# yilane/rag-project-icd10

Measured on AMD Instinct MI355X. Metric: queries_per_sec, higher is better.
Workload: dtype f16; 1 GPU; BASELINE configs[1]: 10000 random fp32 768-d queries x 37000x768 corpus, top_k=10, search only (pre-embedded, HBM-resident inputs), level reweight fused; nq_per_gpu=10000, corpus_rows=37000, dim=768, top_k=10, mode=auto, parallelism=single GPU, collective_ranks=1

## Files before the change

### include/icd_search.h

```cpp
#ifndef ICD_SEARCH_H
#define ICD_SEARCH_H

#include <stdint.h>

#ifdef __cplusplus
extern "C" {
#endif

#define ICD_ABI_VERSION 6
#define ICD_MAX_K 128

typedef struct icd_index icd_index;

typedef enum icd_status {
    ICD_OK = 0,
    ICD_ERR_INVALID = -1,
    ICD_ERR_HIP = -2,
    ICD_ERR_NOMEM = -3,
    ICD_ERR_UNSUPPORTED = -4,
    ICD_ERR_STATE = -5
} icd_status;

typedef enum icd_mode {
    ICD_MODE_AUTO = 0,
// ... 116 lines not shown
                          int32_t lmax, const int32_t *limits, int32_t ranker, double rrf_c, const double *weights, int32_t norm,
                          int32_t k, int32_t reweighted, double *out_adj, double *out_fused, int64_t *out_ids,
                          int32_t *out_levels, uint32_t *out_reqbits, int32_t out_on_device, void *stream);

int icd_index_search_hybrid_grouped(icd_index *idx, icd_fusion *fusion, icd_grouping *grouping, const float *queries, int64_t nq, int32_t R,
                                    int32_t queries_on_device, const int32_t *limits, icd_rowmask *const *masks, const float *radius,
                                    const float *range_filter, int32_t ranker, double rrf_c, const double *weights, int32_t norm, int32_t k,
                                    int32_t group_size, int32_t reweighted, double *out_adj, double *out_fused, int64_t *out_ids,
                                    int32_t *out_levels, uint32_t *out_reqbits, int32_t *out_groups, int32_t out_on_device, void *stream);
int icd_fusion_fuse_lists_grouped(icd_index *idx, icd_fusion *fusion, icd_grouping *grouping, const float *scores, const int64_t *ids,
                                  int64_t nq, int32_t R, int32_t lmax, const int32_t *limits, int32_t ranker, double rrf_c,
                                  const double *weights, int32_t norm, int32_t k, int32_t group_size, int32_t reweighted, double *out_adj,
                                  double *out_fused, int64_t *out_ids, int32_t *out_levels, uint32_t *out_reqbits, int32_t *out_groups,
                                  int32_t out_on_device, void *stream);

typedef struct icd_sparse icd_sparse;
#define ICD_SPARSE_MAX_QUERY_TERMS 64
int icd_sparse_tile_rows(void);
int icd_sparse_pack(const int64_t *row_off, const uint32_t *terms, const float *vals, int64_t n, int64_t vocab,
                    int64_t *post_off, uint32_t *post_row, float *post_val);
int icd_sparse_create(icd_index *idx, const int64_t *row_off, const uint32_t *terms, const float *vals, int64_t vocab,
                      int32_t max_nq, int32_t max_k, icd_sparse **out);
int icd_sparse_destroy(icd_sparse *sp);
int icd_sparse_stats(icd_sparse *sp, int64_t *out_vocab, int64_t *out_nnz, int64_t *out_bytes);
int icd_sparse_search(icd_index *idx, icd_sparse *sp, const int64_t *q_off, const uint32_t *q_terms, const float *q_vals,
                      int64_t nq, int32_t k, int32_t queries_on_device, icd_rowmask *const *masks, int32_t reweighted,
                      double *out_adj, float *out_raw, int64_t *out_ids, int32_t *out_levels, int32_t out_on_device, void *stream);
int icd_sparse_search_range(icd_index *idx, icd_sparse *sp, const int64_t *q_off, const uint32_t *q_terms, const float *q_vals,
                            int64_t nq, int32_t k, int32_t queries_on_device, icd_rowmask *const *masks,
                            const float *radius, const float *range_filter, const float *after_scores, const int64_t *after_ids,
                            int32_t bounds_on_device, int32_t reweighted,
                            double *out_adj, float *out_raw, int64_t *out_ids, int32_t *out_levels, int32_t out_on_device, void *stream);

int icd_grouping_pair_sparse(icd_index *idx, icd_grouping *grouping, icd_sparse *sp);
int icd_sparse_search_grouped(icd_index *idx, icd_sparse *sp, icd_grouping *grouping, const int64_t *q_off, const uint32_t *q_terms,
                              const float *q_vals, int64_t nq, int32_t k, int32_t group_size, int32_t queries_on_device,
                              icd_rowmask *const *masks, int32_t reweighted, double *out_adj, float *out_raw, int64_t *out_ids,
                              int32_t *out_levels, int32_t *out_groups, int32_t out_on_device, void *stream);

int icd_sparse_match_rowmasks(icd_index *idx, icd_sparse *sp, const int64_t *q_off, const uint32_t *q_terms, const int32_t *min_match,
                              int64_t nq, int32_t queries_on_device, icd_rowmask *const *base_masks, icd_rowmask **out_masks, void *stream);
int icd_rowmask_read(icd_rowmask *m, uint32_t *out_words, int64_t out_count);

typedef struct icd_columns icd_columns;
#define ICD_FILTER_MAX_COLUMNS 256
#define ICD_FILTER_RANGE 1
#define ICD_FILTER_SET 2
#define ICD_FILTER_TEXT 3
#define ICD_FILTER_AND 4
#define ICD_FILTER_OR 5
#define ICD_FILTER_NOT 6
int icd_columns_create(icd_index *idx, const int32_t *cols, int32_t ncols, icd_columns **out);
int icd_columns_destroy(icd_columns *columns);
int icd_columns_stats(icd_columns *columns, int32_t *out_ncols, int64_t *out_rows, int64_t *out_bytes);
int icd_filter_program_check(const int64_t *prog_off, const uint32_t *prog, int64_t nq, int32_t ncols, int64_t vocab, char *msg, int64_t msg_len);
int icd_filter_rowmasks(icd_index *idx, icd_columns *columns, icd_sparse *sparse, const int64_t *prog_off, const uint32_t *prog, int64_t nq,
                        icd_rowmask *const *base_masks, icd_rowmask **out_masks, void *stream);

#define ICD_SELECT_MAX_LIMIT 16384
int icd_rowmask_select(icd_index *idx, icd_rowmask *const *masks, int64_t nq, const int64_t *offsets, int32_t limit, int64_t *out_ids,
                       int64_t *out_total, int32_t *out_taken, int32_t out_on_device, void *stream);

int icd_rowmask_group_counts(icd_index *idx, icd_grouping *grouping, icd_rowmask *const *masks, int64_t nq,
                             int32_t *out_counts , int32_t out_on_device, void *stream);

typedef struct icd_mmr icd_mmr;
int icd_mmr_create(icd_index *idx, int64_t max_nq, icd_mmr **out);
int icd_mmr_destroy(icd_mmr *mmr);
int icd_mmr_stats(icd_mmr *mmr, int64_t *out_max_nq, int64_t *out_bytes);
int icd_index_search_mmr(icd_index *idx, icd_mmr *mmr, icd_rowmask *const *masks, const float *queries, int64_t nq, int32_t k,
                         int32_t fetch_k, double lambda, int32_t queries_on_device, const float *radius, const float *range_filter,
                         int32_t bounds_on_device, int32_t reweighted, double *out_adj, float *out_raw, int64_t *out_ids,
                         int32_t *out_levels, double *out_mmr, int32_t out_on_device, void *stream);

#define ICD_MAX_BOOSTS 4
typedef struct icd_boost icd_boost;
int icd_boost_create(icd_index *idx, int64_t max_nq, icd_boost **out);
int icd_boost_destroy(icd_boost *b);
int icd_boost_stats(icd_boost *b, int64_t *out_max_nq, int64_t *out_bytes);
int icd_index_search_boosted(icd_index *idx, icd_boost *ws, icd_rowmask *const *masks,
                             icd_rowmask *const *boost_masks ,
                             const float *boost_weights      ,
                             const float *queries, int64_t nq, int32_t k, int32_t queries_on_device,
                             const float *radius, const float *range_filter, const float *after_scores, const int64_t *after_ids,
                             int32_t bounds_on_device, int32_t reweighted, double *out_adj, float *out_raw, int64_t *out_ids,
                             int32_t *out_levels, int32_t out_on_device, void *stream);

typedef struct icd_byrows icd_byrows;
int icd_byrows_create(icd_index *idx, int64_t max_nq, icd_byrows **out);
int icd_byrows_destroy(icd_byrows *ws);
int icd_byrows_stats(icd_byrows *ws, int64_t *out_max_nq, int64_t *out_bytes);
int icd_index_search_by_rows(icd_index *idx, icd_byrows *ws, icd_rowmask *const *masks, const int64_t *ids, int64_t nq, int32_t k,
                             int32_t ids_on_device, int32_t include_self, const float *radius, const float *range_filter,
                             int32_t bounds_on_device, int32_t reweighted, double *out_adj, float *out_raw, int64_t *out_ids,
                             int32_t *out_levels, int32_t out_on_device, void *stream);

int icd_merge_topk(int32_t device, const float *scores, const int64_t *ids, const int32_t *levels,
                   int32_t G, int64_t nq, int32_t k,
                   double *out_adj, float *out_raw, int64_t *out_ids, int32_t *out_levels, void *stream);

#define ICD_GROUP_ID_BYTES 128
typedef struct icd_group icd_group;
typedef enum icd_group_mode { ICD_GROUP_ROW_SHARD = 0, ICD_GROUP_QUERY_SHARD = 1 } icd_group_mode;
int icd_group_unique_id(uint8_t *out_id );
int icd_group_create(icd_index *local, const uint8_t *id, int32_t rank, int32_t world, int32_t mode, int32_t max_nq,
                     int32_t max_k, icd_group **out);
int icd_group_prepare(icd_index *local, int32_t with_comm, int32_t rank, int32_t world, int32_t mode, int32_t max_nq,
                      int32_t max_k, icd_group **out);
int icd_group_connect(icd_group *group, const uint8_t *id);
int icd_group_search(icd_group *group, const float *queries, int64_t nq, int32_t k, int32_t gather, double *out_adj,
                     float *out_raw, int64_t *out_ids, int32_t *out_levels, void *stream);
int icd_group_destroy(icd_group *group);

int icd_index_lookup_levels(icd_index *idx, const int64_t *ids, int64_t count, int32_t *out_levels,
                            void *stream);

int icd_hier_rescore(int32_t device, const double *adj, const int64_t *ids, int64_t nq, int32_t k, int64_t id_base,
                     int64_t n_rows, const uint8_t *row_tags, const double *q_params, const double *weights,
                     int32_t *out_order, double *out_enhanced, double *out_score, double *out_vs, double *out_hb,
                     double *out_boost, void *stream);

int icd_hier_rescore_entities(int32_t device, const double *adj, const int64_t *ids, int64_t nq, int32_t k, int64_t id_base,
                              int64_t n_rows, const uint8_t *row_tags, const double *q_params, const double *weights,
                              int32_t *out_order, double *out_enhanced, double *out_score, double *out_vs, double *out_hb,
                              double *out_boost, void *stream);

int icd_score_stats(int32_t device, const double *scores, const int32_t *order, int64_t nq, int32_t k, int32_t use,
                    double *out, void *stream);

int icd_pack_winners(int32_t device, const int32_t *order, const int64_t *ids, const float *raw, const double *adj, const double *enhanced,
                     const double *vs, const double *hb, const double *boost, int64_t nq, int32_t k, int32_t kk, double *out, void *stream);

int icd_cosine_rows(int32_t device, const float *x, const float *y, int64_t y_stride, int64_t nq, int32_t dim,
                    double *out, void *stream);

#define ICD_TERM_MAX_LEN 32
int icd_term_first_match(int32_t device, const int32_t *key_cp, const int32_t *key_off, int32_t n_keys, const int32_t *term_cp,
                         const int32_t *term_off, int32_t n_terms, int32_t *out_first, void *stream);

int icd_packed_attention(int32_t device, const float *qkv, int64_t ld, const int32_t *starts, int32_t nseq, int32_t heads,
                         int32_t head_dim, int32_t max_len, float *out, int64_t out_ld, void *stream);

int icd_split_bf16x3(int32_t device, const float *x, int64_t rows, int32_t cols, int64_t ld, int32_t act, void *out, void *stream);

int icd_index_stats(icd_index *idx, icd_stats *out);

int icd_index_cert_terms(icd_index *idx, float *cmax, float *dcmax, int32_t *cexp, float *qnorm, float *qres, int64_t count);

int icd_index_set_chunks(icd_index *idx, int32_t chunks);

int icd_index_set_second_pass(icd_index *idx, int32_t enabled);

enum { ICD_OPT_FAMILY_ORDER = 1, ICD_OPT_STREAM_ONE = 2, ICD_OPT_HOST_ONE = 3, ICD_OPT_PACING_SHIFT = 4, ICD_OPT_PACING_LEAD = 5, ICD_OPT_EXACT_NARROW = 6,
       ICD_OPT_WIDE_FROM = 7 };
int icd_index_set_option(icd_index *idx, int32_t option, int32_t value);

int icd_unpack_query_slices(int32_t device, const void *gathered, int32_t world, int64_t nq, int32_t k, double *out_adj,
                                  float *out_raw, int64_t *out_ids, int32_t *out_levels, void *stream);

typedef struct icd_encoder icd_encoder;
typedef struct {
    int32_t layers, hidden, heads, inter;
    int32_t vocab, max_pos;
    int32_t pos_offset;
    float ln_eps;
    const float *word_emb, *pos_emb, *type_emb0, *emb_ln_g, *emb_ln_b;
    const float *const *w_qkv;  const float *const *b_qkv;
    const float *const *w_ao;   const float *const *b_ao;
    const float *const *ln1_g;  const float *const *ln1_b;
    const float *const *w_up;   const float *const *b_up;
    const float *const *w_down; const float *const *b_down;
    const float *const *ln2_g;  const float *const *ln2_b;
    int32_t arithmetic;
} icd_encoder_desc;
enum { ICD_ENCODER_ARITH_FP32 = 0, ICD_ENCODER_ARITH_BF16X3 = 1 };
#define ICD_ENCODER_MAX_TOKENS 512
#define ICD_ENCODER_MAX_SEQS 64
int icd_encoder_create(int32_t device, const icd_encoder_desc *desc, icd_encoder **out);
int icd_encoder_encode(icd_encoder *e, const int32_t *ids, const int32_t *lengths, int32_t nseq, int32_t pooling, int32_t normalize,
                       float *out, int32_t out_on_device, float *hidden_out, void *stream);
int icd_encoder_encode_many(icd_encoder *e, const int32_t *ids, const int32_t *lengths, int64_t nseq, int32_t pooling, int32_t normalize,
                            float *out, int32_t out_on_device, void *stream);
int icd_encoder_destroy(icd_encoder *e);

int icd_index_debug_counters(icd_index *idx, unsigned long long *out, int32_t count);

int icd_index_set_profiling(icd_index *idx, int32_t enabled);
int icd_index_last_profile(icd_index *idx, icd_profile *out);
int icd_index_profile_summary(icd_index *idx, icd_profile *out_mean, int32_t *out_count);

#ifdef __cplusplus
}
#endif
#endif
```

### rag_project_icd10_amd/_native.py

```python
from __future__ import annotations

import ctypes as C
import math
import os
import sys
from typing import Optional

import numpy as np

_HERE = os.path.dirname(os.path.abspath(__file__))
LIB_PATH = os.path.join(_HERE, "csrc", "libicdsearch.so")

MODE_AUTO = 0
MODE_EXACT = 1
MAX_K = 128
ABI_VERSION = 6

EXPORTED_SYMBOLS = (
    "icd_abi_version", "icd_last_error", "icd_device_count", "icd_index_create", "icd_index_create_view", "icd_index_destroy",
    "icd_index_search", "icd_index_search_reweighted", "icd_merge_topk", "icd_index_lookup_levels",
    "icd_index_stats", "icd_index_cert_terms", "icd_index_set_chunks", "icd_index_debug_counters", "icd_index_set_profiling",
    "icd_index_last_profile", "icd_index_profile_summary", "icd_index_set_option", "icd_packed_attention",
    "icd_hier_rescore", "icd_hier_rescore_entities",
    "icd_score_stats",
    "icd_cosine_rows",
    "icd_term_first_match",
    "icd_index_set_second_pass",
    "icd_group_unique_id", "icd_group_create", "icd_group_prepare", "icd_group_connect", "icd_group_search", "icd_group_destroy",
    "icd_unpack_query_slices", "icd_split_bf16x3", "icd_encoder_create", "icd_encoder_encode", "icd_encoder_encode_many", "icd_encoder_destroy", "icd_pack_winners",
    "icd_grouping_create", "icd_grouping_destroy", "icd_grouping_stats", "icd_index_search_grouped",
    "icd_index_search_range",
    "icd_rowmask_create", "icd_rowmask_destroy", "icd_rowmask_stats", "icd_rowmask_pack", "icd_index_search_masked",
    "icd_fusion_create", "icd_fusion_destroy", "icd_fusion_stats", "icd_index_search_hybrid", "icd_fusion_fuse_lists",
    "icd_sparse_tile_rows", "icd_sparse_pack", "icd_sparse_create", "icd_sparse_destroy", "icd_sparse_stats", "icd_sparse_search",
    "icd_grouping_pair_sparse", "icd_sparse_search_grouped", "icd_index_search_hybrid_grouped", "icd_fusion_fuse_lists_grouped",
    "icd_sparse_search_range",
    "icd_sparse_match_rowmasks", "icd_rowmask_read",
    "icd_columns_create", "icd_columns_destroy", "icd_columns_stats", "icd_filter_program_check", "icd_filter_rowmasks",
    "icd_rowmask_select", "icd_rowmask_group_counts",
    "icd_mmr_create", "icd_mmr_destroy", "icd_mmr_stats", "icd_index_search_mmr",
    "icd_boost_create", "icd_boost_destroy", "icd_boost_stats", "icd_index_search_boosted",
    "icd_byrows_create", "icd_byrows_destroy", "icd_byrows_stats", "icd_index_search_by_rows",
    "icd_grouping_prepare_scorers", "icd_index_search_grouped_scored",
    "icd_grouping_prepare_maxsim", "icd_index_search_maxsim",
)
MAXSIM_SCORERS = {"sum": 1, "mean": 2}
MAXSIM_MAX_T = 64
GROUP_SCORERS = {"max": 0, "sum": 1, "avg": 2}
MAX_BOOSTS = 4
SELECT_MAX_LIMIT = 16384
SELECT_SEGMENT_ROWS = 16384
FACET_LDS_GROUPS = 8192
SPARSE_MAX_QUERY_TERMS = 64
MAX_REQUESTS = 8
RANKER_RRF, RANKER_WEIGHTED = 0, 1
NORMS = {"none": 0, "cosine": 1, "atan": 2}
MAX_K = 128
CREATE_CORPUS_ON_DEVICE, CREATE_ROW_ORDER, CREATE_NO_PROBE, CREATE_NO_CENTER = 1, 2, 4, 8
OPTIONS = {"family_order": 1, "stream_one": 2, "host_one": 3, "pacing_shift": 4, "pacing_lead": 5, "exact_narrow": 6, "wide_from": 7}
GROUP_ROW_SHARD = 0
GROUP_QUERY_SHARD = 1
GROUP_ID_BYTES = 128
SPLIT_TAIL = 64


class IcdError(RuntimeError):

    def __init__(self, code: int, text: str):
        super().__init__(f"libicdsearch error {code}: {text}")
        self.code = code


class _Stats(C.Structure):
    _fields_ = [("n", C.c_int64), ("dim", C.c_int32), ("device", C.c_int32), ("id_base", C.c_int64),
                ("bytes_corpus_f32", C.c_int64), ("bytes_corpus_f16", C.c_int64), ("bytes_workspace", C.c_int64),
                ("max_nq", C.c_int32), ("max_k", C.c_int32), ("fast_path", C.c_int32), ("rmax", C.c_float),
                ("last_nq", C.c_int64), ("last_fallback", C.c_int64), ("last_chunks", C.c_int32),
                ("last_mode", C.c_int32), ("last_second_pass", C.c_int64), ("last_second_pass_lists", C.c_int32),
                ("second_pass_armed", C.c_int32), ("wide_mode", C.c_int32), ("sparse_fallback_armed", C.c_int32),
                ("centered", C.c_int32), ("mean_share", C.c_float)]


_ENC_LAYER_FIELDS = ("w_qkv", "b_qkv", "w_ao", "b_ao", "ln1_g", "ln1_b", "w_up", "b_up", "w_down", "b_down", "ln2_g", "ln2_b")


class _EncoderDesc(C.Structure):
    _fields_ = ([("layers", C.c_int32), ("hidden", C.c_int32), ("heads", C.c_int32), ("inter", C.c_int32), ("vocab", C.c_int32),
                 ("max_pos", C.c_int32), ("pos_offset", C.c_int32), ("ln_eps", C.c_float),
                 ("word_emb", C.c_void_p), ("pos_emb", C.c_void_p), ("type_emb0", C.c_void_p), ("emb_ln_g", C.c_void_p), ("emb_ln_b", C.c_void_p)]
                + [(name, C.POINTER(C.c_void_p)) for name in _ENC_LAYER_FIELDS] + [("arithmetic", C.c_int32)])


ENCODER_ARITH = {"fp32": 0, "bf16x3": 1}
ENCODER_MAX_TOKENS = 512
ENCODER_MAX_SEQS = 64


class _Profile(C.Structure):
    _fields_ = [("ms_prep", C.c_float), ("ms_coarse", C.c_float), ("ms_finalize", C.c_float),
                ("ms_exact", C.c_float), ("ms_exact_finalize", C.c_float), ("ms_total", C.c_float)]


_lib = None


def load_library(path: Optional[str] = None) -> C.CDLL:
    global _lib
    if _lib is not None and path is None:
        return _lib
    p = path or os.environ.get("ICD_SEARCH_LIB", LIB_PATH)
    if not os.path.exists(p):
        raise ImportError(
            f"{p} not found: the HIP extension is not built. Run `python -c 'import __graft_entry__ as g; g.build()'` "
            f"or `make -C rag_project_icd10_amd/csrc`. There is no CPU fallback for the search path.")
    lib = C.CDLL(p)
    vp, i32, i64 = C.c_void_p, C.c_int32, C.c_int64
    lib.icd_abi_version.restype = C.c_int
    lib.icd_last_error.restype = C.c_char_p
    lib.icd_device_count.restype = C.c_int
    lib.icd_index_create.argtypes = [vp, i64, i32, vp, i64, i32, i32, i32, i32, C.POINTER(vp)]
    lib.icd_index_create_view.argtypes = [vp, vp, i64, i32, i32, i32, i32, C.POINTER(vp)]
    lib.icd_index_destroy.argtypes = [vp]
    lib.icd_index_search.argtypes = [vp, vp, i64, i32, i32, i32, vp, vp, i32, vp]
    lib.icd_index_search_reweighted.argtypes = [vp, vp, i64, i32, i32, i32, vp, vp, vp, vp, i32, vp]
    lib.icd_grouping_create.argtypes = [vp, vp, i64, i32, i32, C.POINTER(vp)]
    lib.icd_grouping_destroy.argtypes = [vp]
    lib.icd_grouping_stats.argtypes = [vp, C.POINTER(i64), C.POINTER(i64), C.POINTER(i64)]
    lib.icd_index_search_grouped.argtypes = [vp, vp, vp, i64, i32, i32, i32, i32, vp, vp, vp, vp, vp, i32, vp]
    lib.icd_grouping_prepare_scorers.argtypes = [vp, vp]
    lib.icd_index_search_grouped_scored.argtypes = [vp, vp, vp, i64, i32, i32, i32, i32, i32, vp, vp, vp, vp, vp, vp, vp, i32, vp]
    lib.icd_grouping_prepare_maxsim.argtypes = [vp, vp, i64, i64]
    lib.icd_index_search_maxsim.argtypes = [vp, vp, vp, vp, i64, i32, i32, i32, vp, vp, vp, vp, vp, i32, vp]
    lib.icd_index_search_range.argtypes = [vp, vp, i64, i32, i32, vp, vp, vp, vp, i32, i32, vp, vp, vp, vp, i32, vp]
    lib.icd_rowmask_create.argtypes = [vp, vp, i64, i32, C.POINTER(vp)]
    lib.icd_rowmask_destroy.argtypes = [vp]
    lib.icd_rowmask_stats.argtypes = [vp, C.POINTER(i64), C.POINTER(i64)]
    lib.icd_rowmask_pack.argtypes = [vp, i64, i64, vp, i64]
    lib.icd_index_search_masked.argtypes = [vp, vp, vp, i64, i32, i32, vp, vp, vp, vp, i32, i32, vp, vp, vp, vp, i32, vp]
    lib.icd_fusion_create.argtypes = [vp, i64, C.POINTER(vp)]
    lib.icd_fusion_destroy.argtypes = [vp]
    lib.icd_fusion_stats.argtypes = [vp, C.POINTER(i64), C.POINTER(i64)]
    lib.icd_index_search_hybrid.argtypes = [vp, vp, vp, i64, i32, i32, vp, vp, vp, vp, i32, i32, i32, C.c_double, vp, i32, i32, i32,
                                            vp, vp, vp, vp, vp, i32, vp]
    lib.icd_fusion_fuse_lists.argtypes = [vp, vp, vp, vp, i64, i32, i32, vp, i32, C.c_double, vp, i32, i32, i32, vp, vp, vp, vp, vp, i32, vp]
    lib.icd_sparse_tile_rows.restype = C.c_int
    lib.icd_sparse_pack.argtypes = [vp, vp, vp, i64, i64, vp, vp, vp]
    lib.icd_sparse_create.argtypes = [vp, vp, vp, vp, i64, i32, i32, C.POINTER(vp)]
    lib.icd_sparse_destroy.argtypes = [vp]
    lib.icd_sparse_stats.argtypes = [vp, C.POINTER(i64), C.POINTER(i64), C.POINTER(i64)]
    lib.icd_sparse_search.argtypes = [vp, vp, vp, vp, vp, i64, i32, i32, vp, i32, vp, vp, vp, vp, i32, vp]
    lib.icd_sparse_search_range.argtypes = [vp, vp, vp, vp, vp, i64, i32, i32, vp, vp, vp, vp, vp, i32, i32, vp, vp, vp, vp, i32, vp]
    lib.icd_grouping_pair_sparse.argtypes = [vp, vp, vp]
    lib.icd_sparse_match_rowmasks.argtypes = [vp, vp, vp, vp, vp, i64, i32, vp, vp, vp]
    lib.icd_rowmask_read.argtypes = [vp, vp, i64]
    lib.icd_columns_create.argtypes = [vp, vp, i32, C.POINTER(vp)]
    lib.icd_columns_destroy.argtypes = [vp]
    lib.icd_columns_stats.argtypes = [vp, C.POINTER(i32), C.POINTER(i64), C.POINTER(i64)]
    lib.icd_filter_program_check.argtypes = [vp, vp, i64, i32, i64, vp, i64]
    lib.icd_filter_rowmasks.argtypes = [vp, vp, vp, vp, vp, i64, vp, vp, vp]
    lib.icd_rowmask_select.argtypes = [vp, vp, i64, vp, i32, vp, vp, vp, i32, vp]
    lib.icd_rowmask_group_counts.argtypes = [vp, vp, vp, i64, vp, i32, vp]
    lib.icd_mmr_create.argtypes = [vp, i64, C.POINTER(vp)]
    lib.icd_mmr_destroy.argtypes = [vp]
    lib.icd_mmr_stats.argtypes = [vp, C.POINTER(i64), C.POINTER(i64)]
    lib.icd_index_search_mmr.argtypes = [vp, vp, vp, vp, i64, i32, i32, C.c_double, i32, vp, vp, i32, i32, vp, vp, vp, vp, vp, i32, vp]
    lib.icd_byrows_create.argtypes = [vp, i64, C.POINTER(vp)]
    lib.icd_byrows_destroy.argtypes = [vp]
    lib.icd_byrows_stats.argtypes = [vp, C.POINTER(i64), C.POINTER(i64)]
    lib.icd_index_search_by_rows.argtypes = [vp, vp, vp, vp, i64, i32, i32, i32, vp, vp, i32, i32, vp, vp, vp, vp, i32, vp]
    lib.icd_boost_create.argtypes = [vp, i64, C.POINTER(vp)]
    lib.icd_boost_destroy.argtypes = [vp]
    lib.icd_boost_stats.argtypes = [vp, C.POINTER(i64), C.POINTER(i64)]
    lib.icd_index_search_boosted.argtypes = [vp, vp, vp, vp, vp, vp, i64, i32, i32, vp, vp, vp, vp, i32, i32, vp, vp, vp, vp, i32, vp]
    lib.icd_index_search_hybrid_grouped.argtypes = [vp, vp, vp, vp, i64, i32, i32, vp, vp, vp, vp, i32, C.c_double, vp, i32, i32, i32, i32,
                                                    vp, vp, vp, vp, vp, vp, i32, vp]
    lib.icd_fusion_fuse_lists_grouped.argtypes = [vp, vp, vp, vp, vp, i64, i32, i32, vp, i32, C.c_double, vp, i32, i32, i32, i32,
                                                  vp, vp, vp, vp, vp, vp, i32, vp]
    lib.icd_sparse_search_grouped.argtypes = [vp, vp, vp, vp, vp, vp, i64, i32, i32, i32, vp, i32, vp, vp, vp, vp, vp, i32, vp]
    lib.icd_merge_topk.argtypes = [i32, vp, vp, vp, i32, i64, i32, vp, vp, vp, vp, vp]
    lib.icd_index_lookup_levels.argtypes = [vp, vp, i64, vp, vp]
    lib.icd_index_stats.argtypes = [vp, C.POINTER(_Stats)]
    lib.icd_index_cert_terms.argtypes = [vp, vp, vp, vp, vp, vp, i64]
    lib.icd_index_set_chunks.argtypes = [vp, i32]
    lib.icd_index_set_second_pass.argtypes = [vp, i32]
    lib.icd_index_set_option.argtypes = [vp, i32, i32]
    lib.icd_group_unique_id.argtypes = [vp]
    lib.icd_group_create.argtypes = [vp, vp, i32, i32, i32, i32, i32, C.POINTER(vp)]
    lib.icd_group_prepare.argtypes = [vp, i32, i32, i32, i32, i32, i32, C.POINTER(vp)]
    lib.icd_group_connect.argtypes = [vp, vp]
    lib.icd_group_search.argtypes = [vp, vp, i64, i32, i32, vp, vp, vp, vp, vp]
    lib.icd_group_destroy.argtypes = [vp]
    lib.icd_split_bf16x3.argtypes = [i32, vp, i64, i32, i64, i32, vp, vp]
    lib.icd_unpack_query_slices.argtypes = [i32, vp, i32, i64, i32, vp, vp, vp, vp, vp]
    lib.icd_packed_attention.argtypes = [i32, vp, i64, vp, i32, i32, i32, i32, vp, i64, vp]
    lib.icd_encoder_create.argtypes = [i32, C.POINTER(_EncoderDesc), C.POINTER(vp)]
    lib.icd_encoder_encode.argtypes = [vp, vp, vp, i32, i32, i32, vp, i32, vp, vp]
    lib.icd_encoder_encode_many.argtypes = [vp, vp, vp, i64, i32, i32, vp, i32, vp]
    lib.icd_encoder_destroy.argtypes = [vp]
    lib.icd_hier_rescore.argtypes = [i32, vp, vp, i64, i32, i64, i64, vp, vp, vp, vp, vp, vp, vp, vp, vp, vp]
    lib.icd_hier_rescore_entities.argtypes = lib.icd_hier_rescore.argtypes
    lib.icd_score_stats.argtypes = [i32, vp, vp, i64, i32, i32, vp, vp]
    lib.icd_pack_winners.argtypes = [i32, vp, vp, vp, vp, vp, vp, vp, vp, i64, i32, i32, vp, vp]
    lib.icd_cosine_rows.argtypes = [i32, vp, vp, i64, i64, i32, vp, vp]
    lib.icd_term_first_match.argtypes = [i32, vp, vp, i32, vp, vp, i32, vp, vp]
    lib.icd_index_debug_counters.argtypes = [vp, vp, i32]
    lib.icd_index_set_profiling.argtypes = [vp, i32]
    lib.icd_index_last_profile.argtypes = [vp, C.POINTER(_Profile)]
    lib.icd_index_profile_summary.argtypes = [vp, C.POINTER(_Profile), C.POINTER(C.c_int32)]
    have = lib.icd_abi_version()
    if have != ABI_VERSION:
        raise ImportError(f"{p} has ABI version {have}, this package needs {ABI_VERSION}: rebuild it (make -C rag_project_icd10_amd/csrc)")
    for name in EXPORTED_SYMBOLS:
# ... 1476 lines not shown
```

### rag_project_icd10_amd/csrc/coarse_flat_kernel.hpp

```cpp
#pragma once
#include "coarse_common.hpp"
#include "flat_partition.hpp"

namespace icd {

struct CoarseFlatArgs {
    const _Float16 *q16;
    const _Float16 *c16;
    int nq;
    int n;
    int n_pad;
    int ctiles;
    int total_units;
    int units_per_wg;
    int pos_period;
    int list_tiles;
    int boot_tiles;
    int sparse_from;
    int P;
    float *part_scores;
    int *part_rows;
    float *bounds;
    unsigned int *shared_thr;
    const int *nq_ptr;
    const int *qlist;
    int nwg_virtual;
    int skip_below;
    unsigned long long *dbg;
    unsigned int *pace;
    int pace_period;
    int pace_epochs;
    int pace_shift;
    int pace_lead;
};

constexpr int CO_BOOT_MIN_TILES = 6;
constexpr int CO_KP_WIDE = 24;
constexpr int CO_BOOT_TILES = 8;
constexpr int PACE_SPIN_LIMIT = 20000;
constexpr int CO_SPARSE_FROM = 40;

template <int KP>
__device__ __forceinline__ float flush_emit_parallel(const char *smem, uint32_t qb, int h, int rot, int nlo, int nhi, float thr,
                                                      bool store, float *out_scores, int *out_rows) {
    constexpr int CAP = 64, HALF = 32;
    float v[HALF];
    uint32_t rw[HALF];
    const int lo_end = nlo, hi_begin = CAP - nhi;
#pragma unroll
    for (int j = 0; j < HALF; ++j) {
        const int slot = HALF * h + ((j + rot) & (HALF - 1));
        const bool valid = slot < lo_end || slot >= hi_begin;
        const float sv = *reinterpret_cast<const float *>(smem + qb + slot * 4);
        rw[j] = *reinterpret_cast<const uint32_t *>(smem + qb + CAP * 4 + slot * 4);
        v[j] = valid ? sv : -INFINITY;
    }
    auto pair_sum = [&](int x) {
        const auto sw = __builtin_amdgcn_permlane32_swap((unsigned)x, (unsigned)x, false, false);
        return x + (int)(h ? sw[0] : sw[1]);
    };
    const int total = nlo + nhi;
    float mx = -INFINITY;
#pragma unroll
    for (int j = 0; j < HALF; ++j) mx = fmaxf(mx, v[j]);
    {
        const auto sw = __builtin_amdgcn_permlane32_swap(__float_as_uint(mx), __float_as_uint(mx), false, false);
        mx = fmaxf(mx, __uint_as_float(h ? sw[0] : sw[1]));
    }
    uint32_t lo = order_f32(thr), hi = order_f32(mx);
    int cnt_lo = 0;
#pragma unroll
    for (int j = 0; j < HALF; ++j) cnt_lo += (v[j] > thr) ? 1 : 0;
    cnt_lo = pair_sum(cnt_lo);
    bool active = total > KP && cnt_lo > KP && hi > lo + 1u;
    while (__builtin_amdgcn_ballot_w64(active) != 0ull) {
        const uint32_t mid = lo + ((hi - lo) >> 1);
        const float midf = unorder_f32(mid);
        int c = 0;
#pragma unroll
        for (int j = 0; j < HALF; ++j) c += (v[j] > midf) ? 1 : 0;
        c = pair_sum(c);
        if (active) {
            if (c >= KP) { lo = mid; cnt_lo = c; } else hi = mid;
            active = cnt_lo > KP && hi > lo + 1u;
        }
    }
    float cut = total > KP ? unorder_f32(lo) : -INFINITY;
    float bound = total > KP ? cut : thr;
    int quota_ties = 0;
    float tie = 0.0f;
    if (cnt_lo > KP) {
        tie = unorder_f32(hi);
        int above = 0, tied = 0;
#pragma unroll
        for (int j = 0; j < HALF; ++j) { above += (v[j] > tie) ? 1 : 0; tied += (v[j] == tie) ? 1 : 0; }
        const int above_all = pair_sum(above);
        const auto sw = __builtin_amdgcn_permlane32_swap((unsigned)tied, (unsigned)tied, false, false);
        const int tied_low_lane = h ? (int)sw[0] : tied;
        const int room = KP - above_all;
        quota_ties = h ? max(0, min(tied, room - min(tied_low_lane, room))) : min(tied, room);
        cut = tie;
        bound = tie;
    }
    int mine_n = 0;
#pragma unroll
    for (int j = 0; j < HALF; ++j) mine_n += (v[j] > cut) ? 1 : 0;
    mine_n += quota_ties;
    const auto swn = __builtin_amdgcn_permlane32_swap((unsigned)mine_n, (unsigned)mine_n, false, false);
    const int other_n = (int)(h ? swn[0] : swn[1]);
    int dest = h ? other_n : 0;
    const int kept = mine_n + other_n;
    if (store) {
        int ties_left = quota_ties;
#pragma unroll
        for (int j = 0; j < HALF; ++j) {
            bool take = v[j] > cut;
            if (!take && ties_left > 0 && v[j] == tie && cnt_lo > KP) { take = true; --ties_left; }
            if (take) {
                out_scores[dest] = v[j];
                out_rows[dest] = (int)rw[j];
                ++dest;
            }
        }
        if (h == 0) {
            for (int d = kept; d < KP; ++d) { out_scores[d] = -INFINITY; out_rows[d] = -1; }
        }
    }
    return bound;
}

template <int KP, typename Ops>
__device__ __forceinline__ void compact_all_parallel(char *smem, Sel2 &st, uint32_t qb, int h, int rot) {
    constexpr int CAP = 64, HALF = 32;
    const int mine = Ops::used(st, h);
    const auto swm = __builtin_amdgcn_permlane32_swap((unsigned)mine, (unsigned)mine, false, false);
    const int other = (int)(h ? swm[0] : swm[1]);
    const int nlo = st.kept + (h ? other : mine), nhi = h ? mine : other;
    const int total = nlo + nhi;
    float v[HALF];
    uint32_t rw[HALF];
    const int lo_end = nlo, hi_begin = CAP - nhi;
#pragma unroll
    for (int j = 0; j < HALF; ++j) {
        const int slot = HALF * h + ((j + rot) & (HALF - 1));
        const bool valid = slot < lo_end || slot >= hi_begin;
        const float sv = *reinterpret_cast<const float *>(smem + qb + slot * 4);
        rw[j] = *reinterpret_cast<const uint32_t *>(smem + qb + CAP * 4 + slot * 4);
        v[j] = valid ? sv : -INFINITY;
    }
    auto pair_sum = [&](int x) {
        const auto sw = __builtin_amdgcn_permlane32_swap((unsigned)x, (unsigned)x, false, false);
        return x + (int)(h ? sw[0] : sw[1]);
    };
    float mx = -INFINITY;
#pragma unroll
    for (int j = 0; j < HALF; ++j) mx = fmaxf(mx, v[j]);
    {
        const auto sw = __builtin_amdgcn_permlane32_swap(__float_as_uint(mx), __float_as_uint(mx), false, false);
        mx = fmaxf(mx, __uint_as_float(h ? sw[0] : sw[1]));
    }
    uint32_t lo = order_f32(st.thr), hi = order_f32(mx);
    int cnt_lo = 0;
#pragma unroll
    for (int j = 0; j < HALF; ++j) cnt_lo += (v[j] > st.thr) ? 1 : 0;
    cnt_lo = pair_sum(cnt_lo);
    bool active = total > KP && cnt_lo > KP && hi > lo + 1u;
    while (__builtin_amdgcn_ballot_w64(active) != 0ull) {
        const uint32_t mid = lo + ((hi - lo) >> 1);
        const float midf = unorder_f32(mid);
        int c = 0;
#pragma unroll
        for (int j = 0; j < HALF; ++j) c += (v[j] > midf) ? 1 : 0;
        c = pair_sum(c);
        if (active) {
            if (c >= KP) { lo = mid; cnt_lo = c; } else hi = mid;
            active = cnt_lo > KP && hi > lo + 1u;
        }
    }
    float cut = unorder_f32(lo);
    int quota_ties = 0;
    float tie = 0.0f;
    if (cnt_lo > KP) {
        tie = unorder_f32(hi);
        int above = 0, tied = 0;
#pragma unroll
        for (int j = 0; j < HALF; ++j) { above += (v[j] > tie) ? 1 : 0; tied += (v[j] == tie) ? 1 : 0; }
        const int above_all = pair_sum(above);
        const auto sw = __builtin_amdgcn_permlane32_swap((unsigned)tied, (unsigned)tied, false, false);
        const int tied_low_lane = h ? (int)sw[0] : tied;
        const int room = KP - above_all;
        quota_ties = h ? max(0, min(tied, room - min(tied_low_lane, room))) : min(tied, room);
        cut = tie;
    }
    int mine_n = 0;
#pragma unroll
    for (int j = 0; j < HALF; ++j) mine_n += (v[j] > cut) ? 1 : 0;
    mine_n += quota_ties;
    const auto swn = __builtin_amdgcn_permlane32_swap((unsigned)mine_n, (unsigned)mine_n, false, false);
    const int other_n = (int)(h ? swn[0] : swn[1]);
    if (total > KP) {
        int dest = h ? other_n : 0;
        int ties_left = quota_ties;
#pragma unroll
        for (int j = 0; j < HALF; ++j) {
            bool take = v[j] > cut;
            if (!take && ties_left > 0 && v[j] == tie && cnt_lo > KP) { take = true; --ties_left; }
            if (take) {
                *reinterpret_cast<float *>(smem + qb + dest * 4) = v[j];
                *reinterpret_cast<uint32_t *>(smem + qb + CAP * 4 + dest * 4) = rw[j];
                ++dest;
            }
        }
        const int kept = mine_n + other_n;
        st.thr = cut;
        st.kept = kept;
        st.aw0 = h ? qb + (CAP - 1) * 4 : qb + (uint32_t)kept * 4;
        st.aw = st.aw0;
    }
}

constexpr int CF_PRODUCT_VAR = 1 + 2 + 8 + 128 + 16 + 2048 + 32768;
constexpr int CF_CACHED_VAR = CF_PRODUCT_VAR + 2097152 + 4194304 + 134217728 + 268435456 + 1073741824;
constexpr int CF_PACED_VAR = CF_PRODUCT_VAR + 67108864;
__host__ __device__ constexpr int cf_ring_stages(int var) { return (var & 1048576) ? 6 : CO_S; }
__host__ __device__ constexpr int cf_lds_bytes(int var) { return cf_ring_stages(var) * CO_STAGE_BYTES + CO_BM * CO_CAP * 8 + ((var & 1048576) ? 0 : 4 * 256); }
#define ICD_CF_STAMP(t) do { __builtin_amdgcn_sched_barrier(0); \
    asm volatile("s_memtime %0\n\ts_waitcnt lgkmcnt(0)" : "=s"(t) :: "memory"); \
    __builtin_amdgcn_sched_barrier(0); } while (0)

template <int D, int VAR = CF_PRODUCT_VAR, int KP = CO_KP, bool PERSIST = false>
__global__ __launch_bounds__(256, 1) void coarse_flat_kernel(CoarseFlatArgs a) {
    constexpr int CO_QUOTA = (CO_CAP - KP) / 2 - CO_CHECK_EVERY;
    static_assert(CO_QUOTA >= 8 && KP + 2 * (CO_QUOTA + CO_CHECK_EVERY) <= CO_CAP, "candidate buffer layout");
    constexpr bool EARLY_THR = (VAR & 1) != 0;
    constexpr bool DMA_SPREAD = (VAR & 2) != 0;
    constexpr bool Q_AGPR = (VAR & 8) != 0;
    constexpr bool PF2 = (VAR & 128) != 0;
    constexpr bool REV_WAIT = (VAR & 4) != 0;
    constexpr bool QUAD = (VAR & 16) != 0;
    constexpr bool SETPRIO = (VAR & 131072) != 0;
    constexpr int EXCH = (VAR & 524288) ? 4 : ((VAR & 262144) ? 2 : 1);
    constexpr bool X16 = (VAR & 32768) != 0;
    static_assert(!X16 || (QUAD && (VAR & 8) != 0 && D % 32 == 0), "the 16x16x32 form is built on the quad select and pinned queries");
    constexpr int EPOCH = ((VAR & 32) && (VAR & 2048)) ? 32 : ((VAR & 32) ? 16 : ((VAR & 2048) ? 24 : 0));
    constexpr bool NOBAR = (VAR & 256) != 0, NOVM = (VAR & 512) != 0, STAMPS = (VAR & 1024) != 0;
    constexpr bool NOPASS = (VAR & 4096) != 0, NOSEL = (VAR & 8192) != 0, NODMA = (VAR & 16384) != 0;
    constexpr bool PAIRBAR = (VAR & 1048576) != 0;
    constexpr bool DMA_WIDE = (VAR & 2097152) != 0;
    constexpr bool BOOT_MED3 = (VAR & 4194304) != 0;
    constexpr bool DIRTY_GUARD = (VAR & 8388608) != 0;
    constexpr bool SPARSE_PRE = (VAR & 16777216) != 0;
    static_assert(!SPARSE_PRE || (QUAD && X16), "the group pre-filter is built on the quad select of the 16x16x32 form");
    static_assert(!DMA_WIDE || (X16 && DMA_SPREAD && PF2 && !NODMA), "the wide spread is built on the product's 16x16x32 stage");
    constexpr bool CLOCKS = (VAR & 33554432) != 0;
    constexpr bool PACE = (VAR & 67108864) != 0;
    static_assert(!PACE || (EARLY_THR && EXCH == 1 && !PERSIST), "the pace poll rides on the early threshold load of every tile");
    static_assert(!(CLOCKS && STAMPS), "one use of the debug buffer at a time");
    constexpr bool LOOKAHEAD = (VAR & 134217728) != 0;
    constexpr int LA_B = (VAR & 268435456) ? 8 : 4;
    constexpr bool LA_MAX = (VAR & 536870912) != 0;
    static_assert(!LOOKAHEAD || (QUAD && X16 && !SPARSE_PRE), "the look-ahead tests are built on the quad select of the 16x16x32 form");
    constexpr bool LA_GUARDX = (VAR & 1073741824) != 0;
    static_assert(LOOKAHEAD || (VAR & (268435456 | 536870912 | 1073741824)) == 0, "sub-flags of the look-ahead bit");
    static_assert(!LA_GUARDX || !DIRTY_GUARD, "one form of the overflow guard");
    constexpr int S = cf_ring_stages(VAR);
    constexpr int VM_MID = NOVM ? 63 : (PAIRBAR ? 4 : 4 * (S - 3));
    constexpr int PRO = PAIRBAR ? 4 : S - 1;
    constexpr int VM_TILE_END = NOVM ? 0 : (PAIRBAR ? (DMA_WIDE ? 6 : 8) : (DMA_WIDE ? 4 * (S - 2) - 2 : 4 * (S - 2)));
    constexpr int KS = D / CO_BK;
    constexpr int NF = D / 16;
    static_assert(KS % S == 0, "ring slot must be a compile-time function of the stage");
    using Ops = Sel2Ops<KP>;
    extern __shared__ __attribute__((aligned(16))) char smem[];

    const int tid = threadIdx.x, lane = tid & 63;
    const int wave = __builtin_amdgcn_readfirstlane(tid >> 6);
    const int c = lane & 31, h = lane >> 5;
    const int q16 = lane & 15, g16 = lane >> 4;
    const int nq_act = PERSIST && a.nq_ptr ? min(__builtin_amdgcn_readfirstlane(*a.nq_ptr), a.nq) : a.nq;
    const int total_units = PERSIST ? ((nq_act + CO_BM - 1) / CO_BM) * a.ctiles : a.total_units;
    const int nwg_logical = PERSIST ? (total_units + a.units_per_wg - 1) / a.units_per_wg : (int)gridDim.x;
    if (PERSIST && nq_act <= a.skip_below) return;
    unsigned long long clk_c0 = 0, clk_r0 = 0;
    if constexpr (CLOCKS) {
        clk_c0 = __builtin_amdgcn_s_memtime();
        clk_r0 = __builtin_amdgcn_s_memrealtime();
        __builtin_amdgcn_s_waitcnt(0xC07F);
    }

    uint32_t src_off[4];
#pragma unroll
    for (int i = 0; i < 4; ++i) {
        const int row_local = (wave * 4 + i) * 8 + (lane >> 3);
        const int piece = (lane & 7) ^ ((row_local >> 1) & 7);
        src_off[i] = (uint32_t)row_local * (uint32_t)(D * 2) + (uint32_t)piece * 16u - (uint32_t)(i * 1024);
    }
    uint32_t rd_off[4];
    if constexpr (X16) {
#pragma unroll
        for (int k2 = 0; k2 < 2; ++k2) rd_off[k2] = (uint32_t)q16 * 128u + (uint32_t)(((4 * k2 + g16) ^ ((q16 >> 1) & 7)) * 16);
        rd_off[2] = rd_off[3] = 0u;
    } else {
        const int sw = (c >> 1) & 7;
#pragma unroll
        for (int s = 0; s < 4; ++s) rd_off[s] = (uint32_t)c * 128u + (uint32_t)(((2 * s + h) ^ sw) * 16);
    }
    auto read_frags = [&](half8 (&f)[4], int ring_slot, int s) {
        if constexpr (X16) {
            const char *sb = smem + ring_slot * CO_STAGE_BYTES + (s & 1) * 8192 + rd_off[s >> 1];
#pragma unroll
            for (int t = 0; t < 4; ++t) f[t] = *reinterpret_cast<const half8 *>(sb + t * 2048);
        } else {
            const char *sb = smem + ring_slot * CO_STAGE_BYTES + rd_off[s];
#pragma unroll
            for (int t = 0; t < 4; ++t) f[t] = *reinterpret_cast<const half8 *>(sb + t * 4096);
        }
    };
    constexpr uint32_t RING_BYTES = (uint32_t)S * CO_STAGE_BYTES;
    const uint32_t wave_qbase = RING_BYTES + (uint32_t)(wave * 32) * Ops::QBYTES;
    const uint32_t wave_scratch = RING_BYTES + (uint32_t)CO_BM * Ops::QBYTES + (uint32_t)wave * 256u;
    unsigned long long st_vm = 0, st_bar = 0, st_body = 0, st_sel = 0, st_tiles = 0, st_prev = 0;
    unsigned long long st_comp[2] = {0, 0}, st_thr = 0, st_boot = 0;
    [[maybe_unused]] unsigned long long st_app = 0;
    const int last_tile = a.ctiles - 1;

    half8 qf[NF];
    int cur_mtile = -1;
    for (int vblock = (int)blockIdx.x; vblock < (PERSIST ? nwg_logical : (int)blockIdx.x + 1); vblock += PERSIST ? (int)gridDim.x : 1) {
    const int wg = flat_workgroup_of_block(vblock, nwg_logical, a.pos_period);
    const int u_begin = wg * a.units_per_wg;
    const int u_end = min(total_units, u_begin + a.units_per_wg);
    if (u_begin >= u_end) continue;
    int u = u_begin;
    [[maybe_unused]] bool pacing = false;
    [[maybe_unused]] int pace_cls = 0, pace_members = 0, pace_last_epochs = 0;
    [[maybe_unused]] bool pace_last_mine = false;
    if constexpr (PACE) {
        if (a.pace && a.pace_period > 0) {
            pacing = true;
            pace_cls = wg % a.pace_period;
            pace_members = (nwg_logical - pace_cls + a.pace_period - 1) / a.pace_period;
            const int last_units = total_units - (nwg_logical - 1) * a.units_per_wg;
            pace_last_mine = ((nwg_logical - 1) % a.pace_period) == pace_cls;
            pace_last_epochs = last_units >> a.pace_shift;
        }
    }
    while (u < u_end) {
        const int mtile = u / a.ctiles;
        const int t0 = u - mtile * a.ctiles;
        const int run0 = max(u_begin - mtile * a.ctiles, 0);
        const int run1 = min(u_end - mtile * a.ctiles, a.ctiles);
        const int j = (t0 - run0) / a.list_tiles;
        const int t1 = min(run1, run0 + (j + 1) * a.list_tiles);
        const int ntiles = t1 - t0;
        const int ord = flat_first_ordinal(mtile, wg, a.ctiles, a.units_per_wg, a.list_tiles) + j;
        const int slot0 = mtile * CO_BM;

        if (mtile != cur_mtile) {
            if constexpr (X16) {
#pragma unroll
                for (int gr = 0; gr < 2; ++gr) {
                    int qr = slot0 + wave * 32 + 16 * gr + q16;
                    if (PERSIST && a.qlist) qr = a.qlist[min(qr, nq_act - 1)];
                    const _Float16 *qrow = a.q16 + (size_t)qr * D + 8 * g16;
#pragma unroll
                    for (int s = 0; s < NF / 2; ++s) qf[gr * (NF / 2) + s] = *reinterpret_cast<const half8 *>(qrow + 32 * s);
                }
            } else {
                int qr = slot0 + wave * 32 + c;
                if (PERSIST && a.qlist) qr = a.qlist[min(qr, nq_act - 1)];
                const _Float16 *qrow = a.q16 + (size_t)qr * D + 8 * h;
#pragma unroll
                for (int s = 0; s < NF; ++s) qf[s] = *reinterpret_cast<const half8 *>(qrow + 16 * s);
            }
            if constexpr (Q_AGPR) {
#pragma unroll
                for (int s = 0; s < NF; ++s) asm volatile("" : "+a"(qf[s]));
            }
            cur_mtile = mtile;
        }
        const __amdgpu_buffer_rsrc_t crsrc = __builtin_amdgcn_make_buffer_rsrc(
            const_cast<_Float16 *>(a.c16) + (size_t)t0 * CO_BN * D, 0,
            (int)min((size_t)(a.ctiles - t0) * CO_BN * (size_t)(D * 2), (size_t)0x7FFFFFFF), 0x00020000);
        auto issue_pieces = [&](int g_tile, int g_ks, int ring_slot, auto LO, auto HI) {
            const int trow = min(g_tile, last_tile - t0);
            char *dst = smem + ring_slot * CO_STAGE_BYTES + wave * 4096;
            const uint32_t soff = (uint32_t)trow * (uint32_t)(CO_BN * D * 2) + (uint32_t)g_ks * (CO_BK * 2);
            __attribute__((address_space(3))) void *ldst = (__attribute__((address_space(3))) void *)dst;
            constexpr int lo = decltype(LO)::value, hi = decltype(HI)::value;
            if constexpr (lo <= 0 && 0 < hi) __builtin_amdgcn_raw_ptr_buffer_load_lds(crsrc, ldst, 16, src_off[0], soff, 0, 0);
            if constexpr (lo <= 1 && 1 < hi) __builtin_amdgcn_raw_ptr_buffer_load_lds(crsrc, ldst, 16, src_off[1], soff, 1024, 0);
            if constexpr (lo <= 2 && 2 < hi) __builtin_amdgcn_raw_ptr_buffer_load_lds(crsrc, ldst, 16, src_off[2], soff, 2048, 0);
            if constexpr (lo <= 3 && 3 < hi) __builtin_amdgcn_raw_ptr_buffer_load_lds(crsrc, ldst, 16, src_off[3], soff, 3072, 0);
        };
        auto issue_stage = [&](int g_tile, int g_ks, int ring_slot) {
            issue_pieces(g_tile, g_ks, ring_slot, std::integral_constant<int, 0>{}, std::integral_constant<int, 4>{});
        };

        Sel2 st;
        Ops::init(st, wave_qbase + (uint32_t)c * Ops::QBYTES, h, (slot0 + wave * 32 + c) < nq_act && !NOPASS);
        float boot1 = -INFINITY, boot2 = -INFINITY, boot3 = -INFINITY;
        const int boot_tiles = ntiles >= CO_BOOT_MIN_TILES ? min(a.boot_tiles, ntiles / 3) : 0;
        unsigned int *my_shared = a.shared_thr + (slot0 + wave * 32 + c);
        const bool publish = (slot0 + wave * 32 + c) < nq_act;
        uint32_t published = 0u;
        int dirty = 0;
        auto filter_reg = [&](const f32x16 (&pa)[4], auto F, uint32_t rowbase, auto GUARD) {
            constexpr int f = decltype(F)::value;
            constexpr int t = f >> 4, r = f & 15;
            constexpr uint32_t roff = (uint32_t)(t * 32 + (r & 3) + 8 * (r >> 2));
            float v = pa[t][r];
            if constexpr (decltype(GUARD)::value) {
                if ((int)(rowbase + roff) >= a.n) v = -INFINITY;
            }
            const bool pass = v > st.thr;
            if (__builtin_expect(__builtin_amdgcn_ballot_w64(pass) != 0ull, 0)) {
                asm volatile("" ::: "memory");
                if (pass) {
                    *reinterpret_cast<float *>(smem + st.aw) = v;
                    *reinterpret_cast<uint32_t *>(smem + st.aw + Ops::ROW_OFF) = rowbase + roff;
                    st.aw += st.inc;
                }
            }
            if constexpr (r % CO_CHECK_EVERY == CO_CHECK_EVERY - 1) {
                if (__builtin_amdgcn_ballot_w64(Ops::used(st, h) > CO_QUOTA) != 0ull)
                    Ops::template check<PAIRBAR>(st, lane, smem, wave_qbase, wave_scratch, false, CO_LIMIT, STAMPS ? st_comp : nullptr, CO_QUOTA);
            }
        };

        [[maybe_unused]] auto append_quad = [&](unsigned long long m0, unsigned long long m1, unsigned long long m2, unsigned long long m3,
                               float v0, float v1, float v2, float v3, uint32_t rowq) {
            uint32_t r1, r2, r3, aw = st.aw;
            const uint32_t inc = st.inc;
            asm volatile("v_or_b32_e32 %1, 1, %12\n\t"
                         "v_or_b32_e32 %2, 2, %12\n\t"
                         "v_or_b32_e32 %3, 3, %12\n\t"
                         "s_mov_b64 exec, %4\n\t"
                         "ds_write2st64_b32 %0, %8, %12 offset1:1\n\t"
                         "v_add_u32_e32 %0, %0, %13\n\t"
                         "s_mov_b64 exec, %5\n\t"
                         "ds_write2st64_b32 %0, %9, %1 offset1:1\n\t"
                         "v_add_u32_e32 %0, %0, %13\n\t"
                         "s_mov_b64 exec, %6\n\t"
                         "ds_write2st64_b32 %0, %10, %2 offset1:1\n\t"
                         "v_add_u32_e32 %0, %0, %13\n\t"
                         "s_mov_b64 exec, %7\n\t"
                         "ds_write2st64_b32 %0, %11, %3 offset1:1\n\t"
                         "v_add_u32_e32 %0, %0, %13\n\t"
                         "s_mov_b64 exec, -1"
                         : "+v"(aw), "=&v"(r1), "=&v"(r2), "=&v"(r3)
                         : "s"(m0), "s"(m1), "s"(m2), "s"(m3), "v"(v0), "v"(v1), "v"(v2), "v"(v3), "v"(rowq), "v"(inc)
                         : "memory");
            st.aw = aw;
            if constexpr (DIRTY_GUARD) dirty = 1;
            if constexpr (STAMPS) st_app += (unsigned long long)(__builtin_popcountll(m0) + __builtin_popcountll(m1) + __builtin_popcountll(m2) + __builtin_popcountll(m3));
        };
        [[maybe_unused]] auto quad_guard = [&]() {
            if constexpr (LA_GUARDX) {
                const uint32_t aw = st.aw, aw0 = st.aw0;
                uint32_t dist;
                asm("v_sad_u32 %0, %1, %2, 0" : "=v"(dist) : "v"(aw), "v"(aw0));
                if (__builtin_amdgcn_ballot_w64(dist > 4u * (uint32_t)CO_QUOTA) != 0ull)
                    Ops::template check<PAIRBAR>(st, lane, smem, wave_qbase, wave_scratch, false, CO_LIMIT, STAMPS ? st_comp : nullptr, CO_QUOTA);
            } else
            if constexpr (DIRTY_GUARD) {
                if (dirty) {
                    dirty = 0;
                    if (__builtin_amdgcn_ballot_w64(Ops::used(st, h) > CO_QUOTA) != 0ull)
                        Ops::template check<PAIRBAR>(st, lane, smem, wave_qbase, wave_scratch, false, CO_LIMIT, STAMPS ? st_comp : nullptr, CO_QUOTA);
                }
            } else if (__builtin_amdgcn_ballot_w64(Ops::used(st, h) > CO_QUOTA) != 0ull)
                Ops::template check<PAIRBAR>(st, lane, smem, wave_qbase, wave_scratch, false, CO_LIMIT, STAMPS ? st_comp : nullptr, CO_QUOTA);
        };
        auto filter_quad = [&](const f32x16 (&pa)[X16 ? 1 : 4], const f32x4 (&px)[X16 ? 16 : 1], auto Q, uint32_t rowbase, auto GUARD) {
            constexpr int q = decltype(Q)::value;
            constexpr int t = q >> 2, g = q & 3;
            constexpr uint32_t qoff = X16 ? (uint32_t)(16 * (q >> 1) + 4 * (q & 1)) : (uint32_t)(t * 32 + 8 * g);
            float v0 = X16 ? px[X16 ? q : 0][0] : pa[X16 ? 0 : t][4 * g + 0], v1 = X16 ? px[X16 ? q : 0][1] : pa[X16 ? 0 : t][4 * g + 1];
            float v2 = X16 ? px[X16 ? q : 0][2] : pa[X16 ? 0 : t][4 * g + 2], v3 = X16 ? px[X16 ? q : 0][3] : pa[X16 ? 0 : t][4 * g + 3];
            const uint32_t rowq = rowbase + qoff;
            if constexpr (decltype(GUARD)::value) {
                if ((int)(rowq + 0u) >= a.n) v0 = -INFINITY;
                if ((int)(rowq + 1u) >= a.n) v1 = -INFINITY;
                if ((int)(rowq + 2u) >= a.n) v2 = -INFINITY;
                if ((int)(rowq + 3u) >= a.n) v3 = -INFINITY;
            }
            const unsigned long long m0 = __builtin_amdgcn_ballot_w64(v0 > st.thr), m1 = __builtin_amdgcn_ballot_w64(v1 > st.thr);
            const unsigned long long m2 = __builtin_amdgcn_ballot_w64(v2 > st.thr), m3 = __builtin_amdgcn_ballot_w64(v3 > st.thr);
            if (__builtin_expect(((m0 | m1) | (m2 | m3)) != 0ull, 0)) {
                uint32_t r1, r2, r3;
                asm volatile("v_or_b32_e32 %1, 1, %12\n\t"
                             "v_or_b32_e32 %2, 2, %12\n\t"
                             "v_or_b32_e32 %3, 3, %12\n\t"
                             "s_mov_b64 exec, %4\n\t"
                             "ds_write2st64_b32 %0, %8, %12 offset1:1\n\t"
                             "v_add_u32_e32 %0, %0, %13\n\t"
                             "s_mov_b64 exec, %5\n\t"
                             "ds_write2st64_b32 %0, %9, %1 offset1:1\n\t"
                             "v_add_u32_e32 %0, %0, %13\n\t"
                             "s_mov_b64 exec, %6\n\t"
                             "ds_write2st64_b32 %0, %10, %2 offset1:1\n\t"
                             "v_add_u32_e32 %0, %0, %13\n\t"
                             "s_mov_b64 exec, %7\n\t"
                             "ds_write2st64_b32 %0, %11, %3 offset1:1\n\t"
                             "v_add_u32_e32 %0, %0, %13\n\t"
                             "s_mov_b64 exec, -1"
                             : "+v"(st.aw), "=&v"(r1), "=&v"(r2), "=&v"(r3)
                             : "s"(m0), "s"(m1), "s"(m2), "s"(m3), "v"(v0), "v"(v1), "v"(v2), "v"(v3), "v"(rowq), "v"(st.inc)
                             : "memory");
                if constexpr (DIRTY_GUARD) dirty = 1;
                if constexpr (STAMPS) st_app += (unsigned long long)(__builtin_popcountll(m0) + __builtin_popcountll(m1) + __builtin_popcountll(m2) + __builtin_popcountll(m3));
            }
            if constexpr (q % 2 == 1) {
                if constexpr (DIRTY_GUARD) {
                    if (dirty) {
                        dirty = 0;
                        if (__builtin_amdgcn_ballot_w64(Ops::used(st, h) > CO_QUOTA) != 0ull)
                            Ops::template check<PAIRBAR>(st, lane, smem, wave_qbase, wave_scratch, false, CO_LIMIT, STAMPS ? st_comp : nullptr, CO_QUOTA);
                    }
                } else
                if (__builtin_amdgcn_ballot_w64(Ops::used(st, h) > CO_QUOTA) != 0ull)
                    Ops::template check<PAIRBAR>(st, lane, smem, wave_qbase, wave_scratch, false, CO_LIMIT, STAMPS ? st_comp : nullptr, CO_QUOTA);
            }
        };
        static_assert(!QUAD || Ops::ROW_OFF == 256, "ds_write2st64_b32 offset1:1 = the row array of the query's buffer");
        auto filter_group = [&](const f32x16 (&pa)[X16 ? 1 : 4], const f32x4 (&px)[X16 ? 16 : 1], auto G, uint32_t rowbase, auto GUARD) {
            constexpr int g = decltype(G)::value;
            const f32x4 &x0 = px[X16 ? 2 * g : 0], &x1 = px[X16 ? 2 * g + 1 : 0];
            float m = raw_max3_f32(x0[0], x0[1], x0[2]);
            m = raw_max3_f32(m, x0[3], x1[0]);
            m = raw_max3_f32(m, x1[1], x1[2]);
            m = raw_max_f32(m, x1[3]);
            if (__builtin_expect(__builtin_amdgcn_ballot_w64(m > st.thr) != 0ull, 0)) {
                filter_quad(pa, px, std::integral_constant<int, 2 * g>{}, rowbase, GUARD);
                filter_quad(pa, px, std::integral_constant<int, 2 * g + 1>{}, rowbase, GUARD);
            }
        };
        auto filter_block = [&](const f32x4 (&px)[X16 ? 16 : 1], auto Q0, uint32_t rowbase, auto GUARD) {
            constexpr int q0 = decltype(Q0)::value;
            unsigned long long m[LA_B][LA_MAX ? 1 : 4];
            auto masked = [&](auto Q, auto I) {
                constexpr int q = decltype(Q)::value, i = decltype(I)::value;
                float v = px[X16 ? q : 0][i];
                if constexpr (decltype(GUARD)::value) {
                    if ((int)(rowbase + (uint32_t)(16 * (q >> 1) + 4 * (q & 1) + i)) >= a.n) v = -INFINITY;
                }
                return v;
            };
            using I0 = std::integral_constant<int, 0>; using I1 = std::integral_constant<int, 1>;
            using I2 = std::integral_constant<int, 2>; using I3 = std::integral_constant<int, 3>;
            auto cmp4 = [&](auto Q, unsigned long long &m0, unsigned long long &m1, unsigned long long &m2, unsigned long long &m3) {
                const float t0 = masked(Q, I0{}), t1 = masked(Q, I1{}), t2 = masked(Q, I2{}), t3 = masked(Q, I3{}), thr = st.thr;
                asm volatile("v_cmp_gt_f32_e64 %0, %4, %8\n\t"
                             "v_cmp_gt_f32_e64 %1, %5, %8\n\t"
                             "v_cmp_gt_f32_e64 %2, %6, %8\n\t"
                             "v_cmp_gt_f32_e64 %3, %7, %8"
                             : "=&s"(m0), "=&s"(m1), "=&s"(m2), "=&s"(m3)
                             : "v"(t0), "v"(t1), "v"(t2), "v"(t3), "v"(thr));
            };
            static_for<0, LA_B>([&](auto J) {
                using Q = std::integral_constant<int, q0 + decltype(J)::value>;
                constexpr int j = decltype(J)::value;
                if constexpr (LA_MAX) {
                    const float mx = raw_max_f32(raw_max3_f32(masked(Q{}, I0{}), masked(Q{}, I1{}), masked(Q{}, I2{})), masked(Q{}, I3{}));
                    const float thr = st.thr;
                    unsigned long long mq;
                    asm volatile("v_cmp_gt_f32_e64 %0, %1, %2" : "=s"(mq) : "v"(mx), "v"(thr));
                    m[j][0] = mq;
                } else cmp4(Q{}, m[j][0], m[j][LA_MAX ? 0 : 1], m[j][LA_MAX ? 0 : 2], m[j][LA_MAX ? 0 : 3]);
            });
            __builtin_amdgcn_sched_barrier(0);
            static_for<0, LA_B>([&](auto J) {
                constexpr int j = decltype(J)::value, q = q0 + j;
                using Q = std::integral_constant<int, q>;
                const uint32_t rowq = rowbase + (uint32_t)(16 * (q >> 1) + 4 * (q & 1));
                const f32x4 &x = px[X16 ? q : 0];
                if constexpr (LA_MAX) {
                    if (__builtin_expect(m[j][0] != 0ull, 0)) {
                        unsigned long long m0, m1, m2, m3;
                        cmp4(Q{}, m0, m1, m2, m3);
                        append_quad(m0, m1, m2, m3, x[0], x[1], x[2], x[3], rowq);
                    }
                } else {
                    const unsigned long long m0 = m[j][0], m1 = m[j][LA_MAX ? 0 : 1], m2 = m[j][LA_MAX ? 0 : 2], m3 = m[j][LA_MAX ? 0 : 3];
                    if (__builtin_expect(((m0 | m1) | (m2 | m3)) != 0ull, 0)) append_quad(m0, m1, m2, m3, x[0], x[1], x[2], x[3], rowq);
                }
                if constexpr (q % 2 == 1) quad_guard();
            });
        };

        asm volatile("s_waitcnt vmcnt(0)" ::: "memory");
#pragma unroll
        for (int p = 0; p < PRO - (DMA_WIDE ? 1 : 0); ++p) issue_stage(p / KS, p % KS, p % S);
        if constexpr (DMA_WIDE) issue_pieces((PRO - 1) / KS, (PRO - 1) % KS, (PRO - 1) % S, std::integral_constant<int, 0>{}, std::integral_constant<int, 2>{});
        half8 afn[4], bfn[4];
        asm volatile("s_waitcnt vmcnt(%0) lgkmcnt(0)\n\ts_barrier" ::"i"(4 * (PRO - 1) - (DMA_WIDE ? 2 : 0)) : "memory");
        read_frags(afn, 0, 0);
        if constexpr (PF2) read_frags(bfn, 0, 1);
        if constexpr (STAMPS) ICD_CF_STAMP(st_prev);

        for (int tile = 0; tile < ntiles; ++tile) {
            uint32_t seen_early = 0u;
            [[maybe_unused]] uint32_t pace_seen = 0u;
            [[maybe_unused]] bool pace_due = false;
            [[maybe_unused]] int pace_need = -1, pace_done_epoch = 0;
            if constexpr (PACE) {
                if (pacing) {
                    const int done_after = (u - u_begin) + tile + 1;
                    pace_due = (done_after & ((1 << a.pace_shift) - 1)) == 0;
                    pace_done_epoch = (done_after >> a.pace_shift) - 1;
                    pace_need = pace_done_epoch + 1 - a.pace_lead;
                }
            }
            f32x16 acc[X16 ? 1 : 4];
            f32x4 xs[X16 ? 16 : 1];
            if constexpr (!X16) {
#pragma unroll
                for (int t = 0; t < 4; ++t)
#pragma unroll
                    for (int r = 0; r < 16; ++r) acc[X16 ? 0 : t][r] = 0.0f;
            }
#pragma unroll
            for (int t = 0; t < (X16 ? 16 : 1); ++t)
#pragma unroll
                for (int r = 0; r < 4; ++r) xs[t][r] = 0.0f;
            static_for<0, KS>([&](auto KSI) {
                constexpr int ks = decltype(KSI)::value;
                constexpr int slot = ks % S, nslot = (ks + 1) % S;
                auto mfma4 = [&](const half8 (&f)[4], int qi, int t_lo = 0, int t_hi = 4) {
                    if constexpr (X16) {
                        const int quad = qi & 3, kq = (qi >> 2) * 2 + (quad >> 1);
#pragma unroll
                        for (int t = 0; t < 4; ++t) {
                            if (t < t_lo || t >= t_hi) continue;
                            const int rg = 4 * (quad & 1) + t;
#pragma unroll
                            for (int gr = 0; gr < 2; ++gr)
                                xs[2 * rg + gr] = __builtin_amdgcn_mfma_f32_16x16x32_f16(f[t], qf[gr * (NF / 2) + kq], xs[2 * rg + gr], 0, 0, 0);
                        }
                    } else {
#pragma unroll
                        for (int tt = 0; tt < 4; ++tt) {
                            const int t = REV_WAIT ? 3 - tt : tt;
                            acc[t] = __builtin_amdgcn_mfma_f32_32x32x16_f16(f[t], qf[qi], acc[t], 0, 0, 0);
                        }
                    }
                };
                constexpr int M4 = X16 ? 8 : 4;
                half8 f1[4], f2[4], f3[4];
                if constexpr (DMA_WIDE) {
                    constexpr int pks = PAIRBAR ? ks + 3 : ks + S - 2;
                    read_frags(f2, slot, 2);
                    mfma4(afn, ks * 4 + 0, 0, 2);
                    __builtin_amdgcn_sched_barrier(0);
                    issue_pieces(tile + pks / KS, pks % KS, pks % S, std::integral_constant<int, 2>{}, std::integral_constant<int, 3>{});
                    __builtin_amdgcn_sched_barrier(0);
                    mfma4(afn, ks * 4 + 0, 2, 4);
                    read_frags(f3, slot, 3);
                    mfma4(bfn, ks * 4 + 1, 0, 2);
                    __builtin_amdgcn_sched_barrier(0);
                    issue_pieces(tile + pks / KS, pks % KS, pks % S, std::integral_constant<int, 3>{}, std::integral_constant<int, 4>{});
                    __builtin_amdgcn_sched_barrier(0);
                    mfma4(bfn, ks * 4 + 1, 2, 4);
                } else if constexpr (PF2) {
                    read_frags(f2, slot, 2);
                    mfma4(afn, ks * 4 + 0);
                    read_frags(f3, slot, 3);
                    mfma4(bfn, ks * 4 + 1);
                } else {
                    read_frags(f1, slot, 1);
                    mfma4(afn, ks * 4 + 0);
                    read_frags(f2, slot, 2);
                    mfma4(f1, ks * 4 + 1);
                }
                if constexpr (DMA_WIDE) {
                } else {
                __builtin_amdgcn_sched_group_barrier(0x100, 4, 0);
                __builtin_amdgcn_sched_group_barrier(0x008, M4, 0);
                __builtin_amdgcn_sched_group_barrier(0x100, 4, 0);
                __builtin_amdgcn_sched_group_barrier(0x008, M4, 0);
                }
                __builtin_amdgcn_sched_barrier(0);
                if constexpr (STAMPS) {
                    unsigned long long ta, tb, tc;
                    ICD_CF_STAMP(ta);
                    asm volatile("s_waitcnt vmcnt(%0)" ::"i"(VM_MID) : "memory");
                    ICD_CF_STAMP(tb);
                    if constexpr (!NOBAR) asm volatile("s_barrier" ::: "memory");
                    ICD_CF_STAMP(tc);
                    st_body += ta - st_prev; st_vm += tb - ta; st_bar += tc - tb; st_prev = tc;
                } else if constexpr (NOBAR) {
                    asm volatile("s_waitcnt vmcnt(%0) lgkmcnt(0)" ::"i"(VM_MID) : "memory");
                } else if constexpr (PAIRBAR && (ks & 1) == 1) {
                } else {
                    if constexpr (SETPRIO) __builtin_amdgcn_s_setprio(0);
                    asm volatile("s_waitcnt vmcnt(%0) lgkmcnt(0)\n\ts_barrier" ::"i"(VM_MID) : "memory");
                    if constexpr (SETPRIO) __builtin_amdgcn_s_setprio(1);
                }
                __builtin_amdgcn_sched_barrier(0);
                if constexpr (EARLY_THR && ks == KS - 2) {
                    if (EXCH == 1 || (tile & (EXCH - 1)) == EXCH - 1) {
                        asm volatile("global_load_dword %0, %1, off sc1" : "=v"(seen_early) : "v"(my_shared) : "memory");
                    }
                    if constexpr (PACE) {
                        if (pacing && pace_due && pace_need >= 0 && wave == 0) {
                            const unsigned int *pp = a.pace + (size_t)pace_cls * a.pace_epochs + pace_need;
                            asm volatile("global_load_dword %0, %1, off sc1" : "=v"(pace_seen) : "v"(pp) : "memory");
                        }
                    }
                    __builtin_amdgcn_sched_barrier(0);
                }
                if constexpr (!NODMA && !PAIRBAR) {
                    constexpr int nks = ks + S - 1;
                    if constexpr (!DMA_WIDE) issue_stage(tile + nks / KS, nks % KS, nks % S);
                }
                if constexpr (!NODMA && PAIRBAR && !DMA_WIDE && (ks & 1) == 0) {
                    constexpr int n4 = ks + 4, n5 = ks + 5;
                    issue_stage(tile + n4 / KS, n4 % KS, n4 % S);
                    issue_stage(tile + n5 / KS, n5 % KS, n5 % S);
                }
                if constexpr (DMA_WIDE) {
                    constexpr int nks = PAIRBAR ? ks + 4 : ks + S - 1;
                    read_frags(afn, nslot, 0);
                    mfma4(f2, ks * 4 + 2, 0, 2);
                    __builtin_amdgcn_sched_barrier(0);
                    issue_pieces(tile + nks / KS, nks % KS, nks % S, std::integral_constant<int, 0>{}, std::integral_constant<int, 1>{});
                    __builtin_amdgcn_sched_barrier(0);
                    mfma4(f2, ks * 4 + 2, 2, 4);
                    read_frags(bfn, nslot, 1);
                    mfma4(f3, ks * 4 + 3, 0, 2);
                    __builtin_amdgcn_sched_barrier(0);
                    issue_pieces(tile + nks / KS, nks % KS, nks % S, std::integral_constant<int, 1>{}, std::integral_constant<int, 2>{});
                    __builtin_amdgcn_sched_barrier(0);
                    mfma4(f3, ks * 4 + 3, 2, 4);
                } else if constexpr (PF2) {
                    read_frags(afn, nslot, 0);
                    mfma4(f2, ks * 4 + 2);
                    read_frags(bfn, nslot, 1);
                    mfma4(f3, ks * 4 + 3);
                } else {
                    read_frags(f3, slot, 3);
                    mfma4(f2, ks * 4 + 2);
                    read_frags(afn, nslot, 0);
                    mfma4(f3, ks * 4 + 3);
                }
                if constexpr (!DMA_SPREAD) {
                    __builtin_amdgcn_sched_group_barrier(0x020, 4, 1);
                    __builtin_amdgcn_sched_group_barrier(0x100, 4, 1);
                    __builtin_amdgcn_sched_group_barrier(0x008, M4, 1);
                    __builtin_amdgcn_sched_group_barrier(0x100, 4, 1);
                    __builtin_amdgcn_sched_group_barrier(0x008, M4, 1);
                } else if constexpr (DMA_WIDE) {
                } else {
                    __builtin_amdgcn_sched_group_barrier(0x100, 4, 1);
#pragma unroll
                    for (int i = 0; i < 4; ++i) {
                        __builtin_amdgcn_sched_group_barrier(0x008, M4 / 4, 1);
                        if constexpr (!PAIRBAR) __builtin_amdgcn_sched_group_barrier(0x020, 1, 1);
                        else if constexpr ((ks & 1) == 0) __builtin_amdgcn_sched_group_barrier(0x020, 2, 1);
                    }
                    __builtin_amdgcn_sched_group_barrier(0x100, 4, 1);
                    __builtin_amdgcn_sched_group_barrier(0x008, M4, 1);
                }
                __builtin_amdgcn_sched_barrier(0);
            });
            if constexpr (X16 && (VAR & 65536) == 0) {
#pragma unroll
                for (int rg = 0; rg < 8; ++rg)
#pragma unroll
                    for (int i = 0; i < 4; ++i) {
                        const auto sw = __builtin_amdgcn_permlane16_swap(__float_as_uint(xs[2 * rg][i]), __float_as_uint(xs[2 * rg + 1][i]), false, false);
                        xs[2 * rg][i] = __uint_as_float(sw[0]);
                        xs[2 * rg + 1][i] = __uint_as_float(sw[1]);
                    }
            }
            unsigned long long ts0 = 0;
            if constexpr (STAMPS) ICD_CF_STAMP(ts0);
            if (EXCH == 1 || (tile & (EXCH - 1)) == EXCH - 1) {
                uint32_t seen;
                if constexpr (EARLY_THR) {
                    if constexpr (PACE) asm volatile("s_waitcnt vmcnt(%2)" : "+v"(seen_early), "+v"(pace_seen) : "i"(VM_TILE_END) : "memory");
                    else asm volatile("s_waitcnt vmcnt(%1)" : "+v"(seen_early) : "i"(VM_TILE_END) : "memory");
                    seen = seen_early;
                } else {
                    seen = __hip_atomic_load(my_shared, __ATOMIC_RELAXED, __HIP_MEMORY_SCOPE_AGENT);
                }
                if constexpr (PACE) {
                    if (pacing && pace_due && wave == 0) {
                        if (pace_done_epoch < a.pace_epochs && lane == 0)
                            __hip_atomic_fetch_add(a.pace + (size_t)pace_cls * a.pace_epochs + pace_done_epoch, 1u, __ATOMIC_RELAXED, __HIP_MEMORY_SCOPE_AGENT);
                        if (pace_need >= 0 && pace_need < a.pace_epochs) {
                            const uint32_t want = (uint32_t)(pace_members - ((pace_last_mine && pace_need >= pace_last_epochs) ? 1 : 0));
                            uint32_t got = (uint32_t)__builtin_amdgcn_readfirstlane((int)pace_seen);
                            int spins = 0;
                            while (got < want) {
                                if (++spins > PACE_SPIN_LIMIT) { pacing = false; break; }
                                __builtin_amdgcn_s_sleep(16);
                                got = __hip_atomic_load(a.pace + (size_t)pace_cls * a.pace_epochs + pace_need, __ATOMIC_RELAXED, __HIP_MEMORY_SCOPE_AGENT);
                            }
                        }
                    }
                }
                const uint32_t mine_key = order_f32(st.thr);
                if (seen > mine_key) st.thr = unorder_f32(seen);
                else if (h == 0 && publish && mine_key > seen && mine_key > published) {
                    __hip_atomic_fetch_max(my_shared, mine_key, __ATOMIC_RELAXED, __HIP_MEMORY_SCOPE_AGENT);
                    published = mine_key;
                }
            }
            unsigned long long ts_a = 0;
            if constexpr (STAMPS) { ICD_CF_STAMP(ts_a); st_thr += ts_a - ts0; }
            const int tile_row0 = (t0 + tile) * CO_BN;
            const uint32_t rowbase = (uint32_t)(tile_row0 + (X16 ? 8 : 4) * h);
            if (tile < boot_tiles && tile_row0 + CO_BN <= a.n) {
                if constexpr (BOOT_MED3) {
                    float c1 = -INFINITY, c2 = -INFINITY, c3 = -INFINITY;
#pragma unroll
                    for (int t = 0; t < 4; ++t)
#pragma unroll
                        for (int r = 0; r < 16; r += 2) {
                            const float va = X16 ? xs[X16 ? 4 * t + (r >> 2) : 0][r & 3] : acc[X16 ? 0 : t][r];
                            const float vb = X16 ? xs[X16 ? 4 * t + ((r + 1) >> 2) : 0][(r + 1) & 3] : acc[X16 ? 0 : t][r + 1];
                            const float a3 = __builtin_amdgcn_fmed3f(boot2, boot3, va), a2 = __builtin_amdgcn_fmed3f(boot1, boot2, va);
                            boot1 = raw_max_f32(boot1, va); boot2 = a2; boot3 = a3;
                            const float b3 = __builtin_amdgcn_fmed3f(c2, c3, vb), b2 = __builtin_amdgcn_fmed3f(c1, c2, vb);
                            c1 = raw_max_f32(c1, vb); c2 = b2; c3 = b3;
                        }
#pragma unroll
                    for (int i = 0; i < 3; ++i) {
                        const float v = i == 0 ? c1 : (i == 1 ? c2 : c3);
                        const float a3 = __builtin_amdgcn_fmed3f(boot2, boot3, v), a2 = __builtin_amdgcn_fmed3f(boot1, boot2, v);
                        boot1 = raw_max_f32(boot1, v); boot2 = a2; boot3 = a3;
                    }
                } else {
#pragma unroll
                for (int t = 0; t < 4; ++t)
#pragma unroll
                    for (int r = 0; r < 16; ++r) {
                        const float v = X16 ? xs[X16 ? 4 * t + (r >> 2) : 0][r & 3] : acc[X16 ? 0 : t][r];
                        const float lo1 = raw_min_f32(boot1, v);
                        boot1 = raw_max_f32(boot1, v);
                        const float lo2 = raw_min_f32(boot2, lo1);
                        boot2 = raw_max_f32(boot2, lo1);
                        boot3 = raw_max_f32(boot3, lo2);
                    }
                }
                const auto sw = __builtin_amdgcn_permlane32_swap(__float_as_uint(boot3), __float_as_uint(boot3), false, false);
                const float thr0 = fminf(boot3, __uint_as_float(h ? sw[0] : sw[1]));
                if (thr0 > st.thr) st.thr = thr0;
            }
            if constexpr (STAMPS) { unsigned long long ts_b; ICD_CF_STAMP(ts_b); st_boot += ts_b - ts_a; }
            if constexpr (NOSEL) {
                if constexpr (X16) {
#pragma unroll
                    for (int t = 0; t < 16; ++t) asm volatile("" ::"v"(xs[X16 ? t : 0]));
                } else {
#pragma unroll
                    for (int t = 0; t < 4; ++t) asm volatile("" ::"v"(acc[X16 ? 0 : t]));
                }
            } else if constexpr (LOOKAHEAD) {
                if (tile_row0 + CO_BN > a.n) static_for<0, 16 / LA_B>([&](auto Bk) { filter_block(xs, std::integral_constant<int, LA_B * decltype(Bk)::value>{}, rowbase, std::true_type{}); });
                else static_for<0, 16 / LA_B>([&](auto Bk) { filter_block(xs, std::integral_constant<int, LA_B * decltype(Bk)::value>{}, rowbase, std::false_type{}); });
            } else if constexpr (QUAD) {
                if (tile_row0 + CO_BN > a.n) static_for<0, 16>([&](auto Q) { filter_quad(acc, xs, Q, rowbase, std::true_type{}); });
                else if (SPARSE_PRE && tile >= a.sparse_from) static_for<0, 8>([&](auto G) { filter_group(acc, xs, G, rowbase, std::false_type{}); });
                else static_for<0, 16>([&](auto Q) { filter_quad(acc, xs, Q, rowbase, std::false_type{}); });
            } else if (tile_row0 + CO_BN > a.n) static_for<0, 64>([&](auto F) { filter_reg(acc, F, rowbase, std::true_type{}); });
            else static_for<0, 64>([&](auto F) { filter_reg(acc, F, rowbase, std::false_type{}); });
            if constexpr (EPOCH > 0) {
                if ((tile + 1) % EPOCH == 0 && tile + 1 < ntiles && __builtin_amdgcn_ballot_w64(Ops::used(st, h) > 3) != 0ull)
                    compact_all_parallel<KP, Ops>(smem, st, wave_qbase + (uint32_t)c * Ops::QBYTES, h, c);
            }
            if constexpr (STAMPS) {
                unsigned long long ts1;
                ICD_CF_STAMP(ts1);
                st_sel += ts1 - ts0; st_prev += ts1 - ts0; st_tiles += 1;
            }
        }
        asm volatile("s_waitcnt vmcnt(0)" ::: "memory");
        asm volatile("" ::"v"(afn[0]), "v"(afn[1]), "v"(afn[2]), "v"(afn[3]));
        if constexpr (PF2) asm volatile("" ::"v"(bfn[0]), "v"(bfn[1]), "v"(bfn[2]), "v"(bfn[3]));

        {
            const int mine = Ops::used(st, h);
            const auto swm = __builtin_amdgcn_permlane32_swap((unsigned)mine, (unsigned)mine, false, false);
            const int other = (int)(h ? swm[0] : swm[1]);
            const int nlo = st.kept + (h ? other : mine), nhi = h ? mine : other;
            const int slot = slot0 + wave * 32 + c;
            const bool store = slot < nq_act;
            const size_t o = ((size_t)min(slot, nq_act - 1) * a.P + ord) * KP;
            const float bound = flush_emit_parallel<KP>(smem, wave_qbase + (uint32_t)c * Ops::QBYTES, h, c, nlo, nhi, st.thr,
                                                           store, a.part_scores + o, a.part_rows + o);
            if (store && h == 0) {
                a.bounds[(size_t)slot * a.P + ord] = bound;
                if (t1 == a.ctiles) {
                    for (int e = ord + 1; e < a.P; ++e) {
                        const size_t oe = ((size_t)slot * a.P + e) * KP;
                        for (int d = 0; d < KP; ++d) { a.part_scores[oe + d] = -INFINITY; a.part_rows[oe + d] = -1; }
                        a.bounds[(size_t)slot * a.P + e] = -INFINITY;
                    }
                }
            }
        }
        __syncthreads();
        u += ntiles;
    }
    }
    if constexpr (CLOCKS) {
        const unsigned long long c1 = __builtin_amdgcn_s_memtime(), r1 = __builtin_amdgcn_s_memrealtime();
        if (lane == 0 && a.dbg && blockIdx.x < 2048) {
            unsigned long long *d = a.dbg + ((size_t)blockIdx.x * 4 + wave) * 8;
            d[0] = c1 - clk_c0; d[1] = r1 - clk_r0; d[4] = 1;
        }
    }
    if constexpr (STAMPS) {
        if (lane == 0 && a.dbg) {
            unsigned long long *d = a.dbg + ((size_t)blockIdx.x * 4 + wave) * 8;
            d[0] = st_vm; d[1] = st_bar; d[2] = st_body; d[3] = st_sel; d[4] = (st_app << 32) | (st_tiles & 0xffffffffull); d[5] = st_comp[0]; d[6] = st_comp[1];
            d[7] = (st_thr << 32) | (st_boot & 0xffffffffull);
        }
    }
}

}
```

### rag_project_icd10_amd/csrc/flat_partition.hpp

```cpp
#pragma once
#include <algorithm>
#if defined(__HIPCC__)
#define ICD_HD __host__ __device__
#else
#define ICD_HD
#endif

namespace icd {

constexpr int FLAT_SPARE_TILES = 7;

ICD_HD inline int flat_lists_of_run(int len, int list_tiles) { return (len + list_tiles - 1) / list_tiles; }

ICD_HD inline int flat_first_ordinal(int m, int w, int ctiles, int U, int list_tiles) {
    const long long m0 = (long long)m * ctiles, m1 = m0 + ctiles;
    int ord = 0;
    for (long long wp = m0 / U; wp < w; ++wp) {
        const long long r0 = wp * U > m0 ? wp * U : m0;
        const long long r1 = (wp + 1) * U < m1 ? (wp + 1) * U : m1;
        if (r1 > r0) ord += flat_lists_of_run((int)(r1 - r0), list_tiles);
    }
    return ord;
}


ICD_HD inline int flat_class_period(int U, int ctiles) {
    int g = U % ctiles, h = ctiles;
    while (g) { const int t = h % g; h = g; g = t; }
    return ctiles / h;
}

struct FlatPlan { int ctiles, U; };
ICD_HD inline FlatPlan plan_flat_tiles(int mtc, int ctiles_min, int spare, int num_cu) {
    FlatPlan best{ctiles_min, 1};
    double best_cost = 1e300;
    for (int ce = ctiles_min; ce <= ctiles_min + spare; ++ce) {
        const long long units = (long long)mtc * ce;
        const int umin = (int)((units + num_cu - 1) / num_cu) > 1 ? (int)((units + num_cu - 1) / num_cu) : 1;
        const int umax = umin + (umin / 16 > 1 ? umin / 16 : 1);
        for (int U = umin; U <= umax; ++U) {
            const int nwg = (int)((units + U - 1) / U);
            const int members = nwg / flat_class_period(U, ce);
            const double cost = (double)U * (members >= 4 ? 1.0 : (members >= 2 ? 1.03 : 1.07));
            if (cost < best_cost - 1e-9) { best_cost = cost; best.ctiles = ce; best.U = U; }
        }
    }
    return best;
}

ICD_HD inline int flat_workgroup_of_block(int w, int G, int T) {
    if (T <= 0) return w;
    const int xcd = w & 7, q8 = G >> 3, r8 = G & 7;
    const int jx = (xcd < r8 ? xcd * (q8 + 1) : r8 * (q8 + 1) + (xcd - r8) * q8) + (w >> 3);
    const int qT = G / T, rT = G - qT * T;
    if (qT == 0) return jx;
    if (jx < rT * (qT + 1)) return jx / (qT + 1) + (jx % (qT + 1)) * T;
    const int jj = jx - rT * (qT + 1);
    return rT + jj / qT + (jj % qT) * T;
}


constexpr int FLAT_TILE_ROWS = 128;
constexpr int COARSE_MAX_P = 32;
constexpr int PASS2_CHUNKS = 20;
constexpr int PASS2_MAX_P = 24;
constexpr int PASS2_BELOW = 320;
constexpr long long FLAT_DESC_MAX_BYTES = 0x7FFFFFFFLL;

ICD_HD inline int flat_max_list_tiles(int dim) { return (int)(FLAT_DESC_MAX_BYTES / ((long long)FLAT_TILE_ROWS * dim * 2)); }

inline int flat_lists_needed(int mtc, int ctiles, int U, int list_tiles) {
    int worst = 0;
    for (int m = 0; m < mtc; ++m) {
        const long long m1 = (long long)(m + 1) * ctiles;
        const int wl = (int)((m1 - 1) / U);
        const int p = flat_first_ordinal(m, wl + 1, ctiles, U, list_tiles);
        if (p > worst) worst = p;
    }
    return worst;
}

struct CoarsePlanIn {
    int mtc, ctiles, U;
    int nq, k;
    int kp;
    int kp2;
    int max_cand;
    int wide_lists;
    int wide_now;
    int chunks_override;
    int list_override;
    int pass2;
    long long partc_cap, part2_cap;
    int max_list_tiles;
};
struct CoarsePlan {
    int ok;
    int U, list_tiles, P;
    int U2, list_tiles2, P2;
};

inline CoarsePlan plan_coarse_lists(const CoarsePlanIn &in) {
    const int ctiles = in.ctiles, lcap = std::min(in.max_list_tiles, ctiles);
    CoarsePlan r{};
    int U = in.U;
    int L = std::max(1, (ctiles + 1) / 2);
    if (in.wide_lists) L = std::max(1, std::min(L, ctiles / ((in.k + 5) / 6)));
    else if (in.k > 8) L = std::max(1, std::min(L, ctiles / ((in.k + 3) / 4)));
    if (in.list_override > 0) L = in.list_override;
    if (in.chunks_override > 0) {
        U = std::max(1, (ctiles + in.chunks_override - 1) / in.chunks_override);
        L = ctiles;
    } else if (in.wide_now) {
        L = std::max(1, (ctiles + PASS2_CHUNKS - 1) / PASS2_CHUNKS);
    }
    L = std::min(L, lcap);
    auto fits = [&](int p) { return p <= COARSE_MAX_P && p * in.kp <= in.max_cand && (long long)in.nq * p * in.kp <= in.partc_cap; };
    int P = flat_lists_needed(in.mtc, ctiles, U, L);
    while (!fits(P)) {
        if (L < lcap) L = std::min(lcap, L + std::max(1, L / 8));
        else if (U < ctiles) U = std::min(ctiles, U + std::max(1, U / 4));
        else break;
        P = flat_lists_needed(in.mtc, ctiles, U, L);
    }
    r.ok = fits(P) ? 1 : 0;
    r.U = U; r.list_tiles = L; r.P = P;
    if (!r.ok) return r;
    if (in.pass2 && P * in.kp < PASS2_BELOW) {
        int U2 = std::max(1, (ctiles + PASS2_CHUNKS - 1) / PASS2_CHUNKS);
        const int L2 = lcap;
        int p2 = flat_lists_needed(in.mtc, ctiles, U2, L2);
        while ((p2 > PASS2_MAX_P || (long long)in.nq * p2 * in.kp2 > in.part2_cap) && U2 < ctiles) {
            U2 = std::min(ctiles, U2 + std::max(1, U2 / 8));
            p2 = flat_lists_needed(in.mtc, ctiles, U2, L2);
        }
        if (p2 <= PASS2_MAX_P && (long long)in.nq * p2 * in.kp2 <= in.part2_cap && p2 * in.kp2 > P * in.kp) {
            r.U2 = U2; r.list_tiles2 = L2; r.P2 = p2;
        }
    }
    return r;
}

inline long long coarse_partc_entries(int max_nq_pad, int kcap, int kp, int kp_wide, int max_cand) {
    const int lists = std::min(COARSE_MAX_P, std::max(6, (std::min(kcap, 64) + 3) / 4 + 4));
    const int wide = kcap > 64 ? std::min(max_cand / kp_wide, (kcap + 5) / 6 + 4) : 0;
    return std::max((long long)max_nq_pad * std::max(std::max(lists, PASS2_MAX_P) * kp, wide * kp_wide), 1LL << 20);
}
inline long long coarse_part2_entries(int max_nq_pad, int kp) { return (long long)max_nq_pad * PASS2_MAX_P * kp; }

inline int stream_rows_per_wg(int n, int num_cu) {
    const int nwg_max = std::max(1, std::min(num_cu, 256));
    return ((n + nwg_max - 1) / nwg_max + 255) / 256 * 256;
}
struct StreamOneRows { int rps, rows_per_wg, nwg; };
inline StreamOneRows plan_stream_one_rows(int n, int num_cu) {
    const int ncu = std::max(1, std::min(num_cu, 256));
    const int per_cu = (n + ncu - 1) / ncu;
    const int rps = std::min(64, ((per_cu + 3) / 4 + 7) / 8 * 8);
    const int steps = (per_cu + 4 * rps - 1) / (4 * rps);
    StreamOneRows p;
    p.rps = rps; p.rows_per_wg = 4 * rps * steps; p.nwg = (n + p.rows_per_wg - 1) / p.rows_per_wg;
    return p;
}

ICD_HD inline int plan_reduce_levels(int nlists, int per_max, int p_final, int p_cap, int *plan ) {
    const int target = p_final > 0 ? p_final : p_cap;
    int levels = 1;
    long long reach = (long long)per_max * target;
    while (reach < nlists) { reach *= per_max; ++levels; }
    const bool extra = levels % 2 == 0;
    if (levels + (extra ? 1 : 0) > 8) return 0;
    int cnt = 0, cur = nlists;
    if (extra) { cur = (cur + 1) / 2; plan[cnt++] = cur; }
    for (int l = 1; l < levels; ++l) { cur = (cur + per_max - 1) / per_max; plan[cnt++] = cur; }
    plan[cnt++] = p_final > 0 ? p_final : ((cur + per_max - 1) / per_max > 1 ? (cur + per_max - 1) / per_max : 1);
    return cnt;
}

}
```

### rag_project_icd10_amd/csrc/icd_search.hip

```cpp
#include <hip/hip_runtime.h>

#include <algorithm>
#include <atomic>
#include <chrono>
#include <cmath>
#include <cstdarg>
#include <cstdio>
#include <cstring>
#include <mutex>
#include <new>
#include <string>
#include <vector>

#include "../../include/icd_search.h"
#include "coarse_flat_kernel.hpp"
#include "attention_kernel.hpp"
#include "exact_kernel.hpp"
#include "finalize.hpp"
#include "group_topk.hpp"
#include "group_aggregate_kernel.hpp"
#include "maxsim_kernel.hpp"
#include "hybrid_fuse.hpp"
#include "sparse_kernel.hpp"
#include "text_match_kernel.hpp"
#include "filter_mask_kernel.hpp"
#include "mask_select_kernel.hpp"
#include "facet_count_kernel.hpp"
#include "mmr_select_kernel.hpp"
#include "byrows_kernel.hpp"
#include "hier_kernel.hpp"
#include "stats_kernel.hpp"
#include "stream_kernel.hpp"
#include "term_lookup.hpp"
#include "search_policy.hpp"

using namespace icd;

namespace {
thread_local std::string g_err = "";
}

extern "C" __attribute__((visibility("hidden"))) int icd_internal_fail(int code, const char *fmt, ...) {
    char buf[512];
    va_list ap;
    va_start(ap, fmt);
    vsnprintf(buf, sizeof buf, fmt, ap);
    va_end(ap);
    g_err = buf;
    return code;
}

namespace {
constexpr auto &fail = icd_internal_fail;
}

__global__ void unpack_query_slices_kernel(const double *r_adj, const long long *r_ids, const float *r_raw, const int *r_lv,
                                           int world, long long nq, int k, long long width, double *out_adj, float *out_raw,
                                           long long *out_ids, int *out_lv) {
    const long long total = nq * (long long)k;
    const long long base = nq / world, rem = nq % world;
    for (long long e = (long long)blockIdx.x * blockDim.x + threadIdx.x; e < total; e += (long long)gridDim.x * blockDim.x) {
        const long long q = e / k;
        const int j = (int)(e - q * k);
        const long long split = rem * (base + 1);
        const int r = q < split ? (int)(q / (base + 1)) : (int)(rem + (q - split) / (base > 0 ? base : 1));
        const long long lo = (long long)r * base + (r < rem ? r : rem);
        const long long src = (long long)r * width * k + (q - lo) * k + j;
        out_adj[e] = r_adj[src]; out_ids[e] = r_ids[src]; out_raw[e] = r_raw[src]; out_lv[e] = r_lv[src];
    }
}
extern "C" __attribute__((visibility("hidden"))) int icd_internal_unpack_query_slices(const void *r_adj, const void *r_ids, const void *r_raw,
        const void *r_lv, int world, long long nq, int k, long long width, void *out_adj, void *out_raw, void *out_ids, void *out_lv, void *stream) {
    const long long total = nq * (long long)k;
    if (total <= 0) return 0;
    const int blocks = (int)std::min<long long>((total + 255) / 256, 2048);
    hipLaunchKernelGGL(unpack_query_slices_kernel, dim3(blocks), dim3(256), 0, reinterpret_cast<hipStream_t>(stream),
                       static_cast<const double *>(r_adj), static_cast<const long long *>(r_ids), static_cast<const float *>(r_raw),
                       static_cast<const int *>(r_lv), world, nq, k, width, static_cast<double *>(out_adj), static_cast<float *>(out_raw),
                       static_cast<long long *>(out_ids), static_cast<int *>(out_lv));
    return hipGetLastError() == hipSuccess ? 0 : 1;
}

namespace {

#define HIP_TRY(expr)                                                                              \
    do {                                                                                           \
        hipError_t e_ = (expr);                                                                    \
        if (e_ != hipSuccess)                                                                      \
            return fail(e_ == hipErrorOutOfMemory ? ICD_ERR_NOMEM : ICD_ERR_HIP, "%s: %s (%s:%d)", \
                        #expr, hipGetErrorString(e_), __FILE__, __LINE__);                         \
    } while (0)

#define HIP_TRY_OR(undo, expr)                                                                                             \
    do {                                                                                                                   \
        hipError_t e_ = (expr);                                                                                            \
        if (e_ != hipSuccess) {                                                                                            \
            undo;                                                                                                          \
            return fail(e_ == hipErrorOutOfMemory ? ICD_ERR_NOMEM : ICD_ERR_HIP, "%s: %s", #expr, hipGetErrorString(e_)); \
        }                                                                                                                  \
    } while (0)

constexpr size_t PACE_WORDS = (size_t)1 << 18;
constexpr size_t COARSE_CACHED_IMAGE_BYTES = (size_t)96 << 20;
constexpr int FAST_MAX_K = 100;
static_assert(FLAT_TILE_ROWS == CO_BN, "flat_partition.hpp plans tiles of CO_BN rows");
constexpr int NUM_EV = 6;
constexpr int EV_RING = 128;

constexpr int MAX_DEVICES = 64;
template <auto KERN>
hipError_t ensure_dynamic_lds(int device, size_t bytes) {
    static int configured[MAX_DEVICES] = {};
    if (device < 0 || device >= MAX_DEVICES) return hipErrorInvalidDevice;
    if ((size_t)configured[device] >= bytes) return hipSuccess;
    hipError_t e = hipFuncSetAttribute(reinterpret_cast<const void *>(KERN), hipFuncAttributeMaxDynamicSharedMemorySize, (int)bytes);
    if (e == hipSuccess) configured[device] = (int)bytes;
    return e;
}
template <auto KERN, typename... Args>
hipError_t launch_lds(int device, size_t lds_limit, dim3 grid, dim3 block, size_t lds, hipStream_t s, const Args &...args) {
    const hipError_t e = ensure_dynamic_lds<KERN>(device, lds_limit);
    if (e != hipSuccess) return e;
    hipLaunchKernelGGL(KERN, grid, block, lds, s, args...);
    return hipGetLastError();
}

template <typename T>
hipError_t dmalloc(T **p, size_t count) {
    return hipMalloc(reinterpret_cast<void **>(p), std::max<size_t>(count, 1) * sizeof(T));
}

}

struct icd_index {
    uint32_t magic = 0x1CD10A3Du;
    int device = 0;
    bool opt_permute = true;
    bool opt_probe = true;
    bool opt_center = true;
    int opt_pace_shift = 3, opt_pace_lead = 2;
    bool opt_exact_narrow = true;
    int opt_host_one = 3;
    bool opt_stream_one = true;
    bool opt_family_order = true;
    int opt_wide_from = 48;
    int64_t n = 0, id_base = 0;
    long long *row_map = nullptr;
    int n_pad = 0;
    int dim = 0;
    int max_nq = 0, max_nq_pad = 0, max_k = 0;
    bool fast = false;
    float rmax = 0.f;
    float rmax_scaled = 0.f;
    float dcmax_scaled = 0.f;
    int cexp = 0;
    float *cmean = nullptr;
    float rmax_unc_scaled = 0.f;
    float mean_share = 0.f;
    int num_cu = 256;
    float *corpus = nullptr;
    _Float16 *c16 = nullptr;
    int *levels = nullptr;
    float *qdev = nullptr;
    _Float16 *q16 = nullptr;
    float *qnorm = nullptr;
    float *qres = nullptr;
    int *qexp = nullptr;
    unsigned char *qbad = nullptr;
    float *thr0 = nullptr;
    unsigned int *shared_thr = nullptr;
    long long perm_mul = 0; int perm_mod = 0;
    float *partc_s = nullptr; int *partc_r = nullptr; float *partc_b = nullptr; size_t partc_cap = 0;
    float *part2_s = nullptr; int *part2_r = nullptr; float *part2_b = nullptr; size_t part2_cap = 0;
    float *partx_s = nullptr; int *partx_r = nullptr; size_t partx_cap = 0;
    float *lists_s = nullptr; int *lists_r = nullptr; size_t lists_cap = 0;
    int *nflag = nullptr; int *flagged = nullptr;
    int fallback_word = 0;
    int *h_nflag = nullptr;
    int *h_nflag_dev = nullptr;
    hipEvent_t ev_nflag = nullptr;
    unsigned int *scratch_u32 = nullptr;
    int *order = nullptr, *order_key = nullptr; unsigned int *order_hist = nullptr;
    float *o_scores = nullptr; long long *o_ids = nullptr;
    double *o_adj = nullptr; float *o_adj_raw = nullptr; long long *o_adj_ids = nullptr; int *o_adj_lv = nullptr;
    char *h_pin = nullptr, *h_pin_dev = nullptr;
    const float *host_q = nullptr;
    bool host_one_call = false;
    unsigned long long done_seq = 0;
    bool done_armed = false;
    size_t bytes_ws = 0;
    int chunks_override = 0;
    SearchPolicy pol;
    std::mutex mu;
    int probe_flagged = -1, probe_left = -1;
    bool pass2_enabled = true;
    bool adapt_enabled = true;
    bool profiling = false;
    int prof_every = 1;
    long prof_tick = 0;
    bool prof_now = false;
    bool capturing = false;
    hipEvent_t evring[EV_RING][NUM_EV + 1] = {};
    bool evring_valid[EV_RING][NUM_EV + 1] = {};
    long prof_count = 0;
    hipEvent_t *ev = evring[0];
    bool *ev_valid = evring_valid[0];
    int64_t last_nq = 0;
    int last_chunks = 0, last_mode = 0;
    int last_p2 = 0, last_p2_word = 0;
    BandQ *band_dev = nullptr, *h_band = nullptr;
    std::vector<long long> h_row_map;
    int band_pending = 0;
    const uint32_t **mask_dev = nullptr, **h_mask = nullptr;
    uint32_t *mask_ones = nullptr;
    hipEvent_t ev_mask = nullptr;
    bool mask_copy_pending = false;
    int *sel_counts = nullptr;
    long long *sel_off = nullptr, *h_sel_off = nullptr;
    long long *sel_ids = nullptr, *sel_total = nullptr;
    int *sel_taken = nullptr;
    size_t sel_out_cap = 0;
    unsigned long long uid = 0;
    unsigned long long *dbg = nullptr;
    unsigned int *pace = nullptr;
};

namespace {

bool valid(icd_index *idx) { return idx && idx->magic == 0x1CD10A3Du; }

}

extern "C" __attribute__((visibility("hidden"))) int icd_internal_is_view(const icd_index *idx) {
    return idx && idx->row_map ? 1 : 0;
}

namespace {

void free_all(icd_index *x) {
    if (!x) return;
    hipFree(x->corpus); hipFree(x->c16); hipFree(x->levels); hipFree(x->qdev); hipFree(x->q16);
    hipFree(x->qnorm); hipFree(x->qres); hipFree(x->qexp); hipFree(x->qbad); hipFree(x->thr0); hipFree(x->shared_thr); hipFree(x->partc_s); hipFree(x->partc_r); hipFree(x->partc_b); hipFree(x->partx_s);
    hipFree(x->part2_s); hipFree(x->part2_r); hipFree(x->part2_b);
    hipFree(x->partx_r); hipFree(x->lists_s); hipFree(x->lists_r); hipFree(x->nflag); hipFree(x->flagged); hipFree(x->scratch_u32);
    hipFree(x->order); hipFree(x->order_key); hipFree(x->order_hist); hipFree(x->cmean);
    hipFree(x->o_scores); hipFree(x->o_ids); hipFree(x->o_adj); hipFree(x->o_adj_raw);
    hipFree(x->o_adj_ids); hipFree(x->o_adj_lv);
    hipFree(x->dbg);
    hipFree(x->pace);
    hipFree(x->row_map);
    hipFree(x->band_dev);
    if (x->h_band) hipHostFree(x->h_band);
    hipFree(x->mask_dev); hipFree(x->mask_ones);
    if (x->h_mask) hipHostFree(x->h_mask);
    hipFree(x->sel_counts); hipFree(x->sel_off); hipFree(x->sel_ids); hipFree(x->sel_total); hipFree(x->sel_taken);
    if (x->h_sel_off) hipHostFree(x->h_sel_off);
    if (x->ev_mask) hipEventDestroy(x->ev_mask);
    if (x->h_nflag) hipHostFree(x->h_nflag);
    if (x->h_pin) hipHostFree(x->h_pin);
    if (x->ev_nflag) hipEventDestroy(x->ev_nflag);
    for (int r = 0; r < EV_RING; ++r)
        for (int i = 0; i <= NUM_EV; ++i)
            if (x->evring[r][i]) hipEventDestroy(x->evring[r][i]);
    x->magic = 0;
    delete x;
}


int exact_kp_for(int k) { return k <= 16 ? 16 : (k <= 32 ? 32 : (k <= 64 ? 64 : 128)); }

int fullest_round(int mtiles, int slots, int c_lo, int c_hi, double enough) {
    double best = 0;
    int bestc = c_lo;
    for (int c = c_lo; c <= c_hi; ++c) {
        const long items = (long)mtiles * c;
        const double util = (double)items / (double)(((items + slots - 1) / slots) * slots);
        if (util > best + 1e-9) { best = util; bestc = c; }
        if (util >= enough) { bestc = c; break; }
    }
    return bestc;
}

int pick_chunks(int mtiles, int row_tiles, int pmax, int slots) {
    int p = 1;
    if (mtiles * 2 <= slots) p = std::max(1, slots / mtiles);
    else p = fullest_round(mtiles, slots, 1, std::min(pmax, 8), 0.9);
    p = std::min(p, pmax);
    p = std::min(p, std::max(1, row_tiles));
    return std::max(1, p);
}

template <int KP, int E, int NW, int CAPV = 64 * E, int BK = 32, int OCC = 1, int GROUP = 32, bool BAND = false, bool MASK = false, bool BOOST = false>
int launch_exact(icd_index *x, const ExactArgs &a, int mtiles, hipStream_t s) {
    constexpr auto kern = exact_topk_kernel<KP, E, NW, CAPV, BK, OCC, GROUP, BAND, MASK, BOOST>;
    const size_t lds = exact_lds_bytes<KP, E, NW, CAPV, BK>();
    HIP_TRY(launch_lds<kern>(x->device, (size_t)((int)lds), dim3(mtiles * a.P), dim3(NW * 64), lds, s, a));
    return ICD_OK;
}

template <int D, int VAR = CF_PRODUCT_VAR, int KP = CO_KP, bool PERSIST = false>
int launch_coarse_flat(icd_index *x, const CoarseFlatArgs &a, int nwg, hipStream_t s) {
    constexpr auto kern = coarse_flat_kernel<D, VAR, KP, PERSIST>;
    constexpr int lds = cf_lds_bytes(VAR);
    HIP_TRY(launch_lds<kern>(x->device, (size_t)(lds), dim3(nwg), dim3(256), lds, s, a));
    return ICD_OK;
}

constexpr int LDS_LIMIT = 160 * 1024;
constexpr size_t PIN_Q_BYTES = 64 * 1024;
constexpr size_t PIN_DONE_BYTES = 64;
constexpr size_t PIN_OUT_BYTES = 96 * 1024;

inline bool stream_fits(int kp, int qb, int dim) {
    const int e = kp <= 32 ? 2 : (kp == 64 ? 3 : 4);
    return (size_t)qb * dim * 4 + (size_t)4 * 2 * ST_STAGE_BYTES + (size_t)4 * qb * 64 * e * 8 <= (size_t)LDS_LIMIT;
}

template <int KP, int E, int QB, bool BAND = false, bool MASK = false, bool BOOST = false>
int launch_stream(icd_index *x, const float *dq, const int *qlist, const int *nq_ptr, int nq, int max_active,
                  int p_out, int *p_used, hipStream_t s, const float *thr0 = nullptr, const BandQ *band = nullptr, RowMasks mask = nullptr,
                  const BoostQ *boost = nullptr) {
    const int n = (int)x->n;
    const int per_max = FIN_MAX_CAND / KP;
    const int p_cap = FIN_MAX_CAND / KP;
    const int rows_per_wg = stream_rows_per_wg(n, x->num_cu);
    if ((long long)rows_per_wg * x->dim * 4 > FLAT_DESC_MAX_BYTES) return fail(ICD_ERR_UNSUPPORTED, "stream kernel: %d rows x dim %d per work-group exceed its buffer descriptor", rows_per_wg, x->dim);
    const int nwg = (n + rows_per_wg - 1) / rows_per_wg;
    int plan[8];
    const int levels = plan_reduce_levels(4 * nwg, per_max, p_out, p_cap, plan);
    if (levels <= 0) return fail(ICD_ERR_INVALID, "stream kernel: no reduction plan for %d lists (KP=%d, P=%d)", 4 * nwg, KP, p_out);
    p_out = plan[levels - 1];
    if (p_used) *p_used = p_out;
    StreamArgs a{};
    a.corpus = x->corpus; a.queries = dq; a.qlist = qlist; a.nq_ptr = nq_ptr; a.nq = std::min(nq, max_active);
    a.max_active = max_active; a.n = n; a.dim = x->dim; a.rows_per_wg = rows_per_wg; a.nwg = nwg;
    a.list_scores = x->lists_s; a.list_rows = x->lists_r; a.thr0 = thr0; a.band.q = band; a.mask = mask; a.boost = boost;
    int stages = 4;
    while (stages > 2 && stream_lds_bytes<KP, E, QB>(x->dim, stages) > (size_t)LDS_LIMIT) --stages;
    a.ring_stages = stages;
    if ((size_t)a.nq * 4 * nwg * KP > x->lists_cap) return fail(ICD_ERR_INVALID, "stream workspace too small");
    for (int l = 0; l < levels; ++l) {
        const size_t cap = (l % 2 == 0) ? x->partx_cap + (size_t)128 * FIN_MAX_CAND_X : x->lists_cap;
        if ((size_t)a.nq * plan[l] * KP > cap) return fail(ICD_ERR_INVALID, "stream workspace too small for reduction level %d", l);
    }
    constexpr auto kern = stream_topk_kernel<KP, E, QB, false, BAND, MASK, BOOST>;
    const size_t lds = stream_lds_bytes<KP, E, QB>(x->dim, stages);
    if (lds > (size_t)LDS_LIMIT) return fail(ICD_ERR_INVALID, "stream kernel: dim=%d does not fit LDS with %d queries per pass", x->dim, QB);
    HIP_TRY(launch_lds<kern>(x->device, (size_t)((int)lds), dim3(nwg), dim3(256), lds, s, a));
    int nlists = 4 * nwg;
    for (int l = 0; l < levels; ++l) {
        ReduceArgs r{};
        r.list_scores = (l % 2 == 0) ? x->lists_s : x->partx_s; r.list_rows = (l % 2 == 0) ? x->lists_r : x->partx_r;
        r.part_scores = (l % 2 == 0) ? x->partx_s : x->lists_s; r.part_rows = (l % 2 == 0) ? x->partx_r : x->lists_r;
        r.nlists = nlists; r.KP = KP; r.P_out = plan[l];
        r.nq_ptr = nq_ptr; r.nq = a.nq; r.max_active = max_active;
        hipLaunchKernelGGL(reduce_lists_kernel, dim3((a.nq * plan[l] + 3) / 4), dim3(256), 4 * 512 * 8, s, r);
        HIP_TRY(hipGetLastError());
        nlists = plan[l];
    }
    return ICD_OK;
}

struct StreamOnePlan { int rps, rows_per_wg, nwg, stages; };
inline bool plan_stream_one(int n, int dim, int num_cu, int qb, int cap_entries, StreamOnePlan *p) {
    const StreamOneRows g = plan_stream_one_rows(n, num_cu);
    const int rps = g.rps;
    p->rps = g.rps; p->rows_per_wg = g.rows_per_wg; p->nwg = g.nwg;
    if ((long long)g.rows_per_wg * dim * 4 > FLAT_DESC_MAX_BYTES) return false;
    const size_t fixed = (size_t)qb * dim * 4 + (size_t)4 * qb * cap_entries * 8;
    if (fixed + (size_t)4 * 2 * rps * 128 > (size_t)LDS_LIMIT) return false;
    p->stages = (int)std::min<size_t>(8, ((size_t)LDS_LIMIT - fixed) / ((size_t)4 * rps * 128));
    return p->nwg >= 1 && p->nwg <= 256 && p->stages >= 2;
}

template <int KP, int E, int QB, bool BAND = false, bool MASK = false, bool BOOST = false>
int launch_stream_one(icd_index *x, const float *dq, int nq, const FinArgs &f, hipStream_t s, const float *host_q = nullptr, bool poll_done = false,
                      const BandArgs *band = nullptr, RowMasks mask = nullptr, const BoostQ *boost = nullptr) {
    StreamOnePlan pl;
    if (!plan_stream_one((int)x->n, x->dim, x->num_cu, QB, 64 * E, &pl)) return fail(ICD_ERR_INVALID, "single-launch stream kernel: no plan for n=%lld dim=%d", (long long)x->n, x->dim);
    if ((size_t)nq * pl.nwg * KP * 2 > x->lists_cap) return fail(ICD_ERR_INVALID, "stream workspace too small");
    StreamArgs a{};
    a.corpus = x->corpus; a.queries = dq; a.qlist = nullptr; a.nq_ptr = nullptr; a.nq = nq; a.max_active = nq;
    a.n = (int)x->n; a.dim = x->dim; a.rows_per_wg = pl.rows_per_wg; a.nwg = pl.nwg; a.ring_stages = pl.stages;
    a.rows_per_step = pl.rps;
    a.wg_keys = reinterpret_cast<u64 *>(x->lists_s);
    a.ticket = reinterpret_cast<u64 *>(x->nflag + 6);
    a.fin = f;
    a.fin.counters = x->nflag; a.fin.host_counters = x->h_nflag_dev;
    if (band) a.band = *band;
    a.mask = mask; a.boost = boost;
    if (poll_done) {
        a.done = reinterpret_cast<u64 *>(x->h_pin_dev + PIN_Q_BYTES + PIN_OUT_BYTES);
        a.done_value = ++x->done_seq;
        x->done_armed = true;
    }
    const size_t lds = std::max<size_t>(stream_one_lds_bytes<KP, E, QB>(x->dim, pl.stages, pl.rps), (size_t)84 * 1024);
    constexpr auto kern = stream_topk_kernel<KP, E, QB, true, BAND, MASK, BOOST>;
    if constexpr (QB == 1) {
        if (host_q) {
            constexpr auto kern_in = stream_one_inline_kernel<KP, E, BAND, MASK, BOOST>;
            StreamInlineQuery iq;
            memcpy(iq.v, host_q, (size_t)x->dim * sizeof(float));
            a.queries = nullptr;
            HIP_TRY(launch_lds<kern_in>(x->device, (size_t)LDS_LIMIT, dim3(pl.nwg), dim3(256), lds, s, a, iq));
            return ICD_OK;
        }
    }
    HIP_TRY(launch_lds<kern>(x->device, (size_t)LDS_LIMIT, dim3(pl.nwg), dim3(256), lds, s, a));
    return ICD_OK;
}

template <bool RESCORE, bool DEEP, int EWM>
int launch_finalize_t(icd_index *x, const FinArgs &a, hipStream_t s) {
    constexpr auto kern = finalize_kernel<RESCORE, DEEP, EWM>;
    const size_t lds = 4 * fin_wave_lds_bytes(RESCORE, x->dim, a.lds_cand > 0 ? a.lds_cand : a.P * a.KP, EWM);
    const size_t lds_limit = (size_t)((int)(4 * fin_wave_lds_bytes(RESCORE, x->dim, (!RESCORE && EWM >= 4) ? FIN_MAX_CAND_X : FIN_MAX_CAND, EWM)));
    HIP_TRY(launch_lds<kern>(x->device, lds_limit, dim3((a.nq + 3) / 4), dim3(256), lds, s, a));
    return ICD_OK;
}

template <bool RESCORE>
int launch_finalize(icd_index *x, const FinArgs &a, hipStream_t s) {
    const bool deep = RESCORE && a.nq <= 8 * x->num_cu;
    if (!RESCORE && std::max(a.lds_cand, a.P * a.KP) > FIN_MAX_CAND) return launch_finalize_t<false, false, 4>(x, a, s);
    if (a.k <= 32) return deep ? launch_finalize_t<RESCORE, true, 1>(x, a, s) : launch_finalize_t<RESCORE, false, 1>(x, a, s);
    return deep ? launch_finalize_t<RESCORE, true, 4>(x, a, s) : launch_finalize_t<RESCORE, false, 4>(x, a, s);
}

void rec(icd_index *x, int i, hipStream_t s) {
    if (x->prof_now) {
        hipEventRecord(x->ev[i], s);
        x->ev_valid[i] = true;
    }
}

struct Outs {
    float *scores; long long *ids;
    double *adj; float *adj_raw; long long *adj_ids; int *adj_lv;
    int *lv;
};

__global__ void gather_rows_kernel(const float *src, float *dst, long long stride, int dim, int rows) {
    const int r = blockIdx.x;
    if (r >= rows) return;
    const float4 *s4 = reinterpret_cast<const float4 *>(src + (size_t)r * stride * dim);
    float4 *d4 = reinterpret_cast<float4 *>(dst + (size_t)r * dim);
    for (int i = threadIdx.x; i < dim / 4; i += blockDim.x) d4[i] = s4[i];
}

__global__ __launch_bounds__(256) void gather_view_rows_kernel(const float *src, const int *src_levels, const long long *map,
                                                               long long id_base, long long rows, int dim, float *dst, int *dst_levels) {
    const long long i = (long long)blockIdx.x * 4 + (threadIdx.x >> 6);
    const int lane = threadIdx.x & 63;
    if (i >= rows) return;
    const long long r = map[i] - id_base;
// ... 214 lines not shown
            a.band = c.band->q; a.mask = c.mask;
            if (kpx == 16) rc = launch_exact<16, 1, 4, 60, 16, 2, 32, true, true>(x, a, c.mtx, s);
            else if (kpx == 32) rc = launch_exact<32, 1, 4, 62, 16, 2, 16, true, true>(x, a, c.mtx, s);
            else if (kpx == 64) rc = launch_exact<64, 2, 4, 112, 32, 1, 32, true, true>(x, a, c.mtx, s);
            else rc = launch_exact<128, 3, 2, 192, 32, 1, 32, true, true>(x, a, c.mtx, s);
        }
        else if (c.band) {
            a.band = c.band->q;
            if (kpx == 16) rc = launch_exact<16, 1, 4, 60, 16, 2, 32, true>(x, a, c.mtx, s);
            else if (kpx == 32) rc = launch_exact<32, 1, 4, 62, 16, 2, 16, true>(x, a, c.mtx, s);
            else if (kpx == 64) rc = launch_exact<64, 2, 4, 112, 32, 1, 32, true>(x, a, c.mtx, s);
            else rc = launch_exact<128, 3, 2, 192, 32, 1, 32, true>(x, a, c.mtx, s);
        }
        else if (launch_exact_variant(x, c.ov, kpx, a, c.mtx, s, &rc)) {}
        else if (kpx == 16) rc = launch_exact<16, 1, 4, 60, 16, 2>(x, a, c.mtx, s);
        else if (kpx == 32) rc = launch_exact<32, 1, 4, 62, 16, 2, 16>(x, a, c.mtx, s);
        else if (kpx == 64) rc = launch_exact<64, 2, 4, 112>(x, a, c.mtx, s);
        else rc = launch_exact<128, 3, 2>(x, a, c.mtx, s);
        if (rc) return rc;
    }
    rec(x, 4, s);
    FinArgs g = c.f;
    g.part_scores = x->partx_s; g.part_rows = x->partx_r; g.P = px; g.KP = kpx;
    g.P_dense = px_dense; g.sparse_max = sparse_here; g.track_run = track_run ? 1 : 0; g.lds_cand = std::max(px, (stream && mfma) ? c.p_dense_max : px_dense) * kpx;
    g.dense_grid = c.mtx * std::max(1, px_dense); g.dense_bmq = c.bmq; g.dense_max_p = (stream && mfma) ? c.p_dense_max : 0; g.dense_one_per_cu = c.wg_per_cu_x > 1 ? x->num_cu : 0; g.n_rows = (int)x->n;
    g.nq = nq; g.nq_ptr = nq_ptr; g.qlist = qlist;
    g.counters = x->nflag; g.host_counters = x->h_nflag_dev;
    rc = launch_finalize<false>(x, g, s);
    rec(x, 5, s);
    return rc;
}

int stage_host_query(const SearchCtx &c) {
    icd_index *x = c.x;
    if (!x->host_q) return ICD_OK;
    const size_t qbytes = (size_t)x->dim * sizeof(float);
    memcpy(x->h_pin, x->host_q, qbytes);
    HIP_TRY(hipMemcpyAsync(x->qdev, x->h_pin, qbytes, hipMemcpyHostToDevice, c.s));
    x->host_q = nullptr;
    return ICD_OK;
}

int stage_host_bands(const SearchCtx &c) {
    icd_index *x = c.x;
    if (!c.band || x->band_pending <= 0) return ICD_OK;
    HIP_TRY(hipMemcpyAsync(x->band_dev, x->h_band, (size_t)x->band_pending * sizeof(BandQ), hipMemcpyHostToDevice, c.s));
    x->band_pending = 0;
    return ICD_OK;
}


int search_tiny(const SearchCtx &c) {
    icd_index *x = c.x;
    const int nq = c.nq;
    hipStream_t s = c.s;
    x->last_mode = ICD_MODE_EXACT;
    x->last_chunks = c.p_sparse;
    StreamOnePlan pl;
    const int qb1 = nq <= 1 ? 1 : (nq <= 2 ? 2 : 4);
    const bool one = nq <= 4 && c.kpx == 16 && x->opt_stream_one && plan_stream_one((int)x->n, x->dim, x->num_cu, qb1, 64 * 2, &pl) &&
                     (size_t)nq * pl.nwg * c.kpx * 2 <= x->lists_cap;
    if (one) {
        rec(x, 3, s);
        const float *hq = qb1 == 1 ? x->host_q : nullptr;
        if (!hq) { const int rcq = stage_host_query(c); if (rcq) return rcq; }
        const bool poll = x->host_one_call && (x->opt_host_one & 2) != 0;
        if (c.band) {
            BandArgs b = *c.band;
            if (x->band_pending > 0) { b.q = nullptr; x->band_pending = 0; }
            if (c.mask && c.boost) {
                const int rco = qb1 == 1 ? launch_stream_one<16, 2, 1, true, true, true>(x, c.dq, 1, c.f, s, hq, poll, &b, c.mask, c.boost->q)
                              : qb1 == 2 ? launch_stream_one<16, 2, 2, true, true, true>(x, c.dq, 2, c.f, s, nullptr, false, &b, c.mask, c.boost->q)
                                         : launch_stream_one<16, 2, 4, true, true, true>(x, c.dq, (int)nq, c.f, s, nullptr, false, &b, c.mask, c.boost->q);
                rec(x, 4, s);
                rec(x, 5, s);
                return rco;
            }
            if (c.mask) {
                const int rcm = qb1 == 1 ? launch_stream_one<16, 2, 1, true, true>(x, c.dq, 1, c.f, s, hq, poll, &b, c.mask)
                              : qb1 == 2 ? launch_stream_one<16, 2, 2, true, true>(x, c.dq, 2, c.f, s, nullptr, false, &b, c.mask)
                                         : launch_stream_one<16, 2, 4, true, true>(x, c.dq, (int)nq, c.f, s, nullptr, false, &b, c.mask);
                rec(x, 4, s);
                rec(x, 5, s);
                return rcm;
            }
            const int rcb = qb1 == 1 ? launch_stream_one<16, 2, 1, true>(x, c.dq, 1, c.f, s, hq, poll, &b)
                          : qb1 == 2 ? launch_stream_one<16, 2, 2, true>(x, c.dq, 2, c.f, s, nullptr, false, &b)
                                     : launch_stream_one<16, 2, 4, true>(x, c.dq, (int)nq, c.f, s, nullptr, false, &b);
            rec(x, 4, s);
            rec(x, 5, s);
            return rcb;
        }
        const int rc1 = qb1 == 1 ? launch_stream_one<16, 2, 1>(x, c.dq, 1, c.f, s, hq, poll) : qb1 == 2 ? launch_stream_one<16, 2, 2>(x, c.dq, 2, c.f, s)
                      : launch_stream_one<16, 2, 4>(x, c.dq, (int)nq, c.f, s);
        rec(x, 4, s);
        rec(x, 5, s);
        return rc1;
    }
    { const int rcq = stage_host_query(c); if (rcq) return rcq; }
    { const int rcb = stage_host_bands(c); if (rcb) return rcb; }
    HIP_TRY(hipMemsetAsync(x->nflag, 0, sizeof(int), s));
    rec(x, 3, s);
    return run_exact(c, nullptr, nullptr, c.p_sparse, false, true);
}

int search_exact_narrow(const SearchCtx &c, bool *taken) {
    icd_index *x = c.x;
    const int nq = c.nq, k = c.k;
    hipStream_t s = c.s;
    *taken = false;
    HIP_TRY(hipMemsetAsync(x->nflag, 0, sizeof(int), s));
    const int slots = x->num_cu * 2;
    const int mtx_n = (nq + 127) / 128;
    const int p_need = std::max(2, (k + 7) / 8);
    const int pn = fullest_round(mtx_n, slots, p_need, std::min(FIN_MAX_CAND_X / 32, std::max(p_need + 8, slots / std::max(1, mtx_n))), 2.0);
    if (!((size_t)nq * pn * 32 <= x->partx_cap && pn * 32 <= FIN_MAX_CAND_X)) return ICD_OK;
    *taken = true;
    x->last_chunks = pn;
    x->fallback_word = 0;
    rec(x, 3, s);
    ExactArgs a{};
    a.corpus = x->corpus; a.queries = c.dq; a.nq = nq; a.n = (int)x->n; a.dim = x->dim; a.P = pn; a.strided = 1;
    a.rows_per_chunk = 128;
    a.part_scores = x->partx_s; a.part_rows = x->partx_r;
    int rc = launch_exact<32, 1, 4, 62, 16, 2, 16>(x, a, mtx_n, s);
    if (rc) return rc;
    rec(x, 4, s);
    FinArgs g = c.f;
    g.part_scores = x->partx_s; g.part_rows = x->partx_r; g.P = pn; g.KP = 32; g.nq = nq; g.lds_cand = pn * 32;
    g.narrow_check = 1; g.nflag = x->nflag; g.flagged = x->flagged;
    rc = launch_finalize<false>(x, g, s);
    if (rc) return rc;
    rec(x, 5, s);
    return run_exact(c, x->flagged, x->nflag, std::min(c.p_sparse, c.row_tiles), true, c.stream_ok, true, false, nullptr);
}

int search_exact(const SearchCtx &c) {
    icd_index *x = c.x;
    HIP_TRY(hipMemsetAsync(x->nflag, 0, sizeof(int), c.s));
    int px = pick_chunks(c.mtx, c.row_tiles, c.pmax_x, x->num_cu * c.wg_per_cu_x);
    const int rc = fit_chunks(c, &px);
    if (rc) return rc;
    x->last_chunks = px;
    rec(x, 3, c.s);
    return run_exact(c, nullptr, nullptr, px, true, false);
}

struct AutoPlan {
    bool wide_lists;
    bool wide_now;
    bool sparse_off;
    int kp_c;
    int ctiles, U, nwg;
    int pc;
    CoarseFlatArgs a;
    int p2, nwg2;
    CoarseFlatArgs a2;
};

int auto_prep(const SearchCtx &c, int nq_pad) {
    icd_index *x = c.x;
    ConvertArgs cv{};
    cv.src = c.dq; cv.dst = x->q16; cv.rows = c.nq; cv.rows_pad = nq_pad; cv.dim = x->dim; cv.mode = 0;
    cv.norm = x->qnorm; cv.res = x->qres; cv.scale_exp = x->qexp; cv.bad = x->qbad; cv.zero_u32 = x->shared_thr; cv.zero_i32 = x->nflag;
    cv.zero_u32b = x->shared_thr + x->max_nq_pad;
    hipLaunchKernelGGL(convert_rows_kernel, dim3((nq_pad + 3) / 4), dim3(256), 0, c.s, cv);
    HIP_TRY(hipGetLastError());
    rec(x, 1, c.s);
    return ICD_OK;
}

int split_class_period(int U, int ctiles, int nwg, int xcd_mode = -1) {
    int period = flat_class_period(U, ctiles);
    const int members = nwg / std::max(1, period);
    int split = (members + 11) / 12;
    if (xcd_mode == 0) period = 0;
    else if (xcd_mode == 1) period = 1 << 30;
    else if (xcd_mode == 2) split = 1;
    if (period > 0 && period < (1 << 20)) period *= std::max(1, split);
    return period;
}

int auto_plan(const SearchCtx &c, int nq_pad, AutoPlan &pl) {
    icd_index *x = c.x;
    const int nq = c.nq, k = c.k;
    const int mtc = nq_pad / 128;
    const int ctiles_min = (int)((x->n + 127) / 128);
    const FlatPlan plan = plan_flat_tiles(mtc, ctiles_min, x->n_pad / 128 - ctiles_min, x->num_cu);
    const int ctiles = plan.ctiles;
    pl.ctiles = ctiles;
    pl.wide_lists = k > x->opt_wide_from && x->dim == 768;
    const bool counters_in = !x->capturing && hipEventQuery(x->ev_nflag) == hipSuccess;
    if (counters_in) policy_take_counters(x->pol, search_counters(x->h_nflag));
    const SearchDecision dec = policy_decide(x->pol, x->adapt_enabled, nq, k, x->chunks_override);
    pl.sparse_off = dec.sparse_off;
    pl.wide_now = dec.wide_now;
    pl.kp_c = pl.wide_lists ? CO_KP_WIDE : CO_KP;

    CoarseFlatArgs &a = pl.a;
    a = CoarseFlatArgs{};
    a.q16 = x->q16; a.c16 = x->c16; a.nq = nq; a.n = (int)x->n; a.n_pad = ctiles * 128; a.ctiles = ctiles;
    a.total_units = mtc * ctiles;
    a.boot_tiles = c.ov.flat_boot >= 0 ? c.ov.flat_boot : std::max(1, std::min(CO_BOOT_TILES, 96 / std::max(1, k)));
    a.sparse_from = c.ov.flat_sparse >= 0 ? c.ov.flat_sparse : CO_SPARSE_FROM;
    CoarsePlanIn pin{};
    pin.mtc = mtc; pin.ctiles = ctiles; pin.U = std::max(plan.U, c.ov.flat_u); pin.nq = nq; pin.k = k;
    pin.kp = pl.kp_c; pin.kp2 = CO_KP; pin.max_cand = FIN_MAX_CAND;
    pin.wide_lists = pl.wide_lists; pin.wide_now = pl.wide_now; pin.chunks_override = x->chunks_override;
    pin.pass2 = x->pass2_enabled && x->pol.pass2_armed() && x->part2_s;
    pin.partc_cap = (long long)x->partc_cap; pin.part2_cap = (long long)x->part2_cap;
    pin.max_list_tiles = flat_max_list_tiles(x->dim);
    if (c.ov.flat_list > 0) pin.list_override = c.ov.flat_list;
    const CoarsePlan cp = plan_coarse_lists(pin);
    if (!cp.ok)
        return fail(ICD_ERR_UNSUPPORTED, "coarse pass: no list plan for n=%lld dim=%d nq=%d k=%d (lists per query %d, at most %d tiles per list)",
                    (long long)x->n, x->dim, nq, k, cp.P, pin.max_list_tiles);
    const int U = cp.U;
    pl.U = U; pl.pc = cp.P;
    x->last_chunks = cp.P;
    pl.nwg = (a.total_units + U - 1) / U;
    a.list_tiles = cp.list_tiles;
    a.units_per_wg = U; a.P = cp.P;
    a.pos_period = split_class_period(U, ctiles, pl.nwg, c.ov.xcd_mode);
    a.part_scores = x->partc_s; a.part_rows = x->partc_r; a.bounds = x->partc_b; a.shared_thr = x->shared_thr;
    a.dbg = x->dbg;
    a.nwg_virtual = pl.nwg;
    pl.p2 = 0; pl.nwg2 = 0;
    pl.a2 = CoarseFlatArgs{};
    if (cp.P2 > 0) {
        const int U2 = cp.U2;
        CoarseFlatArgs &a2 = pl.a2;
        pl.p2 = cp.P2;
        a2 = a;
        a2.nq_ptr = nullptr; a2.qlist = nullptr;
        a2.units_per_wg = U2; a2.list_tiles = cp.list_tiles2; a2.P = pl.p2;
        a2.boot_tiles = a.boot_tiles;
        pl.nwg2 = (int)(((long long)mtc * ctiles + U2 - 1) / U2);
        a2.pos_period = split_class_period(U2, ctiles, pl.nwg2);
        a2.nwg_virtual = pl.nwg2;
        a2.part_scores = x->part2_s; a2.part_rows = x->part2_r; a2.bounds = x->part2_b;
        a2.shared_thr = x->shared_thr + x->max_nq_pad;
    }
    return ICD_OK;
}

int auto_coarse(const SearchCtx &c, AutoPlan &pl) {
    icd_index *x = c.x;
    hipStream_t s = c.s;
    CoarseFlatArgs &a = pl.a;
    const int nwg = pl.nwg;
    int rc;
    if (launch_coarse_variant(x, c.ov, a, nwg, s, &rc)) return rc;
    if (x->dim == 1024) return launch_coarse_flat<1024, (CF_PRODUCT_VAR & (3 | 16 | 2048))>(x, a, nwg, s);
    if (pl.wide_lists) return launch_coarse_flat<768, CF_PRODUCT_VAR, CO_KP_WIDE>(x, a, nwg, s);
    if ((size_t)x->n_pad * x->dim * 2 <= COARSE_CACHED_IMAGE_BYTES) return launch_coarse_flat<768, CF_CACHED_VAR>(x, a, nwg, s);
    const int t0 = flat_class_period(pl.U, pl.ctiles);
    const int members0 = t0 > 0 ? nwg / t0 : 0;
    const int epochs = x->opt_pace_shift >= 0 ? (pl.U >> x->opt_pace_shift) + 1 : 0;
    if (x->opt_pace_shift >= 0 && members0 >= 4 && (size_t)t0 * epochs <= PACE_WORDS) {
        a.pace = x->pace; a.pace_period = t0; a.pace_epochs = epochs; a.pace_shift = x->opt_pace_shift; a.pace_lead = std::max(1, x->opt_pace_lead);
        HIP_TRY(hipMemsetAsync(x->pace, 0, (size_t)t0 * epochs * sizeof(unsigned int), s));
    }
    return launch_coarse_flat<768, CF_PACED_VAR>(x, a, nwg, s);
}

int auto_first_finalize(const SearchCtx &c, const AutoPlan &pl, FinArgs &g, bool *wide_fin) {
    icd_index *x = c.x;
    const int nq = c.nq, k = c.k;
    hipStream_t s = c.s;
    g = c.f;
    g.part_scores = x->partc_s; g.part_rows = x->partc_r; g.bounds = x->partc_b; g.P = pl.pc; g.KP = pl.kp_c; g.nq = nq;
    g.perm_mul = x->perm_mul; g.perm_mod = x->perm_mod;
    g.perm_inv = (x->perm_mod > 0 && (double)x->perm_mod * (double)x->perm_mod < 9007199254740992.0) ? 1.0 / (double)x->perm_mod : 0.0;
    *wide_fin = pl.wide_now && k <= 32 && pl.pc * g.KP >= 128;
    if (*wide_fin) g.wide_window = 1;
    if (c.ov.fin_skip_walk) g.skip_walk = 1;
    if (*wide_fin && x->opt_family_order && nq >= 1024) {
        OrderArgs o{};
        o.part_scores = g.part_scores; o.part_rows = g.part_rows; o.P = g.P; o.KP = g.KP; o.nq = nq;
        o.perm_mul = g.perm_mul; o.perm_mod = g.perm_mod; o.perm_inv = g.perm_inv;
        o.shift = 6;
        while (((long long)x->n >> o.shift) >= ORDER_BUCKETS) ++o.shift;
        o.key = x->order_key; o.hist = x->order_hist; o.order = x->order;
        HIP_TRY(hipMemsetAsync(x->order_hist, 0, 2 * ORDER_BUCKETS * sizeof(unsigned int), s));
        hipLaunchKernelGGL(order_keys_kernel, dim3((nq + 3) / 4), dim3(256), 0, s, o);
        hipLaunchKernelGGL(order_scatter_kernel, dim3((nq + 1023) / 1024), dim3(1024), 0, s, o);
        HIP_TRY(hipGetLastError());
        g.qlist = x->order; g.lists_by_query = 1; g.nq = 4 * ((nq + 3) / 4);
    }
    const int rc = *wide_fin ? launch_finalize_t<true, false, 4>(x, g, s) : launch_finalize<true>(x, g, s);
    g.qlist = nullptr; g.lists_by_query = 0; g.nq = nq;
    return rc;
}

int auto_wide_retry(const SearchCtx &c, const FinArgs &g) {
    icd_index *x = c.x;
    FinArgs g2 = g;
    g2.qlist = x->flagged; g2.nq_ptr = x->nflag; g2.lists_by_query = 1; g2.wide_window = 1;
    g2.nflag = x->nflag + 1; g2.flagged = x->flagged + x->max_nq_pad;
    const int rc = launch_finalize_t<true, false, 4>(x, g2, c.s);
    if (rc) return rc;
    x->fallback_word = 1;
    return ICD_OK;
}

int auto_second_pass(const SearchCtx &c, AutoPlan &pl, const FinArgs &g) {
    icd_index *x = c.x;
    hipStream_t s = c.s;
    CoarseFlatArgs &a2 = pl.a2;
    const int w_in = x->fallback_word;
    a2.nq_ptr = x->nflag + w_in;
    a2.qlist = x->flagged + (size_t)w_in * x->max_nq_pad;
    a2.skip_below = PASS2_SKIP;
    const int grid2 = std::max(8, std::min(pl.nwg2, x->num_cu) & ~7);
    int rc;
    if (x->dim == 1024) rc = launch_coarse_flat<1024, (CF_PRODUCT_VAR & (3 | 16 | 2048)), CO_KP, true>(x, a2, grid2, s);
    else rc = launch_coarse_flat<768, CF_PRODUCT_VAR, CO_KP, true>(x, a2, grid2, s);
    if (rc) return rc;
    FinArgs g3 = g;
    g3.part_scores = x->part2_s; g3.part_rows = x->part2_r; g3.bounds = x->part2_b; g3.P = pl.p2; g3.KP = CO_KP;
    g3.qlist = a2.qlist; g3.nq_ptr = a2.nq_ptr; g3.lists_by_query = 0; g3.wide_window = 1; g3.skip_below = PASS2_SKIP;
    g3.nflag = x->nflag + 2; g3.flagged = x->flagged + (size_t)2 * x->max_nq_pad;
    rc = launch_finalize_t<true, false, 4>(x, g3, s);
    if (rc) return rc;
    x->fallback_word = 2;
    x->last_p2 = pl.p2; x->last_p2_word = w_in;
    return ICD_OK;
}

int auto_fallback(const SearchCtx &c, bool sparse_off) {
    icd_index *x = c.x;
    const int *fl_list = x->flagged + (size_t)x->fallback_word * x->max_nq_pad;
    const int *fl_count = x->nflag + x->fallback_word;
    int px = std::min(c.p_sparse, c.row_tiles);
    if (px < c.p_sparse) {
        const int rc = fit_chunks(c, &px);
        if (rc) return rc;
        return run_exact(c, fl_list, fl_count, px, true, false, true, true, c.f.thr0);
    }
    return run_exact(c, fl_list, fl_count, c.p_sparse, true, c.stream_ok, !sparse_off, true, c.f.thr0);
}

int search_auto(const SearchCtx &c) {
    icd_index *x = c.x;
    const int nq_pad = ((c.nq + 127) / 128) * 128;
    int rc = auto_prep(c, nq_pad);
    if (rc) return rc;
    AutoPlan pl;
    rc = auto_plan(c, nq_pad, pl);
    if (rc) return rc;
    rc = auto_coarse(c, pl);
    if (rc) return rc;
    rec(x, 2, c.s);
    FinArgs g;
    bool wide_fin = false;
    rc = auto_first_finalize(c, pl, g, &wide_fin);
    if (rc) return rc;
    x->fallback_word = 0;
    if (!wide_fin && c.k <= 32 && pl.pc * g.KP >= 128) {
        rc = auto_wide_retry(c, g);
        if (rc) return rc;
    }
    if (pl.p2 > 0) {
        rc = auto_second_pass(c, pl, g);
        if (rc) return rc;
    }
    policy_note_search(x->pol, x->adapt_enabled, x->pass2_enabled, c.nq, pl.p2, pl.wide_now, x->chunks_override, pl.pc * pl.kp_c);
    rec(x, 3, c.s);
    return auto_fallback(c, pl.sparse_off);
}

int search_device(icd_index *x, const float *dq, int nq, int k, int mode, const Outs &o, hipStream_t s, const BandArgs *band = nullptr, RowMasks mask = nullptr,
                  const BoostDev *boost = nullptr) {
    const bool use_fast = !band && (mode == ICD_MODE_AUTO) && x->fast && k <= FAST_MAX_K && (x->dim == 768 || x->dim == 1024);
    x->prof_now = !x->capturing && x->profiling && (x->prof_tick++ % x->prof_every == 0);
    if (x->prof_now) {
        const int slot = (int)(x->prof_count % EV_RING);
        x->ev = x->evring[slot];
        x->ev_valid = x->evring_valid[slot];
        ++x->prof_count;
        for (int i = 0; i <= NUM_EV; ++i) x->ev_valid[i] = false;
    }
    x->last_nq = nq;
    x->fallback_word = 0;
    x->last_p2 = 0;
    x->last_mode = use_fast ? ICD_MODE_AUTO : ICD_MODE_EXACT;
    rec(x, 0, s);
    const SearchCtx c = make_search_ctx(x, dq, nq, k, use_fast, o, s, band, mask, boost);
    if (c.stream_ok && nq <= (use_fast ? (k <= 16 ? 16 : 0) : ST_MAX_ACTIVE)) return search_tiny(c);
    { const int rcq = stage_host_query(c); if (rcq) return rcq; }
    { const int rcb = stage_host_bands(c); if (rcb) return rcb; }
    if (!band && !use_fast && c.kpx > 32 && x->opt_exact_narrow && nq > ST_MAX_ACTIVE && c.row_tiles >= 64) {
        bool taken = false;
        const int rc = search_exact_narrow(c, &taken);
        if (rc || taken) return rc;
    }
    return use_fast ? search_auto(c) : search_exact(c);
}

}

extern "C" {

int icd_abi_version(void) { return ICD_ABI_VERSION; }

const char *icd_last_error(void) { return g_err.c_str(); }

int icd_device_count(void) {
// ... 405 lines not shown
    BandArgs band{};
    x->band_pending = 0;
    if (r.range && (rc = pack_bands(x, *r.range, (int)nq, s, &band))) return rc;
    const float *dq = x->qdev;
    const size_t qbytes = (size_t)nq * x->dim * sizeof(float);
    if (!r.q_on_device && nq == 1 && (x->opt_host_one & 1) && qbytes <= sizeof(StreamInlineQuery) && !x->capturing) {
        x->host_q = r.queries;
    } else {
        const float *src = r.queries;
        if (!r.q_on_device && qbytes <= PIN_Q_BYTES) { memcpy(x->h_pin, src, qbytes); src = reinterpret_cast<const float *>(x->h_pin); }
        if ((rc = hc.upload(src, x->qdev, (size_t)nq * x->dim, &dq))) return rc;
    }
    const Outs &user = r.outs;
    Outs dev = user;
    const size_t no = (size_t)nq * k;
    const bool pinned_out = !r.out_on_device && no * 36 <= PIN_OUT_BYTES;
    if (pinned_out) {
        char *d = x->h_pin_dev + PIN_Q_BYTES;
        dev.adj = user.adj ? reinterpret_cast<double *>(d) : nullptr;                          d += no * 8;
        dev.ids = user.ids ? reinterpret_cast<long long *>(d) : nullptr;                       d += no * 8;
        dev.adj_ids = user.adj_ids ? reinterpret_cast<long long *>(d) : nullptr;               d += no * 8;
        dev.scores = user.scores ? reinterpret_cast<float *>(d) : nullptr;                     d += no * 4;
        dev.adj_raw = user.adj_raw ? reinterpret_cast<float *>(d) : nullptr;                   d += no * 4;
        dev.adj_lv = user.adj_lv ? reinterpret_cast<int *>(d) : nullptr;
        dev.lv = (user.lv && !user.adj_lv) ? reinterpret_cast<int *>(d) : nullptr;
    } else {
        dev.scores = hc.target(user.scores, x->o_scores); dev.ids = hc.target(user.ids, x->o_ids);
        dev.adj = hc.target(user.adj, x->o_adj); dev.adj_raw = hc.target(user.adj_raw, x->o_adj_raw);
        dev.adj_ids = hc.target(user.adj_ids, x->o_adj_ids);
        dev.adj_lv = hc.target(user.adj_lv, x->o_adj_lv); dev.lv = hc.target(user.lv, x->o_adj_lv);
    }
    x->done_armed = false;
    x->host_one_call = !r.q_on_device && nq == 1 && pinned_out && !x->capturing;
    rc = search_device(x, dq, (int)nq, k, r.mode, dev, s, r.range ? &band : nullptr, (r.masks || r.boost) ? x->mask_dev : nullptr, r.boost ? &boost : nullptr);
    x->band_pending = 0;
    x->host_q = nullptr;
    x->host_one_call = false;
    if (rc) return rc;
    rec(x, NUM_EV, s);
    if (x->done_armed && pinned_out) {
        const volatile unsigned long long *done = reinterpret_cast<const volatile unsigned long long *>(x->h_pin + PIN_Q_BYTES + PIN_OUT_BYTES);
        const auto t0 = std::chrono::steady_clock::now();
        bool seen = false;
        for (unsigned spin = 0;; ++spin) {
            if (__atomic_load_n(done, __ATOMIC_ACQUIRE) == x->done_seq) { seen = true; break; }
            if ((spin & 255u) == 255u && std::chrono::steady_clock::now() - t0 > std::chrono::microseconds(DONE_POLL_US)) break;
        }
        if (!seen) HIP_TRY(hipStreamSynchronize(s));
        copy_pinned_out(x, user, no);
        return ICD_OK;
    }
    if (!x->capturing) HIP_TRY(hipEventRecord(x->ev_nflag, s));
    if (pinned_out) {
        HIP_TRY(hipStreamSynchronize(s));
        copy_pinned_out(x, user, no);
        return ICD_OK;
    }
    if ((rc = hc.copy_back({{user.scores, dev.scores, 4}, {user.ids, dev.ids, 8}, {user.adj, dev.adj, 8}, {user.adj_raw, dev.adj_raw, 4},
                            {user.adj_ids, dev.adj_ids, 8}, {user.adj_lv, dev.adj_lv, 4}, {user.lv, dev.lv, 4}}, no)))
        return rc;
    return hc.finish(host_bands);
}

extern "C" {

int icd_index_search(icd_index *idx, const float *queries, int64_t nq, int32_t k, int32_t queries_on_device,
                     int32_t mode, float *out_scores, int64_t *out_ids, int32_t out_on_device, void *stream) {
    if (!out_scores || !out_ids) return fail(ICD_ERR_INVALID, "output pointer is NULL");
    return run_search(idx, SearchRequest{queries, nq, k, queries_on_device != 0, out_on_device != 0, mode,
                                         outs_for(false, nullptr, out_scores, out_ids, nullptr), nullptr, nullptr, reinterpret_cast<hipStream_t>(stream)});
}

int icd_index_search_reweighted(icd_index *idx, const float *queries, int64_t nq, int32_t k,
                                int32_t queries_on_device, int32_t mode, double *out_adj, float *out_raw,
                                int64_t *out_ids, int32_t *out_levels, int32_t out_on_device, void *stream) {
    if (!out_adj || !out_ids) return fail(ICD_ERR_INVALID, "output pointer is NULL");
    return run_search(idx, SearchRequest{queries, nq, k, queries_on_device != 0, out_on_device != 0, mode,
                                         outs_for(true, out_adj, out_raw, out_ids, out_levels), nullptr, nullptr, reinterpret_cast<hipStream_t>(stream)});
}

int icd_index_lookup_levels(icd_index *idx, const int64_t *ids, int64_t count, int32_t *out_levels, void *stream) {
    if (!valid(idx)) return fail(ICD_ERR_STATE, "invalid handle");
    if (idx->row_map) return fail(ICD_ERR_UNSUPPORTED, "icd_index_lookup_levels: not supported on a view (its hits carry their levels)");
    std::lock_guard<std::mutex> guard(idx->mu);
    if (!ids || !out_levels || count < 0) return fail(ICD_ERR_INVALID, "bad arguments");
    if (count == 0) return ICD_OK;
    HIP_TRY(hipSetDevice(idx->device));
    hipLaunchKernelGGL(lookup_levels_kernel, dim3((unsigned)((count + 255) / 256)), dim3(256), 0,
                       reinterpret_cast<hipStream_t>(stream), reinterpret_cast<const long long *>(ids),
                       (long long)count, idx->levels, (long long)idx->id_base, (long long)idx->n, out_levels);
    HIP_TRY(hipGetLastError());
    return ICD_OK;
}

int icd_index_stats(icd_index *idx, icd_stats *out) {
    if (!valid(idx)) return fail(ICD_ERR_STATE, "invalid handle");
    std::lock_guard<std::mutex> guard(idx->mu);
    if (!out) return fail(ICD_ERR_INVALID, "out is NULL");
    memset(out, 0, sizeof *out);
    out->n = idx->n; out->dim = idx->dim; out->device = idx->device; out->id_base = idx->id_base;
    out->bytes_corpus_f32 = (int64_t)idx->n * idx->dim * 4;
    out->bytes_corpus_f16 = idx->c16 ? (int64_t)idx->n_pad * idx->dim * 2 : 0;
    out->bytes_workspace = (int64_t)idx->bytes_ws;
    out->max_nq = idx->max_nq; out->max_k = idx->max_k; out->fast_path = idx->fast ? 1 : 0;
    out->rmax = idx->rmax;
    out->last_nq = idx->last_nq;
    int nf = 0;
    if (idx->h_nflag && idx->last_nq > 0) {
        HIP_TRY(hipSetDevice(idx->device));
        HIP_TRY(hipEventSynchronize(idx->ev_nflag));
        nf = idx->h_nflag[idx->fallback_word];
    }
    out->last_fallback = nf;
    out->last_second_pass = (idx->last_p2 > 0 && idx->h_nflag && idx->last_nq > 0) ? idx->h_nflag[idx->last_p2_word] : 0;
    out->last_second_pass_lists = idx->last_p2;
    out->wide_mode = idx->pol.wide_mode ? 1 : 0;
    out->second_pass_armed = (idx->pass2_enabled && idx->pol.pass2_armed()) ? 1 : 0;
    out->sparse_fallback_armed = idx->pol.sparse_disarmed ? 0 : 1;
    out->centered = idx->cmean ? 1 : 0; out->mean_share = idx->mean_share;
    out->last_chunks = idx->last_chunks; out->last_mode = idx->last_mode;
    return ICD_OK;
}

int icd_index_cert_terms(icd_index *idx, float *cmax, float *dcmax, int32_t *cexp, float *qnorm, float *qres, int64_t count) {
    if (!valid(idx)) return fail(ICD_ERR_STATE, "invalid handle");
    std::lock_guard<std::mutex> guard(idx->mu);
    if (!idx->fast) return fail(ICD_ERR_INVALID, "the index has no fp16 image");
    if (count < 0 || count > idx->max_nq_pad || ((qnorm || qres) && count > idx->last_nq))
        return fail(ICD_ERR_INVALID, "count=%lld exceeds the last search's batch", (long long)count);
    if (cmax) *cmax = idx->rmax_scaled;
    if (dcmax) *dcmax = idx->dcmax_scaled;
    if (cexp) *cexp = idx->cexp;
    if (count > 0 && (qnorm || qres)) {
        HIP_TRY(hipSetDevice(idx->device));
        HIP_TRY(hipDeviceSynchronize());
        if (qnorm) HIP_TRY(hipMemcpy(qnorm, idx->qnorm, (size_t)count * sizeof(float), hipMemcpyDeviceToHost));
        if (qres) HIP_TRY(hipMemcpy(qres, idx->qres, (size_t)count * sizeof(float), hipMemcpyDeviceToHost));
    }
    return ICD_OK;
}

int icd_index_set_option(icd_index *idx, int32_t option, int32_t value) {
    if (!valid(idx)) return fail(ICD_ERR_STATE, "invalid handle");
    std::lock_guard<std::mutex> guard(idx->mu);
    icd_index *x = idx;
    switch (option) {
    case ICD_OPT_FAMILY_ORDER: x->opt_family_order = (value & 1) != 0; break;
    case ICD_OPT_STREAM_ONE:   x->opt_stream_one = value != 0; break;
    case ICD_OPT_HOST_ONE:     x->opt_host_one = value & 3; break;
    case ICD_OPT_PACING_SHIFT: x->opt_pace_shift = value > 12 ? 12 : value; break;
    case ICD_OPT_PACING_LEAD:  x->opt_pace_lead = value < 1 ? 1 : value; break;
    case ICD_OPT_EXACT_NARROW: x->opt_exact_narrow = value != 0; break;
    case ICD_OPT_WIDE_FROM:    x->opt_wide_from = value < 0 ? 0 : value; break;
    default: return fail(ICD_ERR_INVALID, "option %d: not one of ICD_OPT_*", option);
    }
    return ICD_OK;
}

int icd_index_set_second_pass(icd_index *idx, int32_t enabled) {
    if (!valid(idx)) return fail(ICD_ERR_STATE, "invalid handle");
    std::lock_guard<std::mutex> guard(idx->mu);
    idx->pass2_enabled = enabled != 0;
    idx->adapt_enabled = enabled == 1;
    idx->pol.rearm(idx->pass2_enabled && idx->adapt_enabled);
    if (idx->nflag) { HIP_TRY(hipSetDevice(idx->device)); HIP_TRY(hipDeviceSynchronize()); HIP_TRY(hipMemset(idx->nflag + 4, 0, sizeof(int))); idx->h_nflag[4] = 0; }
    return ICD_OK;
}

int icd_index_set_chunks(icd_index *idx, int32_t chunks) {
    if (!valid(idx)) return fail(ICD_ERR_STATE, "invalid handle");
    std::lock_guard<std::mutex> guard(idx->mu);
    if (chunks < 0 || chunks > COARSE_MAX_P) return fail(ICD_ERR_INVALID, "chunks=%d (0..%d)", chunks, COARSE_MAX_P);
    idx->chunks_override = chunks;
    return ICD_OK;
}

int icd_index_debug_counters(icd_index *idx, unsigned long long *out, int32_t count) {
    if (!valid(idx)) return fail(ICD_ERR_STATE, "invalid handle");
    std::lock_guard<std::mutex> guard(idx->mu);
    if (!out || count <= 0 || count > 8192 * 16) return fail(ICD_ERR_INVALID, "bad arguments");
    HIP_TRY(hipSetDevice(idx->device));
    HIP_TRY(hipMemcpy(out, idx->dbg, (size_t)count * 8, hipMemcpyDeviceToHost));
    return ICD_OK;
}

int icd_index_set_profiling(icd_index *idx, int32_t enabled) {
    if (!valid(idx)) return fail(ICD_ERR_STATE, "invalid handle");
    std::lock_guard<std::mutex> guard(idx->mu);
    if (enabled < 0) return fail(ICD_ERR_INVALID, "enabled=%d", enabled);
    idx->profiling = enabled != 0;
    idx->prof_every = enabled > 1 ? enabled : 1;
    idx->prof_tick = 0;
    return ICD_OK;
}

int icd_index_profile_summary(icd_index *idx, icd_profile *out_mean, int32_t *out_count) {
    if (!valid(idx)) return fail(ICD_ERR_STATE, "invalid handle");
    std::lock_guard<std::mutex> guard(idx->mu);
    if (!out_mean || !out_count) return fail(ICD_ERR_INVALID, "out is NULL");
    memset(out_mean, 0, sizeof *out_mean);
    HIP_TRY(hipSetDevice(idx->device));
    const long total = idx->prof_count;
    const int n = (int)std::min<long>(total, EV_RING);
    int used = 0;
    double acc[6] = {0, 0, 0, 0, 0, 0};
    for (int j = 0; j < n; ++j) {
        const int slot = (int)((total - 1 - j) % EV_RING);
        hipEvent_t *ev = idx->evring[slot];
        const bool *ok = idx->evring_valid[slot];
        if (!ok[0] || !ok[NUM_EV]) continue;
        HIP_TRY(hipEventSynchronize(ev[NUM_EV]));
        auto span = [&](int a, int b) -> double {
            float ms = 0.f;
            if (ok[a] && ok[b]) hipEventElapsedTime(&ms, ev[a], ev[b]);
            return ms;
        };
        acc[0] += span(0, 1); acc[1] += span(1, 2); acc[2] += span(2, 3); acc[3] += span(3, 4);
        acc[4] += span(4, 5); acc[5] += span(0, NUM_EV);
        ++used;
    }
    if (used) {
        out_mean->ms_prep = (float)(acc[0] / used); out_mean->ms_coarse = (float)(acc[1] / used);
        out_mean->ms_finalize = (float)(acc[2] / used); out_mean->ms_exact = (float)(acc[3] / used);
        out_mean->ms_exact_finalize = (float)(acc[4] / used); out_mean->ms_total = (float)(acc[5] / used);
    }
    *out_count = used;
    idx->prof_count = 0;
    for (int r = 0; r < EV_RING; ++r)
        for (int i = 0; i <= NUM_EV; ++i) idx->evring_valid[r][i] = false;
    return ICD_OK;
}

int icd_index_last_profile(icd_index *idx, icd_profile *out) {
    if (!valid(idx)) return fail(ICD_ERR_STATE, "invalid handle");
    std::lock_guard<std::mutex> guard(idx->mu);
    if (!out) return fail(ICD_ERR_INVALID, "out is NULL");
    memset(out, 0, sizeof *out);
    if (!idx->ev_valid[0] || !idx->ev_valid[NUM_EV]) return fail(ICD_ERR_STATE, "no profiled search recorded");
    HIP_TRY(hipSetDevice(idx->device));
    HIP_TRY(hipEventSynchronize(idx->ev[NUM_EV]));
    auto span = [&](int a, int b) -> float {
        float ms = 0.f;
        if (idx->ev_valid[a] && idx->ev_valid[b]) hipEventElapsedTime(&ms, idx->ev[a], idx->ev[b]);
        return ms;
    };
    out->ms_prep = span(0, 1);
    out->ms_coarse = span(1, 2);
    out->ms_finalize = span(2, 3);
    out->ms_exact = span(3, 4);
    out->ms_exact_finalize = span(4, 5);
    out->ms_total = span(0, NUM_EV);
    return ICD_OK;
}

}

#include "icd_utility.hpp"
#include "icd_grouped.hpp"
#include "icd_maxsim.hpp"
#include "icd_hybrid.hpp"
#include "icd_sparse.hpp"
#include "icd_text_match.hpp"
#include "icd_filter.hpp"
#include "icd_facet.hpp"
#include "icd_mmr.hpp"
#include "icd_byrows.hpp"
#include "icd_encoder.hpp"
```

Measured before the change: 15.96 million queries/s.

## Split the ragged last query tile across waves by corpus rows in coarse pass

The final partial query tile, with nq not a multiple of 128, is processed in a row-split form. Each wave handles its own corpus rows for the few real queries, so wasted query slots no longer drive the tile schedule. A new planner weighs split and unsplit work-unit layouts and picks the split one when it lowers per-workgroup units. This adds a new kernel template path and more planning complexity, and carries a risk of correctness or register pressure issues in the specialized loop.

Measured after the change: 15.98 million queries/s, median of 4. About the same (+0.1%).

```diff
diff --git a/include/icd_search.h b/include/icd_search.h
--- a/include/icd_search.h
+++ b/include/icd_search.h
@@ -292,7 +292,7 @@
 int icd_index_set_second_pass(icd_index *idx, int32_t enabled);
 
 enum { ICD_OPT_FAMILY_ORDER = 1, ICD_OPT_STREAM_ONE = 2, ICD_OPT_HOST_ONE = 3, ICD_OPT_PACING_SHIFT = 4, ICD_OPT_PACING_LEAD = 5, ICD_OPT_EXACT_NARROW = 6,
-       ICD_OPT_WIDE_FROM = 7 };
+       ICD_OPT_WIDE_FROM = 7, ICD_OPT_RAGGED_SPLIT = 8 };
 int icd_index_set_option(icd_index *idx, int32_t option, int32_t value);
 
 int icd_unpack_query_slices(int32_t device, const void *gathered, int32_t world, int64_t nq, int32_t k, double *out_adj,
diff --git a/rag_project_icd10_amd/_native.py b/rag_project_icd10_amd/_native.py
--- a/rag_project_icd10_amd/_native.py
+++ b/rag_project_icd10_amd/_native.py
@@ -57,7 +57,7 @@
 NORMS = {"none": 0, "cosine": 1, "atan": 2}
 MAX_K = 128
 CREATE_CORPUS_ON_DEVICE, CREATE_ROW_ORDER, CREATE_NO_PROBE, CREATE_NO_CENTER = 1, 2, 4, 8
-OPTIONS = {"family_order": 1, "stream_one": 2, "host_one": 3, "pacing_shift": 4, "pacing_lead": 5, "exact_narrow": 6, "wide_from": 7}
+OPTIONS = {"family_order": 1, "stream_one": 2, "host_one": 3, "pacing_shift": 4, "pacing_lead": 5, "exact_narrow": 6, "wide_from": 7, "ragged_split": 8}
 GROUP_ROW_SHARD = 0
 GROUP_QUERY_SHARD = 1
 GROUP_ID_BYTES = 128
diff --git a/rag_project_icd10_amd/csrc/coarse_flat_kernel.hpp b/rag_project_icd10_amd/csrc/coarse_flat_kernel.hpp
--- a/rag_project_icd10_amd/csrc/coarse_flat_kernel.hpp
+++ b/rag_project_icd10_amd/csrc/coarse_flat_kernel.hpp
@@ -32,6 +32,8 @@
     int pace_epochs;
     int pace_shift;
     int pace_lead;
+    int split_from;
+    int split_units;
 };
 
 constexpr int CO_BOOT_MIN_TILES = 6;
@@ -228,7 +230,7 @@
     asm volatile("s_memtime %0\n\ts_waitcnt lgkmcnt(0)" : "=s"(t) :: "memory"); \
     __builtin_amdgcn_sched_barrier(0); } while (0)
 
-template <int D, int VAR = CF_PRODUCT_VAR, int KP = CO_KP, bool PERSIST = false>
+template <int D, int VAR = CF_PRODUCT_VAR, int KP = CO_KP, bool PERSIST = false, bool RSPLIT = false>
 __global__ __launch_bounds__(256, 1) void coarse_flat_kernel(CoarseFlatArgs a) {
     constexpr int CO_QUOTA = (CO_CAP - KP) / 2 - CO_CHECK_EVERY;
     static_assert(CO_QUOTA >= 8 && KP + 2 * (CO_QUOTA + CO_CHECK_EVERY) <= CO_CAP, "candidate buffer layout");
@@ -263,6 +265,8 @@
     constexpr bool LA_GUARDX = (VAR & 1073741824) != 0;
     static_assert(LOOKAHEAD || (VAR & (268435456 | 536870912 | 1073741824)) == 0, "sub-flags of the look-ahead bit");
     static_assert(!LA_GUARDX || !DIRTY_GUARD, "one form of the overflow guard");
+    static_assert(!RSPLIT || (X16 && DMA_WIDE && PF2 && LOOKAHEAD && BOOT_MED3 && !PAIRBAR && !PACE && !PERSIST && !STAMPS && !NOSEL && FLAT_SPLIT == 4),
+                  "the row-split form is built on the cached-image kernel's stage");
     constexpr int S = cf_ring_stages(VAR);
     constexpr int VM_MID = NOVM ? 63 : (PAIRBAR ? 4 : 4 * (S - 3));
     constexpr int PRO = PAIRBAR ? 4 : S - 1;
@@ -347,27 +351,44 @@
     }
     while (u < u_end) {
         const int mtile = u / a.ctiles;
-        const int t0 = u - mtile * a.ctiles;
+        int t0 = u - mtile * a.ctiles;
         const int run0 = max(u_begin - mtile * a.ctiles, 0);
         const int run1 = min(u_end - mtile * a.ctiles, a.ctiles);
         const int j = (t0 - run0) / a.list_tiles;
-        const int t1 = min(run1, run0 + (j + 1) * a.list_tiles);
-        const int ntiles = t1 - t0;
-        const int ord = flat_first_ordinal(mtile, wg, a.ctiles, a.units_per_wg, a.list_tiles) + j;
+        int t1 = min(run1, run0 + (j + 1) * a.list_tiles);
+        int ntiles = t1 - t0;
+        int ord = flat_first_ordinal(mtile, wg, a.ctiles, a.units_per_wg, a.list_tiles) + j;
         const int slot0 = mtile * CO_BM;
+        int adv = ntiles;
+        [[maybe_unused]] bool sp = false;
+        if constexpr (RSPLIT) {
+            sp = a.split_units > 0 && u >= a.split_from;
+            if (sp) {
+                const int v0 = u - a.split_from;
+                const int r0 = max(u_begin - a.split_from, 0), r1 = min(u_end - a.split_from, a.split_units);
+                const int js = (v0 - r0) / a.list_tiles;
+                const int v1 = min(r1, r0 + (js + 1) * a.list_tiles);
+                adv = v1 - v0;
+                t0 = FLAT_SPLIT * v0;
+                t1 = min(FLAT_SPLIT * v1, a.ctiles);
+                ntiles = t1 - t0;
+                ord = FLAT_SPLIT * (flat_first_ordinal_last(mtile, wg, a.ctiles, a.split_units, a.units_per_wg, a.list_tiles) + js) + wave;
+            }
+        }
+        const int wq = (RSPLIT && sp) ? 0 : wave * 32;
 
         if (mtile != cur_mtile) {
             if constexpr (X16) {
 #pragma unroll
                 for (int gr = 0; gr < 2; ++gr) {
-                    int qr = slot0 + wave * 32 + 16 * gr + q16;
+                    int qr = slot0 + wq + 16 * gr + q16;
                     if (PERSIST && a.qlist) qr = a.qlist[min(qr, nq_act - 1)];
                     const _Float16 *qrow = a.q16 + (size_t)qr * D + 8 * g16;
 #pragma unroll
                     for (int s = 0; s < NF / 2; ++s) qf[gr * (NF / 2) + s] = *reinterpret_cast<const half8 *>(qrow + 32 * s);
                 }
             } else {
-                int qr = slot0 + wave * 32 + c;
+                int qr = slot0 + wq + c;
                 if (PERSIST && a.qlist) qr = a.qlist[min(qr, nq_act - 1)];
                 const _Float16 *qrow = a.q16 + (size_t)qr * D + 8 * h;
 #pragma unroll
@@ -398,11 +419,12 @@
         };
 
         Sel2 st;
-        Ops::init(st, wave_qbase + (uint32_t)c * Ops::QBYTES, h, (slot0 + wave * 32 + c) < nq_act && !NOPASS);
+        Ops::init(st, wave_qbase + (uint32_t)c * Ops::QBYTES, h, (slot0 + wq + c) < nq_act && !NOPASS);
         float boot1 = -INFINITY, boot2 = -INFINITY, boot3 = -INFINITY;
-        const int boot_tiles = ntiles >= CO_BOOT_MIN_TILES ? min(a.boot_tiles, ntiles / 3) : 0;
-        unsigned int *my_shared = a.shared_thr + (slot0 + wave * 32 + c);
-        const bool publish = (slot0 + wave * 32 + c) < nq_act;
+        const int bsc = (RSPLIT && sp) ? FLAT_SPLIT : 1;
+        const int boot_tiles = ntiles >= bsc * CO_BOOT_MIN_TILES ? min(bsc * a.boot_tiles, ntiles / 3) : 0;
+        unsigned int *my_shared = a.shared_thr + (slot0 + wq + c);
+        const bool publish = (slot0 + wq + c) < nq_act;
         uint32_t published = 0u;
         int dirty = 0;
         auto filter_reg = [&](const f32x16 (&pa)[4], auto F, uint32_t rowbase, auto GUARD) {
@@ -536,9 +558,9 @@
                 filter_quad(pa, px, std::integral_constant<int, 2 * g + 1>{}, rowbase, GUARD);
             }
         };
-        auto filter_block = [&](const f32x4 (&px)[X16 ? 16 : 1], auto Q0, uint32_t rowbase, auto GUARD) {
-            constexpr int q0 = decltype(Q0)::value;
-            unsigned long long m[LA_B][LA_MAX ? 1 : 4];
+        auto filter_block = [&](const auto &px, auto NBk, auto Q0, uint32_t rowbase, auto GUARD) {
+            constexpr int q0 = decltype(Q0)::value, nb = decltype(NBk)::value;
+            unsigned long long m[nb][LA_MAX ? 1 : 4];
             auto masked = [&](auto Q, auto I) {
                 constexpr int q = decltype(Q)::value, i = decltype(I)::value;
                 float v = px[X16 ? q : 0][i];
@@ -558,7 +580,7 @@
                              : "=&s"(m0), "=&s"(m1), "=&s"(m2), "=&s"(m3)
                              : "v"(t0), "v"(t1), "v"(t2), "v"(t3), "v"(thr));
             };
-            static_for<0, LA_B>([&](auto J) {
+            static_for<0, nb>([&](auto J) {
                 using Q = std::integral_constant<int, q0 + decltype(J)::value>;
                 constexpr int j = decltype(J)::value;
                 if constexpr (LA_MAX) {
@@ -570,7 +592,7 @@
                 } else cmp4(Q{}, m[j][0], m[j][LA_MAX ? 0 : 1], m[j][LA_MAX ? 0 : 2], m[j][LA_MAX ? 0 : 3]);
             });
             __builtin_amdgcn_sched_barrier(0);
-            static_for<0, LA_B>([&](auto J) {
+            static_for<0, nb>([&](auto J) {
                 constexpr int j = decltype(J)::value, q = q0 + j;
                 using Q = std::integral_constant<int, q>;
                 const uint32_t rowq = rowbase + (uint32_t)(16 * (q >> 1) + 4 * (q & 1));
@@ -589,6 +611,115 @@
             });
         };
 
+        [[maybe_unused]] auto split_tile_loop = [&]() {
+            half8 fr[2][2][2];
+            auto read_split = [&](half8 (&f)[2][2], int ring_slot) {
+                const char *sb = smem + ring_slot * CO_STAGE_BYTES + wave * 4096;
+#pragma unroll
+                for (int k2 = 0; k2 < 2; ++k2)
+#pragma unroll
+                    for (int rl = 0; rl < 2; ++rl) f[k2][rl] = *reinterpret_cast<const half8 *>(sb + rl * 2048 + rd_off[k2]);
+            };
+            read_split(fr[0], 0);
+            for (int tile = 0; tile < ntiles; ++tile) {
+                uint32_t seen_early = 0u;
+                f32x4 xs[4];
+#pragma unroll
+                for (int t = 0; t < 4; ++t)
+#pragma unroll
+                    for (int r = 0; r < 4; ++r) xs[t][r] = 0.0f;
+                static_for<0, KS>([&](auto KSI) {
+                    constexpr int ks = decltype(KSI)::value;
+                    constexpr int nslot = (ks + 1) % S, par = ks & 1;
+                    constexpr int pks = ks + S - 2, nks = ks + S - 1;
+                    auto mfma2 = [&](const half8 &f, int k2, int rl) {
+#pragma unroll
+                        for (int gr = 0; gr < 2; ++gr)
+                            xs[2 * rl + gr] = __builtin_amdgcn_mfma_f32_16x16x32_f16(f, qf[gr * (NF / 2) + 2 * ks + k2], xs[2 * rl + gr], 0, 0, 0);
+                    };
+                    mfma2(fr[par][0][0], 0, 0);
+                    __builtin_amdgcn_sched_barrier(0);
+                    issue_pieces(tile + pks / KS, pks % KS, pks % S, std::integral_constant<int, 2>{}, std::integral_constant<int, 3>{});
+                    __builtin_amdgcn_sched_barrier(0);
+                    mfma2(fr[par][0][1], 0, 1);
+                    __builtin_amdgcn_sched_barrier(0);
+                    issue_pieces(tile + pks / KS, pks % KS, pks % S, std::integral_constant<int, 3>{}, std::integral_constant<int, 4>{});
+                    __builtin_amdgcn_sched_barrier(0);
+                    asm volatile("s_waitcnt vmcnt(%0) lgkmcnt(0)\n\ts_barrier" ::"i"(VM_MID) : "memory");
+                    __builtin_amdgcn_sched_barrier(0);
+                    if constexpr (EARLY_THR && ks == KS - 2) {
+                        if (EXCH == 1 || (tile & (EXCH - 1)) == EXCH - 1) {
+                            asm volatile("global_load_dword %0, %1, off sc1" : "=v"(seen_early) : "v"(my_shared) : "memory");
+                        }
+                        __builtin_amdgcn_sched_barrier(0);
+                    }
+                    read_split(fr[1 - par], nslot);
+                    mfma2(fr[par][1][0], 1, 0);
+                    __builtin_amdgcn_sched_barrier(0);
+                    issue_pieces(tile + nks / KS, nks % KS, nks % S, std::integral_constant<int, 0>{}, std::integral_constant<int, 1>{});
+                    __builtin_amdgcn_sched_barrier(0);
+                    mfma2(fr[par][1][1], 1, 1);
+                    __builtin_amdgcn_sched_barrier(0);
+                    issue_pieces(tile + nks / KS, nks % KS, nks % S, std::integral_constant<int, 1>{}, std::integral_constant<int, 2>{});
+                    __builtin_amdgcn_sched_barrier(0);
+                });
+#pragma unroll
+                for (int rl = 0; rl < 2; ++rl)
+#pragma unroll
+                    for (int i = 0; i < 4; ++i) {
+                        const auto sw = __builtin_amdgcn_permlane16_swap(__float_as_uint(xs[2 * rl][i]), __float_as_uint(xs[2 * rl + 1][i]), false, false);
+                        xs[2 * rl][i] = __uint_as_float(sw[0]);
+                        xs[2 * rl + 1][i] = __uint_as_float(sw[1]);
+                    }
+                if (EXCH == 1 || (tile & (EXCH - 1)) == EXCH - 1) {
+                    uint32_t seen;
+                    if constexpr (EARLY_THR) {
+                        asm volatile("s_waitcnt vmcnt(%1)" : "+v"(seen_early) : "i"(VM_TILE_END) : "memory");
+                        seen = seen_early;
+                    } else {
+                        seen = __hip_atomic_load(my_shared, __ATOMIC_RELAXED, __HIP_MEMORY_SCOPE_AGENT);
+                    }
+                    const uint32_t mine_key = order_f32(st.thr);
+                    if (seen > mine_key) st.thr = unorder_f32(seen);
+                    else if (h == 0 && publish && mine_key > seen && mine_key > published) {
+                        __hip_atomic_fetch_max(my_shared, mine_key, __ATOMIC_RELAXED, __HIP_MEMORY_SCOPE_AGENT);
+                        published = mine_key;
+                    }
+                }
+                const int tile_row0 = (t0 + tile) * CO_BN;
+                const uint32_t rowbase = (uint32_t)(tile_row0 + 32 * wave + 8 * h);
+                if (tile < boot_tiles && tile_row0 + CO_BN <= a.n) {
+                    float c1 = -INFINITY, c2 = -INFINITY, c3 = -INFINITY;
+#pragma unroll
+                    for (int t = 0; t < 4; ++t)
+#pragma unroll
+                        for (int r = 0; r < 4; r += 2) {
+                            const float va = xs[t][r], vb = xs[t][r + 1];
+                            const float a3 = __builtin_amdgcn_fmed3f(boot2, boot3, va), a2 = __builtin_amdgcn_fmed3f(boot1, boot2, va);
+                            boot1 = raw_max_f32(boot1, va); boot2 = a2; boot3 = a3;
+                            const float b3 = __builtin_amdgcn_fmed3f(c2, c3, vb), b2 = __builtin_amdgcn_fmed3f(c1, c2, vb);
+                            c1 = raw_max_f32(c1, vb); c2 = b2; c3 = b3;
+                        }
+#pragma unroll
+                    for (int i = 0; i < 3; ++i) {
+                        const float v = i == 0 ? c1 : (i == 1 ? c2 : c3);
+                        const float a3 = __builtin_amdgcn_fmed3f(boot2, boot3, v), a2 = __builtin_amdgcn_fmed3f(boot1, boot2, v);
+                        boot1 = raw_max_f32(boot1, v); boot2 = a2; boot3 = a3;
+                    }
+                    const auto sw = __builtin_amdgcn_permlane32_swap(__float_as_uint(boot3), __float_as_uint(boot3), false, false);
+                    const float thr0 = fminf(boot3, __uint_as_float(h ? sw[0] : sw[1]));
+                    if (thr0 > st.thr) st.thr = thr0;
+                }
+                if (tile_row0 + CO_BN > a.n) filter_block(xs, std::integral_constant<int, 4>{}, std::integral_constant<int, 0>{}, rowbase, std::true_type{});
+                else filter_block(xs, std::integral_constant<int, 4>{}, std::integral_constant<int, 0>{}, rowbase, std::false_type{});
+                if constexpr (EPOCH > 0) {
+                    if ((tile + 1) % EPOCH == 0 && tile + 1 < ntiles && __builtin_amdgcn_ballot_w64(Ops::used(st, h) > 3) != 0ull)
+                        compact_all_parallel<KP, Ops>(smem, st, wave_qbase + (uint32_t)c * Ops::QBYTES, h, c);
+                }
+            }
+            asm volatile("" ::"v"(fr[0][0][0]), "v"(fr[0][0][1]), "v"(fr[0][1][0]), "v"(fr[0][1][1]));
+        };
+
         asm volatile("s_waitcnt vmcnt(0)" ::: "memory");
 #pragma unroll
         for (int p = 0; p < PRO - (DMA_WIDE ? 1 : 0); ++p) issue_stage(p / KS, p % KS, p % S);
@@ -599,6 +730,10 @@
         if constexpr (PF2) read_frags(bfn, 0, 1);
         if constexpr (STAMPS) ICD_CF_STAMP(st_prev);
 
+        if constexpr (RSPLIT) {
+            if (sp) split_tile_loop();
+        }
+        if (!(RSPLIT && sp))
         for (int tile = 0; tile < ntiles; ++tile) {
             uint32_t seen_early = 0u;
             [[maybe_unused]] uint32_t pace_seen = 0u;
@@ -859,8 +994,8 @@
                     for (int t = 0; t < 4; ++t) asm volatile("" ::"v"(acc[X16 ? 0 : t]));
                 }
             } else if constexpr (LOOKAHEAD) {
-                if (tile_row0 + CO_BN > a.n) static_for<0, 16 / LA_B>([&](auto Bk) { filter_block(xs, std::integral_constant<int, LA_B * decltype(Bk)::value>{}, rowbase, std::true_type{}); });
-                else static_for<0, 16 / LA_B>([&](auto Bk) { filter_block(xs, std::integral_constant<int, LA_B * decltype(Bk)::value>{}, rowbase, std::false_type{}); });
+                if (tile_row0 + CO_BN > a.n) static_for<0, 16 / LA_B>([&](auto Bk) { filter_block(xs, std::integral_constant<int, LA_B>{}, std::integral_constant<int, LA_B * decltype(Bk)::value>{}, rowbase, std::true_type{}); });
+                else static_for<0, 16 / LA_B>([&](auto Bk) { filter_block(xs, std::integral_constant<int, LA_B>{}, std::integral_constant<int, LA_B * decltype(Bk)::value>{}, rowbase, std::false_type{}); });
             } else if constexpr (QUAD) {
                 if (tile_row0 + CO_BN > a.n) static_for<0, 16>([&](auto Q) { filter_quad(acc, xs, Q, rowbase, std::true_type{}); });
                 else if (SPARSE_PRE && tile >= a.sparse_from) static_for<0, 8>([&](auto G) { filter_group(acc, xs, G, rowbase, std::false_type{}); });
@@ -886,14 +1021,14 @@
             const auto swm = __builtin_amdgcn_permlane32_swap((unsigned)mine, (unsigned)mine, false, false);
             const int other = (int)(h ? swm[0] : swm[1]);
             const int nlo = st.kept + (h ? other : mine), nhi = h ? mine : other;
-            const int slot = slot0 + wave * 32 + c;
+            const int slot = slot0 + wq + c;
             const bool store = slot < nq_act;
             const size_t o = ((size_t)min(slot, nq_act - 1) * a.P + ord) * KP;
             const float bound = flush_emit_parallel<KP>(smem, wave_qbase + (uint32_t)c * Ops::QBYTES, h, c, nlo, nhi, st.thr,
                                                            store, a.part_scores + o, a.part_rows + o);
             if (store && h == 0) {
                 a.bounds[(size_t)slot * a.P + ord] = bound;
-                if (t1 == a.ctiles) {
+                if (t1 == a.ctiles && (!(RSPLIT && sp) || wave == FLAT_SPLIT - 1)) {
                     for (int e = ord + 1; e < a.P; ++e) {
                         const size_t oe = ((size_t)slot * a.P + e) * KP;
                         for (int d = 0; d < KP; ++d) { a.part_scores[oe + d] = -INFINITY; a.part_rows[oe + d] = -1; }
@@ -903,7 +1038,7 @@
             }
         }
         __syncthreads();
-        u += ntiles;
+        u += adv;
     }
     }
     if constexpr (CLOCKS) {
diff --git a/rag_project_icd10_amd/csrc/flat_partition.hpp b/rag_project_icd10_amd/csrc/flat_partition.hpp
--- a/rag_project_icd10_amd/csrc/flat_partition.hpp
+++ b/rag_project_icd10_amd/csrc/flat_partition.hpp
@@ -80,6 +80,8 @@
     return worst;
 }
 
+inline int flat_lists_needed_split(int mtc, int ctiles, int U, int list_tiles, int split);
+
 struct CoarsePlanIn {
     int mtc, ctiles, U;
     int nq, k;
@@ -93,11 +95,13 @@
     int pass2;
     long long partc_cap, part2_cap;
     int max_list_tiles;
+    int split;
 };
 struct CoarsePlan {
     int ok;
     int U, list_tiles, P;
     int U2, list_tiles2, P2;
+    int split;
 };
 
 inline CoarsePlan plan_coarse_lists(const CoarsePlanIn &in) {
@@ -116,15 +120,16 @@
     }
     L = std::min(L, lcap);
     auto fits = [&](int p) { return p <= COARSE_MAX_P && p * in.kp <= in.max_cand && (long long)in.nq * p * in.kp <= in.partc_cap; };
-    int P = flat_lists_needed(in.mtc, ctiles, U, L);
+    const int split = in.split > 1 ? in.split : 1;
+    int P = flat_lists_needed_split(in.mtc, ctiles, U, L, split);
     while (!fits(P)) {
         if (L < lcap) L = std::min(lcap, L + std::max(1, L / 8));
         else if (U < ctiles) U = std::min(ctiles, U + std::max(1, U / 4));
         else break;
-        P = flat_lists_needed(in.mtc, ctiles, U, L);
+        P = flat_lists_needed_split(in.mtc, ctiles, U, L, split);
     }
     r.ok = fits(P) ? 1 : 0;
-    r.U = U; r.list_tiles = L; r.P = P;
+    r.U = U; r.list_tiles = L; r.P = P; r.split = split;
     if (!r.ok) return r;
     if (in.pass2 && P * in.kp < PASS2_BELOW) {
         int U2 = std::max(1, (ctiles + PASS2_CHUNKS - 1) / PASS2_CHUNKS);
@@ -139,6 +144,72 @@
         }
     }
     return r;
+}
+
+constexpr int FLAT_SPLIT = 4;
+constexpr int FLAT_SPLIT_MAX_REAL = 32;
+
+ICD_HD inline int flat_last_tile_queries(int nq) { return nq - (nq - 1) / FLAT_TILE_ROWS * FLAT_TILE_ROWS; }
+ICD_HD inline int flat_last_units(int ctiles, int split) { return (ctiles + split - 1) / split; }
+ICD_HD inline long long flat_total_units(int mtc, int ctiles, int split) {
+    return (long long)(mtc - 1) * ctiles + flat_last_units(ctiles, split);
+}
+
+ICD_HD inline int flat_first_ordinal_last(int mlast, int w, int ctiles, int ctl, int U, int list_tiles) {
+    const long long m0 = (long long)mlast * ctiles, m1 = m0 + ctl;
+    int ord = 0;
+    for (long long wp = m0 / U; wp < w; ++wp) {
+        const long long r0 = wp * U > m0 ? wp * U : m0;
+        const long long r1 = (wp + 1) * U < m1 ? (wp + 1) * U : m1;
+        if (r1 > r0) ord += flat_lists_of_run((int)(r1 - r0), list_tiles);
+    }
+    return ord;
+}
+
+inline int flat_lists_needed_split(int mtc, int ctiles, int U, int list_tiles, int split) {
+    if (split <= 1) return flat_lists_needed(mtc, ctiles, U, list_tiles);
+    const int full = mtc > 1 ? flat_lists_needed(mtc - 1, ctiles, U, list_tiles) : 0;
+    const int ctl = flat_last_units(ctiles, split);
+    const long long m1 = (long long)(mtc - 1) * ctiles + ctl;
+    const int last = flat_first_ordinal_last(mtc - 1, (int)((m1 - 1) / U) + 1, ctiles, ctl, U, list_tiles);
+    return std::max(full, split * last);
+}
+
+inline FlatPlan plan_flat_tiles_split(int mtc, int ctiles_min, int spare, int num_cu, int split) {
+    if (split <= 1) return plan_flat_tiles(mtc, ctiles_min, spare, num_cu);
+    FlatPlan best{ctiles_min, 1};
+    double best_cost = 1e300;
+    for (int ce = ctiles_min; ce <= ctiles_min + spare; ++ce) {
+        const long long units = flat_total_units(mtc, ce, split);
+        const int umin = (int)((units + num_cu - 1) / num_cu) > 1 ? (int)((units + num_cu - 1) / num_cu) : 1;
+        const int umax = umin + (umin / 16 > 1 ? umin / 16 : 1);
+        for (int U = umin; U <= umax; ++U) {
+            const int nwg = (int)((units + U - 1) / U);
+            const int members = nwg / flat_class_period(U, ce);
+            const double cost = (double)U * (members >= 4 ? 1.0 : (members >= 2 ? 1.03 : 1.07));
+            if (cost < best_cost - 1e-9) { best_cost = cost; best.ctiles = ce; best.U = U; }
+        }
+    }
+    return best;
+}
+
+struct BatchPlan { FlatPlan flat; CoarsePlan lists; int split; };
+inline BatchPlan plan_coarse_batch(CoarsePlanIn in, int ctiles_min, int spare, int num_cu, int u_floor, int split_mode) {
+    BatchPlan b{};
+    b.flat = plan_flat_tiles(in.mtc, ctiles_min, spare, num_cu);
+    in.ctiles = b.flat.ctiles; in.U = std::max(b.flat.U, u_floor); in.split = 1;
+    b.lists = plan_coarse_lists(in);
+    b.split = 1;
+    const bool qualifies = split_mode > 0 && flat_last_tile_queries(in.nq) <= FLAT_SPLIT_MAX_REAL && !in.wide_lists && !in.wide_now &&
+                           in.chunks_override <= 0 && ctiles_min + spare <= in.max_list_tiles;
+    if (!qualifies) return b;
+    BatchPlan s{};
+    s.flat = plan_flat_tiles_split(in.mtc, ctiles_min, spare, num_cu, FLAT_SPLIT);
+    in.ctiles = s.flat.ctiles; in.U = std::max(s.flat.U, u_floor); in.split = FLAT_SPLIT;
+    s.lists = plan_coarse_lists(in);
+    s.split = FLAT_SPLIT;
+    if (s.lists.ok && (split_mode >= 2 || !b.lists.ok || s.lists.U < b.lists.U)) return s;
+    return b;
 }
 
 inline long long coarse_partc_entries(int max_nq_pad, int kcap, int kp, int kp_wide, int max_cand) {
diff --git a/rag_project_icd10_amd/csrc/icd_search.hip b/rag_project_icd10_amd/csrc/icd_search.hip
--- a/rag_project_icd10_amd/csrc/icd_search.hip
+++ b/rag_project_icd10_amd/csrc/icd_search.hip
@@ -143,6 +143,7 @@
     int opt_host_one = 3;
     bool opt_stream_one = true;
     bool opt_family_order = true;
+    int opt_ragged_split = 1;
     int opt_wide_from = 48;
     int64_t n = 0, id_base = 0;
     long long *row_map = nullptr;
@@ -298,9 +299,9 @@
     return ICD_OK;
 }
 
-template <int D, int VAR = CF_PRODUCT_VAR, int KP = CO_KP, bool PERSIST = false>
+template <int D, int VAR = CF_PRODUCT_VAR, int KP = CO_KP, bool PERSIST = false, bool RSPLIT = false>
 int launch_coarse_flat(icd_index *x, const CoarseFlatArgs &a, int nwg, hipStream_t s) {
-    constexpr auto kern = coarse_flat_kernel<D, VAR, KP, PERSIST>;
+    constexpr auto kern = coarse_flat_kernel<D, VAR, KP, PERSIST, RSPLIT>;
     constexpr int lds = cf_lds_bytes(VAR);
     HIP_TRY(launch_lds<kern>(x->device, (size_t)(lds), dim3(nwg), dim3(256), lds, s, a));
     return ICD_OK;
@@ -821,6 +822,7 @@
     bool sparse_off;
     int kp_c;
     int ctiles, U, nwg;
+    int split;
     int pc;
     CoarseFlatArgs a;
     int p2, nwg2;
@@ -855,9 +857,6 @@
     const int nq = c.nq, k = c.k;
     const int mtc = nq_pad / 128;
     const int ctiles_min = (int)((x->n + 127) / 128);
-    const FlatPlan plan = plan_flat_tiles(mtc, ctiles_min, x->n_pad / 128 - ctiles_min, x->num_cu);
-    const int ctiles = plan.ctiles;
-    pl.ctiles = ctiles;
     pl.wide_lists = k > x->opt_wide_from && x->dim == 768;
     const bool counters_in = !x->capturing && hipEventQuery(x->ev_nflag) == hipSuccess;
     if (counters_in) policy_take_counters(x->pol, search_counters(x->h_nflag));
@@ -866,24 +865,32 @@
     pl.wide_now = dec.wide_now;
     pl.kp_c = pl.wide_lists ? CO_KP_WIDE : CO_KP;
 
-    CoarseFlatArgs &a = pl.a;
-    a = CoarseFlatArgs{};
-    a.q16 = x->q16; a.c16 = x->c16; a.nq = nq; a.n = (int)x->n; a.n_pad = ctiles * 128; a.ctiles = ctiles;
-    a.total_units = mtc * ctiles;
-    a.boot_tiles = c.ov.flat_boot >= 0 ? c.ov.flat_boot : std::max(1, std::min(CO_BOOT_TILES, 96 / std::max(1, k)));
-    a.sparse_from = c.ov.flat_sparse >= 0 ? c.ov.flat_sparse : CO_SPARSE_FROM;
     CoarsePlanIn pin{};
-    pin.mtc = mtc; pin.ctiles = ctiles; pin.U = std::max(plan.U, c.ov.flat_u); pin.nq = nq; pin.k = k;
+    pin.mtc = mtc; pin.nq = nq; pin.k = k;
     pin.kp = pl.kp_c; pin.kp2 = CO_KP; pin.max_cand = FIN_MAX_CAND;
     pin.wide_lists = pl.wide_lists; pin.wide_now = pl.wide_now; pin.chunks_override = x->chunks_override;
     pin.pass2 = x->pass2_enabled && x->pol.pass2_armed() && x->part2_s;
     pin.partc_cap = (long long)x->partc_cap; pin.part2_cap = (long long)x->part2_cap;
     pin.max_list_tiles = flat_max_list_tiles(x->dim);
     if (c.ov.flat_list > 0) pin.list_override = c.ov.flat_list;
-    const CoarsePlan cp = plan_coarse_lists(pin);
+    const bool split_kernel = x->dim == 768 && !pl.wide_lists && !c.ov.has_flat_var &&
+                              (size_t)x->n_pad * x->dim * 2 <= COARSE_CACHED_IMAGE_BYTES;
+    const BatchPlan bp = plan_coarse_batch(pin, ctiles_min, x->n_pad / 128 - ctiles_min, x->num_cu, c.ov.flat_u, split_kernel ? x->opt_ragged_split : 0);
+    const CoarsePlan &cp = bp.lists;
+    const int ctiles = bp.flat.ctiles;
+    pl.ctiles = ctiles;
+    pl.split = bp.split;
     if (!cp.ok)
         return fail(ICD_ERR_UNSUPPORTED, "coarse pass: no list plan for n=%lld dim=%d nq=%d k=%d (lists per query %d, at most %d tiles per list)",
                     (long long)x->n, x->dim, nq, k, cp.P, pin.max_list_tiles);
+
+    CoarseFlatArgs &a = pl.a;
+    a = CoarseFlatArgs{};
+    a.q16 = x->q16; a.c16 = x->c16; a.nq = nq; a.n = (int)x->n; a.n_pad = ctiles * 128; a.ctiles = ctiles;
+    a.total_units = (int)flat_total_units(mtc, ctiles, bp.split);
+    if (bp.split > 1) { a.split_from = (mtc - 1) * ctiles; a.split_units = flat_last_units(ctiles, bp.split); }
+    a.boot_tiles = c.ov.flat_boot >= 0 ? c.ov.flat_boot : std::max(1, std::min(CO_BOOT_TILES, 96 / std::max(1, k)));
+    a.sparse_from = c.ov.flat_sparse >= 0 ? c.ov.flat_sparse : CO_SPARSE_FROM;
     const int U = cp.U;
     pl.U = U; pl.pc = cp.P;
     x->last_chunks = cp.P;
@@ -902,6 +909,7 @@
         pl.p2 = cp.P2;
         a2 = a;
         a2.nq_ptr = nullptr; a2.qlist = nullptr;
+        a2.total_units = mtc * ctiles; a2.split_from = 0; a2.split_units = 0;
         a2.units_per_wg = U2; a2.list_tiles = cp.list_tiles2; a2.P = pl.p2;
         a2.boot_tiles = a.boot_tiles;
         pl.nwg2 = (int)(((long long)mtc * ctiles + U2 - 1) / U2);
@@ -922,7 +930,10 @@
     if (launch_coarse_variant(x, c.ov, a, nwg, s, &rc)) return rc;
     if (x->dim == 1024) return launch_coarse_flat<1024, (CF_PRODUCT_VAR & (3 | 16 | 2048))>(x, a, nwg, s);
     if (pl.wide_lists) return launch_coarse_flat<768, CF_PRODUCT_VAR, CO_KP_WIDE>(x, a, nwg, s);
-    if ((size_t)x->n_pad * x->dim * 2 <= COARSE_CACHED_IMAGE_BYTES) return launch_coarse_flat<768, CF_CACHED_VAR>(x, a, nwg, s);
+    if ((size_t)x->n_pad * x->dim * 2 <= COARSE_CACHED_IMAGE_BYTES) {
+        if (pl.split > 1) return launch_coarse_flat<768, CF_CACHED_VAR, CO_KP, false, true>(x, a, nwg, s);
+        return launch_coarse_flat<768, CF_CACHED_VAR>(x, a, nwg, s);
+    }
     const int t0 = flat_class_period(pl.U, pl.ctiles);
     const int members0 = t0 > 0 ? nwg / t0 : 0;
     const int epochs = x->opt_pace_shift >= 0 ? (pl.U >> x->opt_pace_shift) + 1 : 0;
@@ -1634,6 +1645,7 @@
     case ICD_OPT_PACING_LEAD:  x->opt_pace_lead = value < 1 ? 1 : value; break;
     case ICD_OPT_EXACT_NARROW: x->opt_exact_narrow = value != 0; break;
     case ICD_OPT_WIDE_FROM:    x->opt_wide_from = value < 0 ? 0 : value; break;
+    case ICD_OPT_RAGGED_SPLIT: x->opt_ragged_split = value < 0 ? 0 : (value > 2 ? 2 : value); break;
     default: return fail(ICD_ERR_INVALID, "option %d: not one of ICD_OPT_*", option);
     }
     return ICD_OK;
```
